# SimonsRoad/gf-pl-slam

Measured on AMD Instinct MI355X. Metric: stereo frames/sec (2k ORB + 500 LBD, 10 GN iters), higher is better.
Workload: dtype f64

## Files before the change

gf-pl-slam_amd/csrc/gfpl_abi.hip:

```cpp
#include <hip/hip_runtime.h>

#include <algorithm>
#include <atomic>
#include <cmath>
#include <mutex>
#include <cstdio>
#include <cstdlib>
#include <cstring>
#include <vector>

#include "../../include/gfpl.h"
#include "gfpl_kernels.hpp"

using namespace gfpl;

#define GFPL_NEV 10

struct gfpl_ctx {
    int device = 0;
    hipStream_t stream = nullptr;
    bool own_stream = false;
    gfpl_camera cam{};
    gfpl_config cfg{};
    bool has_cam = false, has_cfg = false;
// ... 33 lines not shown
struct gfpl_event {
    int device = 0;
    hipEvent_t ev = nullptr;
    int64_t records = 0;
};

int gfpl_ctx_device(const gfpl_ctx* c) { return c->device; }
void* gfpl_ctx_stream(const gfpl_ctx* c) { return (void*)c->stream; }
const gfpl_camera* gfpl_ctx_camera(const gfpl_ctx* c) { return c->has_cam ? &c->cam : nullptr; }
int64_t gfpl_event_records(const gfpl_event* e) { return e->records; }
void gfpl_ctx_attach(gfpl_ctx* c) { c->n_detectors.fetch_add(1); }
void gfpl_ctx_detach(gfpl_ctx* c) { c->n_detectors.fetch_sub(1); }


namespace {

#define HIPCHK(x)                                                  \
    do {                                                            \
        hipError_t e_ = (x);                                        \
        if (e_ != hipSuccess) {                                     \
            std::fprintf(stderr, "gfpl: %s failed: %s\n", #x, hipGetErrorString(e_)); \
            return GFPL_E_HIP;                                      \
        }                                                           \
    } while (0)

int debug_fill_byte() {
    const char* e = getenv("GFPL_DEBUG_FILL");
    return e ? (int)(strtol(e, nullptr, 0) & 0xFF) : 0;
}

template <typename F, typename H, typename V>
void frame_fields(F& f, H& o, V& v) {
    v.pt(f.pt.pl, o.pt_pl, 2); v.pt(f.pt.pl_obs, o.pt_pl_obs, 2);
    v.pt(f.pt.disp, o.pt_disp, 1); v.pt(f.pt.P, o.pt_P, 3); v.pt(f.pt.sigma2, o.pt_sigma2, 1);
    v.pt(f.pt.idx, o.pt_idx, 1); v.pt(f.pt.level, o.pt_level, 1); v.pt(f.pt.inlier, o.pt_inlier, 1);
    v.pt(f.pt.desc, o.pdesc, 32); v.count(f.pt.n);
    v.ls(f.ls.spl, o.ls_spl, 2); v.ls(f.ls.epl, o.ls_epl, 2);
    v.ls(f.ls.spl_obs, o.ls_spl_obs, 2); v.ls(f.ls.epl_obs, o.ls_epl_obs, 2);
    v.ls(f.ls.sdisp, o.ls_sdisp, 1); v.ls(f.ls.edisp, o.ls_edisp, 1);
    v.ls(f.ls.sdisp_obs, o.ls_sdisp_obs, 1); v.ls(f.ls.edisp_obs, o.ls_edisp_obs, 1);
    v.ls(f.ls.angle, o.ls_angle, 1); v.ls(f.ls.sigma2, o.ls_sigma2, 1);
    v.ls(f.ls.sP, o.ls_sP, 3); v.ls(f.ls.eP, o.ls_eP, 3);
    v.ls(f.ls.le, o.ls_le, 3); v.ls(f.ls.le_obs, o.ls_le_obs, 3);
    v.ls(f.ls.covS, o.ls_covS, 9); v.ls(f.ls.covE, o.ls_covE, 9);
    v.ls(f.ls.cut, o.ls_cut, 2); v.ls(f.ls.invcov, o.ls_invcov, 36);
    v.ls(f.ls.idx, o.ls_idx, 1); v.ls(f.ls.level, o.ls_level, 1); v.ls(f.ls.inlier, o.ls_inlier, 1);
    v.ls(f.ls.desc, o.ldesc, 32); v.count(f.ls.n);
    v.seq(f.pose.Tfw, o.Tfw, 16); v.seq(f.pose.DT, o.DT, 16);
    v.seq(f.pose.DT_cov, o.DT_cov, 36); v.seq(f.pose.Tfw_cov, o.Tfw_cov, 36);
    v.seq(f.pose.DT_cov_eig, o.DT_cov_eig, 6);
    v.seq(f.pose.err_norm, &o.err_norm, 1); v.seq(f.pose.time_stamp, &o.time_stamp, 1);
}

struct SlotCarve {
    Carver& c;
    size_t B, P, L;
    template <typename T, typename U> void pt(T*& d, U, int w) { d = c.take<T>(P * w); }
    template <typename T, typename U> void ls(T*& d, U, int w) { d = c.take<T>(L * w); }
    template <typename T, typename U> void seq(T*& d, U, int w) { d = c.take<T>(B * w); }
    void count(int32_t*& d) { d = c.take<int32_t>(B); }
};

void carve(Carver& c, gfpl_seqbatch* sb) {
    const size_t B = sb->B, P = (size_t)B * sb->kp_cap, L = (size_t)B * sb->kl_cap;
    const gfpl_frame_host none{};
    SlotCarve v{c, B, P, L};
    for (int s = 0; s < 2; ++s) frame_fields(sb->slot[s], none, v);
    sb->tr.matched_pt = c.take<int32_t>(B * sb->mpt_cap);
    sb->tr.n_matched_pt = c.take<int32_t>(B);
    sb->tr.matched_ls = c.take<int32_t>(B * sb->mls_cap);
    sb->tr.n_matched_ls = c.take<int32_t>(B);
    sb->tr.n_inliers = c.take<int32_t>(B);
    sb->tr.n_inliers_pt = c.take<int32_t>(B);
    sb->tr.n_inliers_ls = c.take<int32_t>(B);
    sb->tr.num_frame_loss = c.take<int32_t>(B);
    sb->tr.kf_T = c.take<double>(B * 16);
    sb->tr.kf_cov = c.take<double>(B * 36);
    sb->tr.kf_entropy0 = c.take<double>(B);
    sb->tr.kf_ratio = c.take<double>(B);
    sb->tr.kf_prev_iskf = c.take<int32_t>(B);
    sb->tr.kf_nsince = c.take<int32_t>(B);
    sb->tr.kf_flag = c.take<int32_t>(B);
    sb->scr.cut_rec = c.take<double>(B * sb->mls_cap * CUT_REC);
    sb->scr.knn = c.take<int32_t>(B * 2 * (size_t)sb->kp_cap * 3);
    sb->scr.proj = reinterpret_cast<double*>(sb->scr.knn);
    sb->scr.bytes = c.take<int64_t>(B * STEP_REC);
    sb->scr.n_subpix = c.take<int32_t>(B);
    sb->scr.cut_sum = c.take<double>(B * 24);
    sb->scr.cut_dtinv = c.take<double>(B * 16);
    sb->scr.cut_vtab = c.take<double>(B * sb->mls_cap * 2 * CUT_KS);
    sb->scr.pose_DT = c.take<double>(B * 16);
    sb->scr.pose_H = c.take<double>(B * 36);
    sb->scr.pose_err = c.take<double>(B);
    sb->scr.pose_ok = c.take<int32_t>(B);
    sb->scr.pose_in = c.take<double>(B * (6 * (size_t)sb->mpt_cap + 10 * (size_t)sb->mls_cap));
    sb->scr.pose_act = c.take<double>(B * (6 * (size_t)sb->mpt_cap + 10 * (size_t)sb->mls_cap));
    sb->scr.pose_dtini = c.take<double>(B * 16);
    sb->scr.cross_tinv = c.take<double>(B * 16);
    sb->scr.dbg = c.take<int64_t>(B * 8);
    sb->scr.cut_prog = c.take<int32_t>((size_t)1 << 17);
    sb->scr.cut_path = c.take<uint8_t>(B * sb->mls_cap * CUT_PATH);
    sb->scr.cut_flag = c.take<int32_t>(B);
    sb->scr.cut_vmax = c.take<double>(B * sb->mls_cap * CUT_VMAX);
    sb->scr.cut_offl = c.take<int32_t>(1 + B * sb->mls_cap);
    sb->scr.cut_dtln = c.take<int32_t>(1 + CUT_DTL * B);
    sb->scr.cut_dtl = c.take<double>(CUT_DTL * B * 32);
    sb->scr.kf_mask = c.take<int32_t>(B);
    sb->last_n_pt = c.take<int32_t>(B);
    sb->last_n_ls = c.take<int32_t>(B);
}

DevCam devcam(const gfpl_camera& c) {
    DevCam d;
    d.fx = c.fx; d.fy = c.fy; d.cx = c.cx; d.cy = c.cy; d.b = c.b;
    d.width = c.width; d.height = c.height; d.n_levels = c.n_levels;
    for (int i = 0; i < GFPL_MAX_LEVELS; ++i) {
        d.scale[i] = c.scale[i]; d.inv_scale[i] = c.inv_scale[i];
        d.lvl_cols[i] = c.lvl_cols[i]; d.lvl_rows[i] = c.lvl_rows[i];
        d.lvl_offset[i] = c.lvl_offset[i];
        d.sigma2_pt[i] = c.sigma2_pt[i]; d.sigma2_ln[i] = c.sigma2_ln[i];
    }
    d.pyr_bytes = c.pyr_bytes;
    return d;
}

KParams params(gfpl_seqbatch* sb, const gfpl_frames* in) {
    KParams p;
    std::memset(&p, 0, sizeof p);
    p.cam = devcam(sb->ctx->cam);
    p.cfg = sb->ctx->cfg;
    p.prev = sb->slot[sb->prev_slot];
    p.curr = sb->slot[1 - sb->prev_slot];
    p.tr = sb->tr;
    p.scr = sb->scr;
    if (in) p.in = *in;
    p.B = sb->B; p.kp_cap = sb->kp_cap; p.kl_cap = sb->kl_cap;
    p.mpt_cap = sb->mpt_cap; p.mls_cap = sb->mls_cap;
    p.cfg.max_point_match_num = std::min(p.cfg.max_point_match_num, sb->mpt_cap);
    p.cfg.max_line_match_num = std::min(p.cfg.max_line_match_num, sb->mls_cap);
    p.sp_maxD = (float)p.cam.fx;
    p.sp_mbf = (float)(p.cam.fx * p.cam.b);
    p.cut_tq = 0.25 * p.cfg.cut_certify - 4.0 * 0x1p-53;
    {
        const double s = p.cfg.cut_step, lo = p.cfg.cut_rng[0], hi = p.cfg.cut_rng[1];
        auto same = [](double x, double y) { return std::memcmp(&x, &y, sizeof x) == 0; };
        int n = 0;
        for (double t = 0.0; n < CUT_KS && t <= hi && s > 0.0; t = t + s) p.cut_keys[n++] = t;
        const int ns = n;
        for (int i = 1; i < ns && n < CUT_KS; ++i) {
            const double e = p.cut_keys[i] - s;
            bool have = false;
            for (int k = 0; k < n; ++k) have = have || same(p.cut_keys[k], e);
            if (!have && e >= lo) p.cut_keys[n++] = e;
        }
        for (int i = 0; i < n; ++i) {
            int up = -1, dn = -1;
            for (int k = 0; k < n; ++k) {
                if (same(p.cut_keys[k], p.cut_keys[i] + s)) up = k;
                if (same(p.cut_keys[k], p.cut_keys[i] - s)) dn = k;
            }
            p.cut_knxt[i] = (int8_t)up;
            p.cut_kprv[i] = (int8_t)dn;
        }
        p.cut_nkeys = n;
    }
    return p;
// ... 898 lines not shown
    HIPCHK(v.e);
    HIPCHK(hipStreamSynchronize(s));
    sb->initialized = true;
    if (which == GFPL_CURR) sb->has_curr = true;
    return GFPL_OK;
}

int gfpl_read_track(gfpl_seqbatch* sb, int seq, gfpl_track_host* o) {
    return read_track(sb, seq, o, sb ? sb->tr.n_matched_pt : nullptr, sb ? sb->tr.n_matched_ls : nullptr);
}

int gfpl_read_last_track(gfpl_seqbatch* sb, int seq, gfpl_track_host* o) {
    return read_track(sb, seq, o, sb ? sb->last_n_pt : nullptr, sb ? sb->last_n_ls : nullptr);
}

int gfpl_write_track(gfpl_seqbatch* sb, int seq, const gfpl_track_host* o) {
    if (!sb || !o || seq < 0 || seq >= sb->B) return GFPL_E_INVALID;
    if (o->n_matched_pt < 0 || o->n_matched_pt > sb->mpt_cap || o->n_matched_ls < 0 || o->n_matched_ls > sb->mls_cap)
        return GFPL_E_CAPACITY;
    hipStream_t s = sb->ctx->stream;
    XFER(h2d, sb->tr.n_matched_pt + seq, &o->n_matched_pt, 1);
    XFER(h2d, sb->tr.n_matched_ls + seq, &o->n_matched_ls, 1);
    XFER(h2d, sb->tr.n_inliers + seq, &o->n_inliers, 1);
    XFER(h2d, sb->tr.n_inliers_pt + seq, &o->n_inliers_pt, 1);
    XFER(h2d, sb->tr.n_inliers_ls + seq, &o->n_inliers_ls, 1);
    XFER(h2d, sb->tr.num_frame_loss + seq, &o->num_frame_loss, 1);
    XFER(h2d, sb->tr.matched_pt + (size_t)seq * sb->mpt_cap, o->matched_pt, (size_t)o->n_matched_pt);
    XFER(h2d, sb->tr.matched_ls + (size_t)seq * sb->mls_cap, o->matched_ls, (size_t)o->n_matched_ls);
    HIPCHK(hipStreamSynchronize(s));
    return GFPL_OK;
}

int gfpl_set_timing(gfpl_ctx* c, int enable) {
    if (!c) return GFPL_E_INVALID;
    c->timing = enable != 0;
    return GFPL_OK;
}

int gfpl_get_stage_times(gfpl_ctx* c, float* ms7) {
    if (!c || !ms7) return GFPL_E_INVALID;
    if (!c->timing) return GFPL_E_STATE;
    HIPCHK(hipEventSynchronize(c->ev[6]));
    for (int i = 0; i < 6; ++i) HIPCHK(hipEventElapsedTime(&ms7[i], c->ev[i], c->ev[i + 1]));
    HIPCHK(hipEventElapsedTime(&ms7[6], c->ev[0], c->ev[6]));
    return GFPL_OK;
}

int gfpl_get_kernel_times(gfpl_ctx* c, float* ms4) {
    if (!c || !ms4) return GFPL_E_INVALID;
    if (!c->timing) return GFPL_E_STATE;
    if (!c->cfg.use_line_conf_cut) return GFPL_E_STATE;
    HIPCHK(hipEventSynchronize(c->ev[6]));
    HIPCHK(hipEventElapsedTime(&ms4[0], c->ev[4], c->ev[7]));
    HIPCHK(hipEventElapsedTime(&ms4[1], c->ev[7], c->ev[8]));
    HIPCHK(hipEventElapsedTime(&ms4[2], c->ev[8], c->ev[5]));
    HIPCHK(hipEventElapsedTime(&ms4[3], c->ev[5], c->ev[9]));
    return GFPL_OK;
}

}

namespace {
int step_rec_sums(gfpl_seqbatch* sb, int64_t* sums) {
    std::vector<int64_t> v((size_t)sb->B * STEP_REC);
    HIPCHK(hipStreamSynchronize(sb->ctx->stream));
    HIPCHK(hipMemcpy(v.data(), sb->scr.bytes, sizeof(int64_t) * v.size(), hipMemcpyDeviceToHost));
    for (int s = 0; s < STEP_REC; ++s) {
        int64_t t = 0;
        for (int b = 0; b < sb->B; ++b) t += v[(size_t)b * STEP_REC + s];
        sums[s] = t;
    }
    return GFPL_OK;
}
}

extern "C" {

int gfpl_last_step_kernel_bytes(gfpl_seqbatch* sb, int64_t* bytes4) {
    if (!sb || !bytes4) return GFPL_E_INVALID;
    int64_t v[STEP_REC];
    int e = step_rec_sums(sb, v);
    if (e) return e;
    const bool cut = sb->last_cut_mode >= 0;
    bytes4[0] = cut ? 212 * v[14] + 44 * v[13] + 552 * (int64_t)sb->B : 0;
    bytes4[1] = v[7];
    bytes4[2] = cut ? 612 * v[14] : 0;
    bytes4[3] = v[5];
    return GFPL_OK;
}

int gfpl_last_step_stage_bytes(gfpl_seqbatch* sb, int64_t* bytes7) {
    if (!sb || !bytes7) return GFPL_E_INVALID;
    int64_t v[STEP_REC];
    int e = step_rec_sums(sb, v);
    if (e) return e;
    for (int s = 0; s < 7; ++s) bytes7[s] = v[s];
    return GFPL_OK;
}

int gfpl_last_step_counts(gfpl_seqbatch* sb, int64_t* counts8) {
    if (!sb || !counts8) return GFPL_E_INVALID;
    int64_t v[STEP_REC];
    int e = step_rec_sums(sb, v);
    if (e) return e;
    for (int s = 0; s < 8; ++s) counts8[s] = v[8 + s];
    return GFPL_OK;
}

int gfpl_last_step_track_counts(gfpl_seqbatch* sb, int64_t* counts4) {
    if (!sb || !counts4) return GFPL_E_INVALID;
    int64_t v[STEP_REC];
    int e = step_rec_sums(sb, v);
    if (e) return e;
    for (int s = 0; s < 4; ++s) counts4[s] = v[16 + s];
    return GFPL_OK;
}

int gfpl_last_step_cut_proof(gfpl_seqbatch* sb, int64_t* counts4) {
    if (!sb || !counts4) return GFPL_E_INVALID;
    int64_t v[STEP_REC];
    int e = step_rec_sums(sb, v);
    if (e) return e;
    const bool on = sb->last_cut_mode == 1 || sb->last_cut_mode == 3;
    for (int s = 0; s < 4; ++s) counts4[s] = on ? v[20 + s] : 0;
    return GFPL_OK;
}

int gfpl_debug_cut_records(gfpl_seqbatch* sb, int b, double* out, int n_lines) {
    if (!sb || !out || b < 0 || b >= sb->B || n_lines < 0 || n_lines > sb->mls_cap) return GFPL_E_INVALID;
    if (hipSetDevice(sb->ctx->device) != hipSuccess) return GFPL_E_HIP;
    if (hipStreamSynchronize(sb->ctx->stream) != hipSuccess) return GFPL_E_HIP;
    const size_t n = (size_t)n_lines * CUT_REC;
    return hipMemcpy(out, sb->scr.cut_rec + (size_t)b * sb->mls_cap * CUT_REC, n * sizeof(double),
                     hipMemcpyDeviceToHost) == hipSuccess ? GFPL_OK : GFPL_E_HIP;
}

int gfpl_debug_step_records(gfpl_seqbatch* sb, int64_t* out) {
    if (!sb || !out) return GFPL_E_INVALID;
    if (hipSetDevice(sb->ctx->device) != hipSuccess) return GFPL_E_HIP;
    if (hipStreamSynchronize(sb->ctx->stream) != hipSuccess) return GFPL_E_HIP;
    return hipMemcpy(out, sb->scr.bytes, (size_t)sb->B * STEP_REC * sizeof(int64_t), hipMemcpyDeviceToHost) == hipSuccess
               ? GFPL_OK : GFPL_E_HIP;
}

int gfpl_debug_clocks(gfpl_seqbatch* sb, int64_t* out) {
    if (!sb || !out) return GFPL_E_INVALID;
    if (hipSetDevice(sb->ctx->device) != hipSuccess) return GFPL_E_HIP;
    if (hipStreamSynchronize(sb->ctx->stream) != hipSuccess) return GFPL_E_HIP;
    return hipMemcpy(out, sb->scr.dbg, (size_t)sb->B * 8 * sizeof(int64_t), hipMemcpyDeviceToHost) == hipSuccess
               ? GFPL_OK : GFPL_E_HIP;
}

int gfpl_last_step_bytes(gfpl_seqbatch* sb, int64_t* bytes) {
    if (!bytes) return GFPL_E_INVALID;
    int64_t v[7];
    int e = gfpl_last_step_stage_bytes(sb, v);
    if (e) return e;
    *bytes = v[6];
    return GFPL_OK;
}

}
```

gf-pl-slam_amd/csrc/gfpl_state.hpp:

```cpp
#pragma once
#include <stdint.h>

#include "../../include/gfpl.h"
#include "gfpl_device.hpp"

namespace gfpl {

struct DevPoints {
    double* pl;
    double* pl_obs;
    double* disp;
    double* P;
    double* sigma2;
    int32_t* idx;
    int32_t* level;
    uint8_t* inlier;
    uint8_t* desc;
    int32_t* n;
};

struct DevLines {
    double *spl, *epl, *spl_obs, *epl_obs;
    double *sdisp, *edisp, *sdisp_obs, *edisp_obs;
    double *angle, *sigma2;
    double *sP, *eP, *le, *le_obs;
    double *covS, *covE;
    double *cut;
    double *invcov;
    int32_t *idx, *level;
    uint8_t *inlier;
    uint8_t *desc;
    int32_t* n;
};

struct DevPose {
    double *Tfw, *DT;
    double *DT_cov, *Tfw_cov;
    double *DT_cov_eig;
    double *err_norm, *time_stamp;
};

struct DevFrame {
    DevPoints pt;
    DevLines ls;
    DevPose pose;
};

struct DevTrack {
    int32_t* matched_pt;
    int32_t* n_matched_pt;
    int32_t* matched_ls;
    int32_t* n_matched_ls;
    int32_t* n_inliers;
    int32_t* n_inliers_pt;
    int32_t* n_inliers_ls;
    int32_t* num_frame_loss;
    double* kf_T;
    double* kf_cov;
    double* kf_entropy0;
    double* kf_ratio;
    int32_t* kf_prev_iskf;
    int32_t* kf_nsince;
    int32_t* kf_flag;
};

#define STEP_REC 24
#define CUT_PATH 64
#define CUT_DTL 4
#define CUT_VMAX 14
#define CUT_P_STAY 8
#define CUT_P_EXACT 16
#define CUT_KS 22
#define CUT_FAST 56
#define CUT_REC 80

struct DevScratch {
    double* cut_rec;
    int32_t* knn;
    double* proj;
    int64_t* bytes;
    int32_t* n_subpix;
    double* cut_sum;
    double* cut_dtinv;
    double* cut_vtab;
    double* pose_DT;
    double* pose_H;
    double* pose_err;
    int32_t* pose_ok;
    double* pose_in;
    double* pose_act;
    double* pose_dtini;
    int32_t* kf_mask;
    double* cross_tinv;
    int64_t* dbg;
    int32_t* cut_prog;
    uint8_t* cut_path;
    int32_t* cut_flag;
    int32_t* cut_offl;
    int32_t* cut_dtln;
    double* cut_dtl;
    double* cut_vmax;
};

struct KParams {
    DevCam cam;
    gfpl_config cfg;
    DevFrame prev, curr;
    DevTrack tr;
    DevScratch scr;
    gfpl_frames in;
    int B, kp_cap, kl_cap, mpt_cap, mls_cap;
    const double* dt_ini;
    float sp_maxD, sp_mbf;
    double cut_tq;
    double cut_keys[CUT_KS];
    int cut_nkeys;
    int8_t cut_knxt[CUT_KS], cut_kprv[CUT_KS];
};

}
```

gf-pl-slam_amd/csrc/k_cut.hip:

```cpp
#include <cstdlib>

#include "gfpl_kernels.hpp"

namespace gfpl {

struct LineCutData {
    double sP[3], eP[3], covS[9], covE[9], Jl[2];
};

template <typename T, bool SD = false>
__device__ __forceinline__ T endpointVar_t(const DevCam& cam, const double* DT_inv, const T* Jl, const T* Pt,
                                           const T* cov, double zlo) {
    T Jdt[9];
#pragma unroll
    for (int i = 0; i < 3; ++i)
#pragma unroll
        for (int j = 0; j < 3; ++j) Jdt[i * 3 + j] = T(DT_inv[i * 4 + j]);
    T cur[3];
    se3_apply_t<T, double>(DT_inv, Pt, cur);
    rb_floor(cur[2], zlo);
    const T f = T(cam.fx), pz = cur[2], pz_2 = pz * pz;
    T Jp[9];
    Jp[0] = f / pz; Jp[3] = T(0.0); Jp[6] = T(0.0);
    Jp[1] = T(0.0); Jp[4] = f / pz; Jp[7] = T(0.0);
// ... 32 lines not shown
    const T r0 = Jl[0] * M[0] + Jl[1] * M[2];
    const T r1 = Jl[0] * M[1] + Jl[1] * M[3];
    return r0 * Jl[0] + r1 * Jl[1];
}

template <typename T, bool VAR = true>
__device__ __forceinline__ void cut_endpoint_t(const DevCam& cam, double homog, const double* DT_inv, const T* Jl,
                                               const T* P0, const T* P1, const T* C0, const T* C1, T c, T* out7,
                                               double zlo) {
    T Pt[3];
#pragma unroll
    for (int k = 0; k < 3; ++k) Pt[k] = (T(1.0) - c) * P0[k] + c * P1[k];
    if (VAR) {
        const T a = (T(1.0) - c) * (T(1.0) - c), q = c * c;
        T cov[9];
#pragma unroll
        for (int i = 0; i < 9; ++i) cov[i] = a * C0[i] + q * C1[i];
        out7[0] = endpointVar_t<T>(cam, DT_inv, Jl, Pt, cov, zlo);
    }
    T cur[3];
    se3_apply_t<T, double>(DT_inv, Pt, cur);
    rb_floor(cur[2], zlo);
    poseJac_t<T>(cam, homog, cur, Jl[0], Jl[1], out7 + 1);
}
__device__ __forceinline__ void cut_endpoint(const DevCam& cam, double homog, const double* DT_inv, const double* Jl,
                                             const double* P0, const double* P1, const double* C0, const double* C1,
                                             double c, double* out7) {
    cut_endpoint_t<double>(cam, homog, DT_inv, Jl, P0, P1, C0, C1, c, out7, 0.0);
}

template <bool FULL>
__device__ __forceinline__ void cut_assemble(const double* S7, const double* E7, double* info) {
    const double vs = S7[0], ve = E7[0];
    const double* Js = S7 + 1;
    const double* Je = E7 + 1;
    const double det = vs * ve - 0.0 * 0.0;
    const double invdet = 1.0 / det;
    const double i00 = ve * invdet, i10 = -0.0 * invdet, i01 = -0.0 * invdet, i11 = vs * invdet;
    double T0[6], T1[6];
#pragma unroll
    for (int i = 0; i < 6; ++i) {
        T0[i] = Js[i] * i00 + Je[i] * i10;
        T1[i] = Js[i] * i01 + Je[i] * i11;
    }
    if (FULL) {
#pragma unroll
        for (int i = 0; i < 6; ++i)
#pragma unroll
            for (int j = 0; j < 6; ++j) info[i * 6 + j] = T0[i] * Js[j] + T1[i] * Je[j];
    } else {
#pragma unroll
        for (int i = 0; i < 6; ++i)
#pragma unroll
            for (int j = 0; j <= i; ++j) info[tri(i, j)] = T0[i] * Js[j] + T1[i] * Je[j];
    }
}

template <bool FULL>
__device__ __forceinline__ void poseInfoOnLine(const DevCam& cam, double homog, const double* DT_inv,
                                               const LineCutData& L, double c0, double c1, double* info) {
    double S7[7], E7[7];
    cut_endpoint(cam, homog, DT_inv, L.Jl, L.sP, L.eP, L.covS, L.covE, c0, S7);
    cut_endpoint(cam, homog, DT_inv, L.Jl, L.eP, L.sP, L.covE, L.covS, c1, E7);
    cut_assemble<FULL>(S7, E7, info);
}

__device__ __forceinline__ void load_line(const DevLines& L, size_t q, LineCutData& d) {
#pragma unroll
    for (int k = 0; k < 3; ++k) { d.sP[k] = L.sP[3 * q + k]; d.eP[k] = L.eP[3 * q + k]; }
#pragma unroll
    for (int k = 0; k < 9; ++k) { d.covS[k] = L.covS[9 * q + k]; d.covE[k] = L.covE[9 * q + k]; }
    d.Jl[0] = L.le_obs[3 * q];
    d.Jl[1] = L.le_obs[3 * q + 1];
}

#define PD_PS 0
#define PD_PE 18
#define PD_VS 36
#define PD_VE 41
#define PD_OK 46
#define PD_NEXT 47
#define PD_ERR 48
static_assert(CUT_FAST == 56, "per-line comparison data layout");

template <typename T>
__device__ __forceinline__ T sym3_t(const T* A, const T* x, const T* y) {
    const T ax = (A[0] * y[0] + A[1] * y[1]) + A[2] * y[2];
    const T ay = (A[1] * y[0] + A[3] * y[1]) + A[4] * y[2];
    const T az = (A[2] * y[0] + A[4] * y[1]) + A[5] * y[2];
    return (x[0] * ax + x[1] * ay) + x[2] * az;
}

template <typename T>
__device__ __forceinline__ void cut_poly_coeff_t(const T* g0, const T* g1, T lx, T ly, int k, T* Pk) {
    const T dx = g1[0] - g0[0], dy = g1[1] - g0[1], dz = g1[2] - g0[2];
    auto prod = [&](T a0, T a1, T b0, T b1) -> T {
        return k == 0 ? a0 * b0 : (k == 1 ? a0 * b1 + a1 * b0 : a1 * b1);
    };
    auto lin = [&](T a0, T a1) -> T { return k == 0 ? a0 : (k == 1 ? a1 : T(0.0)); };
    const T x0 = g0[0], y0 = g0[1], z0 = g0[2];
    Pk[0] = lx * lin(z0, dz);
    Pk[1] = ly * lin(z0, dz);
    Pk[2] = -(lx * lin(x0, dx) + ly * lin(y0, dy));
    Pk[3] = -((lx * prod(x0, dx, y0, dy) + ly * prod(y0, dy, y0, dy)) + ly * prod(z0, dz, z0, dz));
    Pk[4] = (lx * prod(x0, dx, x0, dx) + lx * prod(z0, dz, z0, dz)) + ly * prod(x0, dx, y0, dy);
    Pk[5] = ly * prod(x0, dx, z0, dz) - lx * prod(y0, dy, z0, dz);
}

template <typename T>
__device__ __forceinline__ void cut_poly_coef_t(const double* Dl, const T* sP, const T* eP, const T* covS,
                                                const T* covE, const T* Jl, T* P, T* V, T* g) {
    se3_apply_t<T, double>(Dl, sP, g);
    se3_apply_t<T, double>(Dl, eP, g + 3);
    T A[2][6];
    const T* Cs[2] = {covS, covE};
#pragma unroll
    for (int w = 0; w < 2; ++w) {
        T Tm[9];
#pragma unroll
        for (int i = 0; i < 3; ++i)
#pragma unroll
            for (int k = 0; k < 3; ++k)
                Tm[i * 3 + k] = (T(Dl[i * 4 + 0]) * Cs[w][0 * 3 + k] + T(Dl[i * 4 + 1]) * Cs[w][1 * 3 + k]) +
                                T(Dl[i * 4 + 2]) * Cs[w][2 * 3 + k];
        const int ii[6] = {0, 0, 0, 1, 1, 2}, jj[6] = {0, 1, 2, 1, 2, 2};
#pragma unroll
        for (int e = 0; e < 6; ++e)
            A[w][e] = (Tm[ii[e] * 3 + 0] * T(Dl[jj[e] * 4 + 0]) + Tm[ii[e] * 3 + 1] * T(Dl[jj[e] * 4 + 1])) +
                      Tm[ii[e] * 3 + 2] * T(Dl[jj[e] * 4 + 2]);
    }
#pragma unroll
    for (int side = 0; side < 2; ++side) {
        T* Ps = P + 18 * side;
#pragma unroll
        for (int k = 0; k < 3; ++k) cut_poly_coeff_t<T>(g + 3 * side, g + 3 * (1 - side), Jl[0], Jl[1], k, Ps + 6 * k);
        const T* p0 = Ps;
        const T* p1 = Ps + 6;
        const T a0 = sym3_t<T>(A[side], p0, p0), a1 = sym3_t<T>(A[side], p0, p1), a2 = sym3_t<T>(A[side], p1, p1);
        const T b0 = sym3_t<T>(A[1 - side], p0, p0), b1 = sym3_t<T>(A[1 - side], p0, p1), b2 = sym3_t<T>(A[1 - side], p1, p1);
        T* v = V + 5 * side;
        v[0] = a0;
        v[1] = T(2.0) * (a1 - a0);
        v[2] = ((a2 - T(4.0) * a1) + a0) + b0;
        v[3] = T(2.0) * ((a1 - a2) + b1);
        v[4] = a2 + b2;
    }
}

__device__ __forceinline__ void cut_poly_data(const double* Dl, const LineCutData& d, double homog, double* fd) {
    double P[36], V[10], g[6];
    cut_poly_coef_t<double>(Dl, d.sP, d.eP, d.covS, d.covE, d.Jl, P, V, g);
#pragma unroll
    for (int i = 0; i < 18; ++i) { fd[PD_PS + i] = P[i]; fd[PD_PE + i] = P[18 + i]; }
#pragma unroll
    for (int i = 0; i < 5; ++i) { fd[PD_VS + i] = V[i]; fd[PD_VE + i] = V[5 + i]; }
    const double z0 = g[2], z1 = g[5];
    fd[PD_OK] = (((z0 > 0.0 && z1 > 0.0) || (z0 < 0.0 && z1 < 0.0)) && z0 * z0 > 2.0 * homog && z1 * z1 > 2.0 * homog)
                    ? 1.0 : 0.0;
}

__device__ __forceinline__ void wave_lds_sync() { asm volatile("s_waitcnt lgkmcnt(0)" ::: "memory"); }

template <int W>
__global__ void __launch_bounds__(64 * W) k_cut_prep(KParams p) {
    extern __shared__ double prep_lds[];
    const int b = blockIdx.x;
    const int lane = threadIdx.x & 63, wv = W > 1 ? (int)(threadIdx.x >> 6) : 0;
    const int nls = p.tr.n_matched_ls[b];
    const int npt = p.tr.n_matched_pt[b];
    if (nls == 0) return;
    double (*chunk)[65] = reinterpret_cast<double (*)[65]>(prep_lds + (size_t)wv * 21 * 65);
    const DevCam& cam = p.cam;
    const double homog = p.cfg.homog_th;
    DevLines& L = p.prev.ls;
    const DevPoints& P = p.prev.pt;
    const size_t lb = (size_t)b * p.kl_cap, pbase = (size_t)b * p.kp_cap;
    const int32_t* mls = p.tr.matched_ls + (size_t)b * p.mls_cap;
    const int32_t* mpt = p.tr.matched_pt + (size_t)b * p.mpt_cap;
    double* rec_l = p.scr.cut_rec + (size_t)b * p.mls_cap * CUT_REC;
    double Dl[16];
    {
        double Tc[16], Tp[16], Ti[16];
#pragma unroll
        for (int i = 0; i < 16; ++i) { Tc[i] = p.curr.pose.Tfw[16 * b + i]; Tp[i] = p.prev.pose.Tfw[16 * b + i]; }
        mat4_inv(Tc, Ti);
        mat4_mul(Ti, Tp, Dl);
    }
    if (wv == 0 && lane < 16) p.scr.cut_dtinv[16 * b + lane] = Dl[lane];
    double s = 0.0;
    const int nl_ch = (nls + 63) >> 6, np_ch = (npt + 63) >> 6;
    auto chunk_cnt = [&](int c) {
        const bool lines = c < nl_ch;
        return min(64, (lines ? nls : npt) - (((lines ? c : c - nl_ch)) << 6));
    };
    for (int c0 = 0; c0 < nl_ch + np_ch; c0 += W) {
        const int c = c0 + wv;
        if (c < nl_ch + np_ch) {
            const bool lines = c < nl_ch;
            const int m = ((lines ? c : c - nl_ch) << 6) + lane;
            const int cnt = chunk_cnt(c);
            double info[21];
            double fd[CUT_FAST];
            if (lane < cnt) {
                if (lines) {
                    LineCutData d;
                    load_line(L, lb + mls[m], d);
                    poseInfoOnLine<false>(cam, homog, Dl, d, 0.0, 0.0, info);
#pragma unroll
                    for (int i = PD_ERR; i < CUT_FAST; ++i) fd[i] = 0.0;
                    cut_poly_data(Dl, d, homog, fd);
                    fd[PD_NEXT] = (double)mls[min(m + 1, nls - 1)];
                } else {
                    const size_t q = pbase + mpt[m];
                    double Pp[3] = {P.P[3 * q], P.P[3 * q + 1], P.P[3 * q + 2]};
                    double cur[3], uv[2];
                    se3_apply(Dl, Pp, cur);
                    projection(cam, cur, uv);
                    const double dx = uv[0] - P.pl_obs[2 * q], dy = uv[1] - P.pl_obs[2 * q + 1];
                    double J[6];
                    poseJac(cam, homog, cur, dx, dy, J);
#pragma unroll
                    for (int i = 0; i < 6; ++i)
#pragma unroll
                        for (int j = 0; j <= i; ++j) info[tri(i, j)] = J[i] * J[j];
                }
            }
            if (lines) {
                double* stg = &chunk[0][0];
                const int pl = lane >> 3, pp = lane & 7;
                double* rc = rec_l + (size_t)(c << 6) * CUT_REC;
#pragma unroll
                for (int sl = 0; sl < CUT_REC / 16; ++sl) {
                    if (lane < cnt) {
#pragma unroll
                        for (int k = 0; k < 16; ++k) {
                            const int x = 16 * sl + k;
                            stg[lane * 17 + k] = x < CUT_FAST ? fd[x] : (x < CUT_FAST + 21 ? info[x - CUT_FAST] : 0.0);
                        }
                    }
                    wave_lds_sync();
#pragma unroll
                    for (int g8 = 0; g8 < 8; ++g8) {
                        const int ln = 8 * g8 + pl;
                        if (ln < cnt)
                            reinterpret_cast<double2*>(rc + (size_t)ln * CUT_REC + 16 * sl)[pp] =
                                make_double2(stg[ln * 17 + 2 * pp], stg[ln * 17 + 2 * pp + 1]);
                    }
                    wave_lds_sync();
                }
            }
            if (lane < cnt) {
#pragma unroll
                for (int i = 0; i < 21; ++i) chunk[i][lane] = info[i];
            }
        }
        __syncthreads();
        if (wv == 0 && lane < 21) {
            const double (*all)[21][65] = reinterpret_cast<const double (*)[21][65]>(prep_lds);
            for (int k = 0; k < W && c0 + k < nl_ch + np_ch; ++k) {
                const int cnt = chunk_cnt(c0 + k);
                for (int e = 0; e < cnt; ++e) s = s + all[k][lane][e];
            }
        }
        __syncthreads();
    }
    if (wv == 0 && lane < 21) p.scr.cut_sum[24 * b + lane] = s;
}
constexpr size_t cut_prep_lds(int w) { return (size_t)w * 21 * 65 * sizeof(double); }

__device__ __forceinline__ float ceil_f32(double x) {
    if (!(x >= 0.0)) return __builtin_inff();
    float f = (float)x;
    if ((double)f < x) f = __uint_as_float(__float_as_uint(f) + 1u);
    return f;
}
__device__ __forceinline__ double ref_vprime(const DevCam& cam, double homog, const double* Dl, const DevLines& L,
                                             size_t q, int side, double c) {
    const double* P0 = side ? L.eP + 3 * q : L.sP + 3 * q;
    const double* P1 = side ? L.sP + 3 * q : L.eP + 3 * q;
    const double* C0 = side ? L.covE + 9 * q : L.covS + 9 * q;
    const double* C1 = side ? L.covS + 9 * q : L.covE + 9 * q;
    const double Jl[2] = {L.le_obs[3 * q], L.le_obs[3 * q + 1]};
    double Pt[3];
#pragma unroll
    for (int k = 0; k < 3; ++k) Pt[k] = (1.0 - c) * P0[k] + c * P1[k];
    const double a = (1.0 - c) * (1.0 - c), qq = c * c;
    double cov[9];
#pragma unroll
    for (int i = 0; i < 9; ++i) cov[i] = a * C0[i] + qq * C1[i];
    const double v = endpointVar_t<double>(cam, Dl, Jl, Pt, cov, 0.0);
    double cur[3];
    se3_apply(Dl, Pt, cur);
    const double f = cam.fx / ref_max(homog, cur[2] * cur[2]);
    return v / (f * f);
}

__global__ void __launch_bounds__(256) k_cut_vtab(KParams p) {
    const int b = blockIdx.x;
    const int nls = p.tr.n_matched_ls[b];
    const int nk = p.cut_nkeys;
    if (nls == 0 || nk == 0 || (p.cfg.cut_proof != 2 && p.scr.cut_flag[b] == 0)) return;
    const DevLines& L = p.prev.ls;
    const double* Dl = p.scr.cut_dtinv + 16 * (size_t)b;
    const int per = 2 * nk;
    for (int idx = threadIdx.x; idx < nls * per; idx += 256) {
        const int m = idx / per, r = idx - m * per;
        const int side = r >= nk ? 1 : 0, slot = r - side * nk;
        const size_t q = (size_t)b * p.kl_cap + p.tr.matched_ls[(size_t)b * p.mls_cap + m];
        p.scr.cut_vtab[((size_t)b * p.mls_cap + m) * (2 * CUT_KS) + side * CUT_KS + slot] =
            ref_vprime(p.cam, p.cfg.homog_th, Dl, L, q, side, p.cut_keys[slot]);
    }
}

__device__ __forceinline__ void cut_line_bounds(const KParams& p, size_t q, bool pd_ok, const double* Dl, float* eb) {
    const DevLines& L = p.prev.ls;
    const double rlo = p.cfg.cut_rng[0], rhi = p.cfg.cut_rng[1];
    const double C = fmax(rhi, 0.0), T = fmax(fabs(rlo), fabs(rhi));
#pragma unroll
    for (int i = 0; i < 14; ++i) eb[i] = __builtin_inff();
    bool ok = rlo >= 0.0 && rhi <= 1.0 && pd_ok && p.cam.fx > 0.0;
// ... 34 lines not shown
#pragma unroll
        for (int side = 0; side < 2; ++side) {
            RB o7[7];
            cut_endpoint_t<RB, false>(p.cam, p.cfg.homog_th, Dl, Jl, side ? eP : sP, side ? sP : eP, side ? cE : cS,
                                      side ? cS : cE, RB(C, 0.0, 0.0), o7, zlo);
#pragma unroll
            for (int i = 0; i < 6; ++i) eb[7 * side + i] = ceil_f32(1.01 * (eo[side][i] + o7[1 + i].e * s1));
            {
                const RB c(C, 0.0, 0.0);
                const RB* Q0 = side ? eP : sP;
                const RB* Q1 = side ? sP : eP;
                RB Pt[3], cur[3];
#pragma unroll
                for (int k = 0; k < 3; ++k) Pt[k] = (RB(1.0) - c) * Q0[k] + c * Q1[k];
                se3_apply_t<RB, double>(Dl, Pt, cur);
                rb_floor(cur[2], zlo);
                eb[7 * side + 6] = cur[2].lo > 0.0 ? ceil_f32(1.01 * cur[2].e / cur[2].lo) : __builtin_inff();
            }
        }
    }
}

__device__ __forceinline__ void cut_line_bounds_p(const KParams& p, size_t q, bool pd_ok, const double* Dl, float* eb) {
    const DevLines& L = p.prev.ls;
    const double rlo = p.cfg.cut_rng[0], rhi = p.cfg.cut_rng[1];
    const double C = fmax(rhi, 0.0), T = fmax(fabs(rlo), fabs(rhi));
#pragma unroll
    for (int i = 0; i < 14; ++i) eb[i] = __builtin_inff();
    if (!(rlo >= 0.0 && rhi <= 1.0 && pd_ok && p.cam.fx > 0.0)) return;
    RB sP[3], eP[3], Jl[2];
#pragma unroll
    for (int k = 0; k < 3; ++k) { sP[k] = RB(L.sP[3 * q + k]); eP[k] = RB(L.eP[3 * q + k]); }
    Jl[0] = RB(L.le_obs[3 * q]);
    Jl[1] = RB(L.le_obs[3 * q + 1]);
    RB g[6];
    se3_apply_t<RB, double>(Dl, sP, g);
    se3_apply_t<RB, double>(Dl, eP, g + 3);
    double gd[6];
    {
        const double s3[3] = {L.sP[3 * q], L.sP[3 * q + 1], L.sP[3 * q + 2]};
        const double e3[3] = {L.eP[3 * q], L.eP[3 * q + 1], L.eP[3 * q + 2]};
        se3_apply(Dl, s3, gd);
        se3_apply(Dl, e3, gd + 3);
    }
    const double zlo = fmin(fabs(gd[2]) - g[2].e, fabs(gd[5]) - g[5].e);
    const double zmax = fmax(fabs(gd[2]) + g[2].e, fabs(gd[5]) + g[5].e);
    if (!(zlo > 0.0)) return;
    const double s1 = zmax * zmax / p.cam.fx;
#pragma unroll
    for (int side = 0; side < 2; ++side) {
        double eo[6] = {0, 0, 0, 0, 0, 0};
        double tk = 1.0;
#pragma unroll
        for (int k = 0; k < 3; ++k) {
            RB Pk[6];
            cut_poly_coeff_t<RB>(g + 3 * side, g + 3 * (1 - side), Jl[0], Jl[1], k, Pk);
#pragma unroll
            for (int i = 0; i < 6; ++i) eo[i] = eo[i] + tk * Pk[i].e;
            tk = tk * T;
        }
        RB o7[7];
        cut_endpoint_t<RB, false>(p.cam, p.cfg.homog_th, Dl, Jl, side ? eP : sP, side ? sP : eP, nullptr, nullptr,
                                  RB(C, 0.0, 0.0), o7, zlo);
#pragma unroll
        for (int i = 0; i < 6; ++i) eb[7 * side + i] = ceil_f32(1.01 * (eo[i] + o7[1 + i].e * s1));
        const RB c(C, 0.0, 0.0);
        const RB* Q0 = side ? eP : sP;
        const RB* Q1 = side ? sP : eP;
        RB Pt[3], cur[3];
#pragma unroll
        for (int k = 0; k < 3; ++k) Pt[k] = (RB(1.0) - c) * Q0[k] + c * Q1[k];
        se3_apply_t<RB, double>(Dl, Pt, cur);
        rb_floor(cur[2], zlo);
        eb[7 * side + 6] = cur[2].lo > 0.0 ? ceil_f32(1.01 * cur[2].e / cur[2].lo) : __builtin_inff();
    }
}

__global__ void __launch_bounds__(64) k_cut_bounds(KParams p) {
    const int b = blockIdx.y;
    const int m = blockIdx.x * 64 + threadIdx.x;
    const int nls = p.tr.n_matched_ls[b];
    if (m >= nls || (p.cfg.cut_proof != 2 && p.scr.cut_flag[b] == 0)) return;
    const size_t q = (size_t)b * p.kl_cap + p.tr.matched_ls[(size_t)b * p.mls_cap + m];
    double* rec = p.scr.cut_rec + ((size_t)b * p.mls_cap + m) * CUT_REC;
    double Dl[16];
#pragma unroll
    for (int i = 0; i < 16; ++i) Dl[i] = p.scr.cut_dtinv[16 * b + i];
    float eb[14];
    cut_line_bounds(p, q, rec[PD_OK] != 0.0, Dl, eb);
    float* out = reinterpret_cast<float*>(rec + PD_ERR);
#pragma unroll
    for (int i = 0; i < 14; ++i) out[i] = eb[i];
}

#define CUT_G 8
#ifndef CUT_BATCH
#define CUT_BATCH 8
#endif
#ifndef CUT_WAIT
#define CUT_WAIT 16
#endif
#define CUT_SL 7
#define CUT_EP 43
#define CUT_NX (CUT_FAST + 21)
static_assert(CUT_REC * 8 == 640 && CUT_NX + 3 <= CUT_REC, "a record is 5 x 128 B: five 16-B loads per lane");

__device__ __forceinline__ void exact_endpoint(const DevCam& cam, double homog, const double* Dl, const DevLines& L,
                                               size_t q, int side, double t, double* o7) {
    const double* sP = L.sP + 3 * q;
    const double* eP = L.eP + 3 * q;
    const double* cS = L.covS + 9 * q;
    const double* cE = L.covE + 9 * q;
    const double Jl[2] = {L.le_obs[3 * q], L.le_obs[3 * q + 1]};
    cut_endpoint(cam, homog, Dl, Jl, side ? eP : sP, side ? sP : eP, side ? cE : cS, side ? cS : cE, t, o7);
}

__device__ __forceinline__ int nb_off(int j, int side) {
    const unsigned pl = side == 0 ? 0x31u : 0x54u, mi = side == 0 ? 0xC2u : 0xA8u;
    return (int)((pl >> j) & 1u) - (int)((mi >> j) & 1u);
}
__device__ __forceinline__ double nb_step(int j, int side, double st) {
    return (double)nb_off(j, side) * st;
}
__device__ __forceinline__ int nb_slot(int j, int side) {
    return 1 + nb_off(j, side);
}

constexpr double CUT_MIN_PIVOT = 1e-2;
__device__ __forceinline__ void chol_s(const double* a, double* out) {
    double L[21];
#pragma unroll
    for (int i = 0; i < 21; ++i) L[i] = a[i];
    bool ok = true;
#pragma unroll
    for (int k = 0; k < 6; ++k) {
        const double akk = L[tri(k, k)];
        double x = akk;
#pragma unroll
        for (int j = 0; j < k; ++j) x = x - L[tri(k, j)] * L[tri(k, j)];
        if (!(x > CUT_MIN_PIVOT * akk && akk < 1e300)) { ok = false; x = 1.0; }
        double r = __builtin_amdgcn_rsq(x);
        r = r * (1.5 - (0.5 * x) * (r * r));
        r = r * (1.5 - (0.5 * x) * (r * r));
        L[tri(k, k)] = 0.0;
        out[21 + k] = r;
#pragma unroll
        for (int i = k + 1; i < 6; ++i) {
            double v = L[tri(i, k)];
#pragma unroll
            for (int j = 0; j < k; ++j) v = v - L[tri(i, j)] * L[tri(k, j)];
            L[tri(i, k)] = v * r;
        }
    }
#pragma unroll
    for (int i = 0; i < 21; ++i) out[i] = L[i];
    out[27] = ok ? 1.0 : 0.0;
}

__device__ __forceinline__ double rcp_fast(double x) {
    double r = __builtin_amdgcn_rcp(x);
    r = __builtin_fma(__builtin_fma(-x, r, 1.0), r, r);
    r = __builtin_fma(__builtin_fma(-x, r, 1.0), r, r);
    return r;
}

__device__ __forceinline__ double h4(const double* c, double t) {
    return __builtin_fma(t, __builtin_fma(t, __builtin_fma(t, __builtin_fma(t, c[4], c[3]), c[2]), c[1]), c[0]);
}
__device__ __forceinline__ double h4abs(const double* c, double t) {
    return __builtin_fma(t, __builtin_fma(t, __builtin_fma(t, __builtin_fma(t, fabs(c[4]), fabs(c[3])), fabs(c[2])),
                                          fabs(c[1])), fabs(c[0]));
}
__device__ __forceinline__ double h2(double c0, double c1, double c2, double t) {
    return __builtin_fma(t, __builtin_fma(t, c2, c1), c0);
}

__device__ __forceinline__ double cut_ours_P(const double* fd, int side, int i, double t) {
    const int o = side ? PD_PE : PD_PS;
    return h2(fd[o + i], fd[o + 6 + i], fd[o + 12 + i], t);
}
__device__ __forceinline__ double cut_ours_V(const double* fd, int side, double t) {
    const int o = side ? PD_VE : PD_VS;
    return __builtin_fma(t, __builtin_fma(t, __builtin_fma(t, __builtin_fma(t, fd[o + 4], fd[o + 3]), fd[o + 2]),
                                          fd[o + 1]), fd[o]);
}
__device__ __forceinline__ double cut_ours_info(const double* xs, double is, double ie, int ra, int cb) {
    return __builtin_fma(xs[1 + ra] * is, xs[1 + cb], (xs[8 + ra] * ie) * xs[8 + cb]);
}

struct __attribute__((aligned(16))) CutCmp {
    double ns[5], ne[5];
    double vs[5], ve[5];
    double cc[9];
    double bnd[3];
    double bs[3], be[3];
    float eb[6];
};
static_assert(sizeof(CutCmp) == 336, "CutCmp: 84 dwords (bank spread of the 8 groups' rows)");
struct CutReg {
    double ns[5], ne[5], vs[5], ve[5], cc[9], bnd[3];
    float eb[6];
};
__device__ __forceinline__ void cut_reg_load(const CutCmp& c, CutReg& r) {
#pragma unroll
    for (int i = 0; i < 5; ++i) { r.ns[i] = c.ns[i]; r.ne[i] = c.ne[i]; r.vs[i] = c.vs[i]; r.ve[i] = c.ve[i]; }
#pragma unroll
    for (int i = 0; i < 9; ++i) r.cc[i] = c.cc[i];
#pragma unroll
    for (int i = 0; i < 3; ++i) r.bnd[i] = c.bnd[i];
#pragma unroll
    for (int i = 0; i < 6; ++i) r.eb[i] = c.eb[i];
}

template <bool PROOF>
__device__ __forceinline__ double cut_dcore_p1(double Ns, double Vs, double Ne, double Ve, double C, double P1,
                                              double VsA, double VeA, const float* eb, double tq, int& bound_ok) {
    const double D = __builtin_fma(Vs + Ns, Ve + Ne, -(C * C));
    const double den = Vs * Ve;
    const double r = rcp_fast(den);
    const double d = D * r;
    const double P2 = __builtin_fma(VsA, Ve, VeA * Vs);
    constexpr double u = 0x1p-53;
    const double Dd = D * den;
    const bool healthy = (Vs > 0.0) & (Ve > 0.0) & (D > 0.0) & (d < 1e300) & (Dd < 1e300);
    const float iVs = (float)(Ve * r), iVe = (float)(Vs * r);
    const float E = __builtin_fmaf(iVs, __builtin_fmaf(eb[2], iVs, eb[1]), iVe * __builtin_fmaf(eb[4], iVe, eb[3]));
    bool agree = true;
    if (PROOF) agree = (E * 1.0001f <= eb[0]) & (eb[5] * (iVs + iVe) <= 0.25f);
    (void)E;
    const bool fwd = __builtin_fma((40.0 * u) * P1, den, ((16.0 * u) * P2) * D) <= tq * Dd;
    bound_ok = healthy & agree & fwd;
    return healthy ? d : __longlong_as_double(0x7ff8000000000000ll);
}
template <bool PROOF>
__device__ __forceinline__ double cut_dval(const CutReg& c, double t0, double t1, double tq, int& bound_ok,
                                           double vs_t = 0.0, double ve_t = 0.0) {
    const double Ns = h4(c.ns, t0), Ne = h4(c.ne, t1);
    const double Vs = PROOF ? vs_t : h4(c.vs, t0), Ve = PROOF ? ve_t : h4(c.ve, t1);
    const double C = __builtin_fma(t1, __builtin_fma(t1, h2(c.cc[2], c.cc[5], c.cc[8], t0), h2(c.cc[1], c.cc[4], c.cc[7], t0)),
                                   h2(c.cc[0], c.cc[3], c.cc[6], t0));
    return cut_dcore_p1<PROOF>(Ns, Vs, Ne, Ve, C, c.bnd[0], c.bnd[1], c.bnd[2], c.eb, tq, bound_ok);
}

__device__ __attribute__((noinline)) double cut_exact_step(const double* sj, const double* ej, const double* s1,
                                                           const double* e4, const double* S, const double* Sb,
                                                           int first, double* mc) {
    double tot[21], tmp[21];
    cut_assemble<false>(sj, ej, tmp);
#pragma unroll
    for (int i = 0; i < 21; ++i) tot[i] = tmp[i] + S[i];
    const double vj = logdet6_lower(tot);
    if (first) {
#pragma unroll
        for (int i = 0; i < 21; ++i) tot[i] = Sb[i];
    } else {
        cut_assemble<false>(s1, e4, tmp);
#pragma unroll
        for (int i = 0; i < 21; ++i) tot[i] = tmp[i] + S[i];
    }
    *mc = logdet6_lower(tot);
    return vj;
}


// ... 14 lines not shown
template <int CTRL>
__device__ __forceinline__ double dpp_mov_f64(double v) {
    const int lo = __builtin_amdgcn_mov_dpp(__double2loint(v), CTRL, 0xF, 0xF, false);
    const int hi = __builtin_amdgcn_mov_dpp(__double2hiint(v), CTRL, 0xF, 0xF, false);
    return __hiloint2double(hi, lo);
}
__device__ __forceinline__ int group_first_max(double v, int valid, int j, double mc, double& top) {
    const double x = (valid && v == v) ? v : -__builtin_inf();
    double mx = fmax(x, dpp_mov_f64<DPP_XOR1>(x));
    mx = fmax(mx, dpp_mov_f64<DPP_XOR2>(mx));
    mx = fmax(mx, dpp_mov_f64<DPP_HALF_MIRROR>(mx));
    top = mx;
    const unsigned long long at = __ballot((x == mx) & (mx > -__builtin_inf()));
    const unsigned gb = (unsigned)(at >> (threadIdx.x & ~7u)) & 0xFFu;
    const int k = gb ? __builtin_ctz(gb) : 8;
    (void)j;
    return (k < 8 && mx > mc) ? k : -1;
}


struct CutX {
    int best;
    int m_sync;
};
template <typename T>
__device__ __forceinline__ T* rl_ptr(T* p, int l) {
    const unsigned long long v = reinterpret_cast<unsigned long long>(p);
    const unsigned lo = (unsigned)__builtin_amdgcn_readlane((int)(unsigned)v, l);
    const unsigned hi = (unsigned)__builtin_amdgcn_readlane((int)(unsigned)(v >> 32), l);
    return reinterpret_cast<T*>(((unsigned long long)hi << 32) | lo);
}
__device__ __attribute__((noinline)) CutX cut_exact_round(bool exact, int valid, int first, int m, int m_sync, double r0,
                                                          double r1, size_t q_cur, size_t lb, int best,
                                                          const int32_t* mls, const double* rec_l, double* sP, double* eP,
                                                          double* covS, double* covE, double* le_obs, double* cut,
                                                          double* sumE, double* tmp, double* tmpw, const double* Dl,
                                                          double fx, double cb, double homog, double st) {
    const int j = threadIdx.x & 7;
    const int lane = threadIdx.x & 63;
    DevCam cam{};
    cam.fx = fx;
    cam.b = cb;
    DevLines L{};
    L.sP = sP;
    L.eP = eP;
    L.covS = covS;
    L.covE = covE;
    L.le_obs = le_obs;
    L.cut = cut;
    __builtin_amdgcn_fence(__ATOMIC_SEQ_CST, "workgroup");
    {
        unsigned long long need = __ballot(j == 0 && exact && m_sync < m);
        while (need) {
            const int gl = __ffsll((long long)need) - 1;
            need &= need - 1;
            const int ms = __builtin_amdgcn_readlane(m_sync, gl), me = __builtin_amdgcn_readlane(m, gl);
            const size_t lbG = (size_t)(unsigned)__builtin_amdgcn_readlane((int)(unsigned)lb, gl) |
                               ((size_t)(unsigned)__builtin_amdgcn_readlane((int)(unsigned)(lb >> 32), gl) << 32);
            const int32_t* mlsG = rl_ptr(mls, gl);
            const double* recG = rl_ptr(rec_l, gl);
            const double* DlG = rl_ptr(Dl, gl);
            double* sumEG = rl_ptr(sumE, gl);
            const bool mine = (lane >> 3) == (gl >> 3);
            for (int s0 = ms; s0 < me; s0 += 64) {
                const int nl = min(64, me - s0);
                double info[21];
                if (lane < nl) {
                    const size_t qf = lbG + mlsG[s0 + lane];
                    const double c0 = __hip_atomic_load(&L.cut[2 * qf], __ATOMIC_RELAXED, __HIP_MEMORY_SCOPE_WORKGROUP);
                    const double c1 = __hip_atomic_load(&L.cut[2 * qf + 1], __ATOMIC_RELAXED, __HIP_MEMORY_SCOPE_WORKGROUP);
                    double s7[7], e7[7];
                    exact_endpoint(cam, homog, DlG, L, qf, 0, c0, s7);
                    exact_endpoint(cam, homog, DlG, L, qf, 1, c1, e7);
                    cut_assemble<false>(s7, e7, info);
                }
#pragma unroll
                for (int c = 0; c < 6; ++c) {
                    if (lane < nl) {
#pragma unroll
                        for (int i = 0; i < 4; ++i) {
                            const int e = 4 * c + i;
                            if (e < 21) {
                                tmpw[4 * lane + i] = info[e];
                                tmpw[256 + 4 * lane + i] = recG[(size_t)(s0 + lane) * CUT_REC + CUT_FAST + e];
                            }
                        }
                    }
                    wave_lds_sync();
                    if (mine && j < 4 && 4 * c + j < 21) {
                        const int e = 4 * c + j;
                        double Se = sumEG[e];
                        for (int l = 0; l < nl; ++l) Se = (Se - tmpw[256 + 4 * l + j]) + tmpw[4 * l + j];
                        sumEG[e] = Se;
                    }
                    wave_lds_sync();
                }
            }
            if (mine) m_sync = me;
        }
    }
    double* const epf = tmp;
    double* const xs = tmp + CUT_EP;
    if (exact) {
        if (j < 6) {
            const int eside = j < 3 ? 0 : 1;
            const double eoff = (j % 3) == 0 ? -st : ((j % 3) == 2 ? st : 0.0);
            const double t = (eside == 0 ? r0 : r1) + eoff;
            double o7[7];
            exact_endpoint(cam, homog, Dl, L, q_cur, eside, t, o7);
#pragma unroll
            for (int i = 0; i < 7; ++i) epf[CUT_SL * j + i] = o7[i];
        }
#pragma unroll
        for (int e = 0; e < 21; ++e) xs[e] = sumE[e] - rec_l[(size_t)m * CUT_REC + CUT_FAST + e];
    }
    wave_lds_sync();
    if (exact) {
        const int cs = nb_slot(j, 0), ce = 3 + nb_slot(j, 1);
        double mc, top;
        const double vj = cut_exact_step(&epf[CUT_SL * cs], &epf[CUT_SL * ce], &epf[CUT_SL * 1], &epf[CUT_SL * 4], xs,
                                         sumE, first, &mc);
        best = group_first_max(vj, valid, j, mc, top);
    }
    wave_lds_sync();
    return CutX{best, m_sync};
}

constexpr unsigned long long tri_pack(int want_row) {
    unsigned long long v = 0;
    int e = 0;
    for (int i = 0; i < 6; ++i)
        for (int k = 0; k <= i; ++k, ++e) v |= (unsigned long long)(want_row ? i : k) << (3 * e);
    return v;
}

__device__ __attribute__((noinline)) void cut_bound_row(int j, double T, const double* fs, const double* sA,
                                                        const double* tg, double* wg) {
    const float* ef = reinterpret_cast<const float*>(fs + PD_ERR);
    const double sg = 1.002 * tg[57 + j];
    const double Sii = sA[tri(j, j)];
    const double es = ef[j], ee = ef[7 + j];
    const double ps = fabs(fs[PD_PS + j]) + T * (fabs(fs[PD_PS + 6 + j]) + T * fabs(fs[PD_PS + 12 + j])) + es;
    const double pe = fabs(fs[PD_PE + j]) + T * (fabs(fs[PD_PE + 6 + j]) + T * fabs(fs[PD_PE + 12 + j])) + ee;
    const double rs = sqrt(sg);
    double row = 0.0;
    const double kc = Sii * sg;
    const int ex = __builtin_amdgcn_frexp_exp(Sii);
    wg[j] = kc;
    wg[6 + j] = sqrt(kc);
    wg[12 + j] = sg * ps * ps;
    wg[18 + j] = sg * pe * pe;
    wg[24 + j] = es * rs;
    wg[30 + j] = ee * rs;
    wg[36 + j] = (Sii > 0.0 && Sii < 1e300) ? 0.6931471805599453 * (double)(abs(ex) + 1) : __builtin_inf();
    wg[42 + j] = row * rs;
}
__device__ __attribute__((noinline)) void cut_bound_line(double T, double tau, const double* cl, const double* fs,
                                                         const double* wg, float* eb) {
    const float* ef = reinterpret_cast<const float*>(fs + PD_ERR);
    const double Bs = h2(cl[32], cl[33], cl[34], T), Be = h2(cl[35], cl[36], cl[37], T);
    double sum[8];
    for (int q = 0; q < 8; ++q) {
        double a = wg[6 * q];
        for (int i = 1; i < 6; ++i) a = a + wg[6 * q + i];
        sum[q] = a;
    }
    constexpr double u = 0x1p-53;
    const double Kc = sum[0], xi = sum[1], Qs = sum[2], Qe = sum[3], Lam = sum[6];
    const double epsS = sum[7] + (7.01 * u) * xi * xi;
    const double hs = sum[4] + (6.01 * u) * Bs * xi, he = sum[5] + (6.01 * u) * Be * xi;
    const double rvs = 4.1 * (double)ef[6] + 12.0 * u, rve = 4.1 * (double)ef[13] + 12.0 * u;
    const double ck = 110.0 * u;
    const double K0 = 1.002 * epsS + ck * Kc + (7.1 * u) * Lam;
    const double bs = Bs + hs, be = Be + he;
    const double A1 = 1.03 * (2.0 * ck * Qs + 4.0 * hs * bs + 4.0 * rvs * bs * bs), A2 = 0.0;
    const double B1 = 1.03 * (2.0 * ck * Qe + 4.0 * he * be + 4.0 * rve * be * be), B2 = 0.0;
    double R0 = fmin(0.125 * tau, 1e-3) - 1.01 * K0;
    if (!(epsS <= 1e-3 && Kc <= 1e8 && R0 > 0.0)) R0 = -1.0;
    float r0f = (float)R0;
    if ((double)r0f > R0) r0f = R0 > 0.0 ? __uint_as_float(__float_as_uint(r0f) - 1u) : -1.0f;
    eb[0] = r0f;
    eb[1] = ceil_f32(A1);
    eb[2] = ceil_f32(A2);
    eb[3] = ceil_f32(B1);
    eb[4] = ceil_f32(B2);
    eb[5] = (rvs <= 0.25 && rve <= 0.25) ? 0.0f : __builtin_inff();
}

__device__ __forceinline__ int wave_sum8(int v) {
    v += __shfl_xor(v, 8);
    v += __shfl_xor(v, 16);
    v += __shfl_xor(v, 32);
    return __builtin_amdgcn_readfirstlane(v);
}
struct CutProg { int* own; int* partner; };
__device__ __forceinline__ CutProg cut_prog_slots(int* base) {
    const unsigned hw = __builtin_amdgcn_s_getreg((4 << 0) | (0 << 6) | (31 << 11));
    const unsigned xcc = __builtin_amdgcn_s_getreg((20 << 0) | (0 << 6) | (31 << 11));
    const unsigned simd = ((((xcc & 7u) * 8u + ((hw >> 13) & 7u)) * 2u + ((hw >> 12) & 1u)) * 16u + ((hw >> 8) & 15u)) * 4u +
                          ((hw >> 4) & 3u);
    const unsigned slot = hw & 15u;
    return CutProg{base + simd * 16u + slot, base + simd * 16u + (slot ^ 1u)};
}
#ifndef GFPL_CUT_WPE
#define GFPL_CUT_WPE 2
#endif
#ifndef GFPL_CUT_NOPF
#define GFPL_CUT_NOPF 0
#endif
#define CUT_SSTR (GFPL_CUT_NOPF ? 21 : 25)
template <bool PROOF, bool REC = false>
__global__ void __launch_bounds__(64) __attribute__((amdgpu_waves_per_eu(GFPL_CUT_WPE, GFPL_CUT_WPE))) k_cut_search(KParams p) {
    __shared__ double sumA[CUT_G][CUT_SSTR];
    __shared__ double sumE[CUT_G][CUT_SSTR];
    __shared__ double fst[CUT_G][CUT_FAST + 1];
    constexpr bool PF = !PROOF && !GFPL_CUT_NOPF;
    __shared__ __attribute__((aligned(16))) double nxl[PF ? 5 : 1][PF ? 128 : 2];
    __shared__ double tmp[CUT_G][CUT_EP + 25 + 1];
    static_assert(CUT_G * (CUT_EP + 25 + 1) >= 512, "the exact-sum flush stages 64 x (4 + 4) doubles in tmp");
    __shared__ CutCmp cmpl[CUT_G];
    __shared__ double vtab[PROOF ? CUT_G : 1][PROOF ? 2 * CUT_KS : 1];
    __shared__ int cnxt[PROOF ? CUT_KS : 1], cprv[PROOF ? CUT_KS : 1];
    const int lane = threadIdx.x;
#ifdef GFPL_CUT_CLOCK
    const uint64_t t_beg = wall_clock64();
#endif
    const int g = lane >> 3, j = lane & 7;
    const int b = blockIdx.x * CUT_G + g;
    if (!PROOF && p.cfg.cut_proof == 0 && j == 0 && b < p.B) {
        p.scr.dbg[8 * (size_t)b + 6] = (int64_t)__builtin_amdgcn_s_getreg((4 << 0) | (0 << 6) | (31 << 11));
        p.scr.dbg[8 * (size_t)b + 7] = (int64_t)__builtin_amdgcn_s_getreg((20 << 0) | (0 << 6) | (31 << 11));
    }
    const bool live = b < p.B && (!PROOF || p.cfg.cut_proof == 2 || p.scr.cut_flag[b] != 0);
    const int nls = live ? p.tr.n_matched_ls[b] : 0;
    constexpr bool rec = !PROOF && REC;
    uint8_t* const path = p.scr.cut_path + (size_t)(live ? b : 0) * p.mls_cap * CUT_PATH;
    int lstep = 0;
    __shared__ __attribute__((aligned(8))) uint8_t pth[REC ? CUT_G : 1][REC ? CUT_PATH : 8];
    const DevCam& cam = p.cam;
    const double homog = p.cfg.homog_th;
    const double tau = p.cfg.cut_certify;
    const double tq = p.cut_tq;
    DevLines& L = p.prev.ls;
    const size_t lb = (size_t)(live ? b : 0) * p.kl_cap;
    const int32_t* mls = p.tr.matched_ls + (size_t)(live ? b : 0) * p.mls_cap;
    const double* rec_l = p.scr.cut_rec + (size_t)(live ? b : 0) * p.mls_cap * CUT_REC;
    const double* Dl = p.scr.cut_dtinv + 16 * (size_t)(live ? b : 0);
    const double st = p.cfg.cut_step;
    const double rlo = p.cfg.cut_rng[0], rhi = p.cfg.cut_rng[1];
    double* const xs = &tmp[g][CUT_EP];
    double* const wg = &tmp[g][0];
    double* const gm = &tmp[g][36];
    const double nb0 = nb_step(j, 0, st), nb1 = nb_step(j, 1, st);
    constexpr unsigned long long TRI_ROW = tri_pack(1), TRI_COL = tri_pack(0);
    if (PROOF) {
        if (lane < CUT_KS) {
            cnxt[lane] = p.cut_knxt[lane];
            cprv[lane] = p.cut_kprv[lane];
        }
        __syncthreads();
    }
    int m = 0;
    int m_sync = 0;
    int first = 1;
    double r0 = 0.0, r1 = 0.0;
    int line_ok = 0;
    int pend = 0;
    int wait = 0;
    double dc = 0.0;
    int c_ok = 0;
    int n_unb = 0;
    int i0 = 0, i1 = 0, n0s = -1, p0s = -1, n1s = -1, p1s = -1;
    size_t q_cur = 0, q_nx = 0;
    auto open_line = [&]() {
        if (PROOF) {
            const double* vt = p.scr.cut_vtab + ((size_t)(live ? b : 0) * p.mls_cap + m) * (2 * CUT_KS);
            for (int idx = j; idx < 2 * CUT_KS; idx += 8) vtab[g][idx] = vt[idx];
            i0 = 0;
            i1 = 0;
            n0s = n1s = cnxt[0];
            p0s = p1s = cprv[0];
        }
        double o[28];
        {
            double S[21];
#pragma unroll
            for (int e = 0; e < 21; ++e) S[e] = sumA[g][e];
            chol_s(S, o);
        }
        line_ok = (o[27] != 0.0) && (fst[g][PD_OK] != 0.0);
        if (j < 6) {
            double w[6];
#pragma unroll
            for (int i = 0; i < 6; ++i) {
                double u = fst[g][6 * j + i];
#pragma unroll
                for (int k = 0; k < i; ++k) u = __builtin_fma(-o[tri(i, k)], w[k], u);
                w[i] = u * o[21 + i];
            }
#pragma unroll
            for (int i = 0; i < 6; ++i) wg[6 * j + i] = w[i];
            double x[6], sg = 0.0;
            if (PROOF) {
#pragma unroll
            for (int i = 0; i < 6; ++i) {
                double uu = i == j ? 1.0 : 0.0;
#pragma unroll
                for (int k = 0; k < i; ++k) uu = __builtin_fma(-o[tri(i, k)], x[k], uu);
                x[i] = uu * o[21 + i];
                sg = __builtin_fma(x[i], x[i], sg);
            }
            tmp[g][57 + j] = sg;
            }
        }
        wave_lds_sync();
#pragma unroll
        for (int kk = 0; kk < 3; ++kk) {
            const int e = j + 8 * kk;
            if (e < 21) {
                const int ra = (int)((TRI_ROW >> (3 * e)) & 7), cb = (int)((TRI_COL >> (3 * e)) & 7);
                double s = wg[6 * ra] * wg[6 * cb];
#pragma unroll
                for (int i = 1; i < 6; ++i) s = __builtin_fma(wg[6 * ra + i], wg[6 * cb + i], s);
                gm[e] = s;
            }
        }
        wave_lds_sync();
        double* cl = reinterpret_cast<double*>(&cmpl[g]);
        if (j < 2) {
            const int a = 3 * j, b2 = a + 1, c2 = a + 2;
            double* o = cl + 5 * j;
            o[0] = gm[tri(a, a)];
            o[1] = 2.0 * gm[tri(b2, a)];
            o[2] = __builtin_fma(2.0, gm[tri(c2, a)], gm[tri(b2, b2)]);
            o[3] = 2.0 * gm[tri(c2, b2)];
            o[4] = gm[tri(c2, c2)];
        } else if (j < 4) {
#pragma unroll
            for (int i = 0; i < 5; ++i) cl[10 + 5 * (j - 2) + i] = fst[g][PD_VS + 5 * (j - 2) + i];
        } else if (j < 7) {
            const int i = j - 4;
#pragma unroll
            for (int k = 0; k < 3; ++k) cl[20 + 3 * i + k] = gm[tri(3 + k, i)];
            const double gs = fmax(gm[tri(i, i)], 0.0), ge = fmax(gm[tri(3 + i, 3 + i)], 0.0);
            cl[32 + i] = gs > 0.0 ? 1.01 * gs * __builtin_amdgcn_rsq(gs) : 0.0;
            cl[35 + i] = ge > 0.0 ? 1.01 * ge * __builtin_amdgcn_rsq(ge) : 0.0;
        }
        wave_lds_sync();
        const double T = fmax(fabs(rlo), fabs(rhi));
        if (j == 7) {
            const double Bs = h2(cl[32], cl[33], cl[34], T), Be = h2(cl[35], cl[36], cl[37], T);
            const double VsA = h4abs(cl + 10, T), VeA = h4abs(cl + 15, T);
            const double Bs2 = Bs * Bs, Be2 = Be * Be;
            cl[29] = __builtin_fma(Bs2 + VsA, Be2 + VeA, Bs2 * Be2);
            cl[30] = VsA;
            cl[31] = VeA;
        } else if (PROOF && j < 6) {
            cut_bound_row(j, T, fst[g], sumA[g], tmp[g], wg);
        }
        wave_lds_sync();
        if (PROOF && j == 7) cut_bound_line(T, tau, cl, fst[g], wg, cmpl[g].eb);
        wave_lds_sync();
        if (PROOF) {
            const float* e6 = cmpl[g].eb;
            bool usable = e6[0] > 0.0f;
#pragma unroll
            for (int i = 1; i < 6; ++i) usable = usable && e6[i] < __builtin_inff();
            n_unb += usable ? 0 : 1;
            if (j < 6 && live) reinterpret_cast<float*>(const_cast<double*>(rec_l) + (size_t)m * CUT_REC + CUT_NX)[j] = e6[j];
        }
        const double vs0 = PROOF ? vtab[g][0] : cl[10], ve0 = PROOF ? vtab[g][CUT_KS] : cl[15];
        dc = cut_dcore_p1<PROOF>(cl[0], vs0, cl[5], ve0, cl[20], cl[29], cl[30], cl[31], cmpl[g].eb, tq, c_ok);
    };
    auto pf_issue = [&](int mm) {
        if (!PF) return;
        const char* src = reinterpret_cast<const char*>(rec_l + (size_t)mm * CUT_REC) + 16 * j;
#pragma unroll
        for (int k = 0; k < (PF ? 5 : 0); ++k) {
            const uint32_t dst = (uint32_t)(uintptr_t)&nxl[k][0];
            asm volatile("s_mov_b32 m0, %1\n\tglobal_load_lds_dwordx4 %0, off" ::"v"(src + 128 * k), "s"(dst)
                         : "memory", "m0");
        }
    };
    if (m < nls) {
        q_cur = lb + mls[0];
        if (nls > 1) q_nx = lb + mls[1];
        for (int e = j; e < CUT_FAST; e += 8) fst[g][e] = rec_l[e];
#pragma unroll
        for (int e = j; e < 21; e += 8) {
            const double s0 = p.scr.cut_sum[24 * b + e];
            sumA[g][e] = s0 - rec_l[CUT_FAST + e];
            sumE[g][e] = s0;
        }
        wave_lds_sync();
        open_line();
        if (nls > 1) pf_issue(1);
    }
    __syncthreads();
    int n_steps = 0, n_exact = 0;
    const CutProg prog = cut_prog_slots(p.scr.cut_prog);
    if (lane == 0) __hip_atomic_store(prog.own, 0, __ATOMIC_RELAXED, __HIP_MEMORY_SCOPE_AGENT);
    int partner_done = 0;
    __shared__ int pslot[1];
    if (!PROOF && lane == 0) pslot[0] = 0;
    __builtin_amdgcn_s_setprio(2);
#ifdef GFPL_CUT_PCLOCK
    uint64_t pk[4] = {0, 0, 0, 0};
    uint64_t pk0 = clock64();
    int n_it = 0, n_tr = 0;
    uint64_t tk[3] = {0, 0, 0}, tk0 = 0;
#define PCK(i) do { const uint64_t t_ = clock64(); pk[i] += t_ - pk0; pk0 = t_; } while (0)
#define TCK0() do { tk0 = clock64(); } while (0)
#define TCK(i) do { const uint64_t t_ = clock64(); tk[i] += t_ - tk0; tk0 = t_; } while (0)
#else
#define PCK(i) do { } while (0)
#define TCK0() do { } while (0)
#define TCK(i) do { } while (0)
#endif
    while (__any(m < nls)) {
        const bool act = m < nls && !pend;
        const double t0 = r0 + nb0, t1 = r1 + nb1;
        int valid = act ? 1 : 0;
        if (t0 + t1 > 1.0) valid = 0;
        if (t0 < rlo || t0 > rhi) valid = 0;
        if (t1 < rlo || t1 > rhi) valid = 0;
        int bok;
        double dj;
        CutReg cr;
        cut_reg_load(cmpl[g], cr);
        double vst = 0.0, vet = 0.0;
        if (PROOF) {
            const int s0 = nb0 > 0.0 ? n0s : (nb0 < 0.0 ? p0s : i0);
            const int s1 = nb1 > 0.0 ? n1s : (nb1 < 0.0 ? p1s : i1);
            vst = s0 >= 0 ? vtab[g][s0] : __longlong_as_double(0x7ff8000000000000ll);
            vet = s1 >= 0 ? vtab[g][CUT_KS + s1] : __longlong_as_double(0x7ff8000000000000ll);
        }
        dj = cut_dval<PROOF>(cr, t0, t1, tq, bok, vst, vet);
        double top;
        int best = group_first_max(dj, valid, j, dc, top);
        const bool has = best >= 0, vl = valid != 0;
        const bool f1 = vl & !bok;
        const bool f2 = has & vl & (j != best) & !(top - dj > tau * top);
        const bool f3 = has & !(top - dc > tau * top);
        const bool f4 = !has & vl & !(dc - dj > tau * dc);
        const bool f5 = !((tau > 0.0) & (line_ok != 0) & (c_ok != 0) & (dc == dc));
        const int ok = (f1 | f2 | f3 | f4 | f5) ? 0 : 1;
        const bool exact = act && ((__ballot(!ok) >> (8 * g)) & 0xFFull) != 0;
        n_steps += act ? 1 : 0;
        n_exact += exact ? 1 : 0;
        double dnext = top;
        int cnext = 1;
        PCK(0);
        if (__any(exact)) {
            const CutX xr = cut_exact_round(exact, valid, first, m, m_sync, r0, r1, q_cur, lb, best, mls, rec_l, L.sP, L.eP,
                                            L.covS, L.covE, L.le_obs, L.cut, sumE[g], tmp[g], &tmp[0][0], Dl, cam.fx, cam.b,
                                            homog, st);
            best = xr.best;
            m_sync = xr.m_sync;
            const int src = (lane & ~7) + (best >= 0 ? best : 0);
            const double sd = __shfl(dj, src);
            const int sb = __shfl(bok, src);
            if (exact) { dnext = sd; cnext = sb; }
        }
        PCK(1);
        int finalize = 0;
        if (rec && act) {
            if (j == 0 && lstep < CUT_PATH)
                pth[g][lstep] = (uint8_t)((best >= 0 ? best : CUT_P_STAY) | (exact ? CUT_P_EXACT : 0));
            ++lstep;
        }
        if (act) {
            first = 0;
            if (best >= 0) {
                if (PROOF) {
                    const double a0 = nb_step(best, 0, st), a1 = nb_step(best, 1, st);
                    i0 = i0 < 0 ? -1 : (a0 > 0.0 ? n0s : (a0 < 0.0 ? p0s : i0));
                    i1 = i1 < 0 ? -1 : (a1 > 0.0 ? n1s : (a1 < 0.0 ? p1s : i1));
                    n0s = i0 >= 0 ? cnxt[i0] : -1;
                    p0s = i0 >= 0 ? cprv[i0] : -1;
                    n1s = i1 >= 0 ? cnxt[i1] : -1;
                    p1s = i1 >= 0 ? cprv[i1] : -1;
                }
                r0 = r0 + nb_step(best, 0, st);
                r1 = r1 + nb_step(best, 1, st);
                dc = dnext;
                c_ok = cnext;
                if (!(r0 + r1 <= 1.0)) finalize = 1;
            } else {
                finalize = 1;
            }
        }
        if (rec && act && finalize && m + 1 >= nls) {
            __builtin_amdgcn_wave_barrier();
            if (8 * j < lstep)
                *reinterpret_cast<unsigned long long*>(path + (size_t)m * CUT_PATH + 8 * j) =
                    *reinterpret_cast<const unsigned long long*>(&pth[g][8 * j]);
        }
        if (act && finalize) {
            if (j == 0 && (PROOF || m + 1 >= nls)) {
                L.cut[2 * q_cur] = r0;
                L.cut[2 * q_cur + 1] = r1;
            }
            ++m;
            pend = m < nls;
            wait = 0;
        }
        PCK(2);
        const int npend = __popcll(__ballot(pend)) >> 3;
#ifdef GFPL_CUT_PCLOCK
        ++n_it;
#endif
        if (npend > 0 && (npend >= CUT_BATCH || __any(pend && wait >= CUT_WAIT) || __ballot(m < nls && !pend) == 0)) {
#ifdef GFPL_CUT_PCLOCK
            ++n_tr;
#endif
            TCK0();
            double info[3];
            if (pend) {
                if (!PROOF && fst[g][PD_OK] != 0.0) {
                    if (j < 6) {
                        xs[1 + j] = cut_ours_P(fst[g], 0, j, r0);
                        xs[8 + j] = cut_ours_P(fst[g], 1, j, r1);
                    } else {
                        xs[7 * (j - 6)] = cut_ours_V(fst[g], j - 6, j == 6 ? r0 : r1);
                    }
                } else if (j < 2) {
                    double o7[7];
                    exact_endpoint(cam, homog, Dl, L, q_cur, j, j ? r1 : r0, o7);
#pragma unroll
                    for (int i = 0; i < 7; ++i) xs[7 * j + i] = o7[i];
                }
            }
            wave_lds_sync();
            if (pend) {
                const double is = rcp_fast(xs[0]), ie = rcp_fast(xs[7]);
                const double invdet = 1.0 / (xs[0] * xs[7] - 0.0 * 0.0);
                const double i00 = xs[7] * invdet, i10 = -0.0 * invdet, i01 = -0.0 * invdet, i11 = xs[0] * invdet;
#pragma unroll
                for (int kk = 0; kk < 3; ++kk) {
                    const int e = min(j + 8 * kk, 20);
                    const int ra = (int)((TRI_ROW >> (3 * e)) & 7), cb = (int)((TRI_COL >> (3 * e)) & 7);
                    if (PROOF) {
                        const double T0 = xs[1 + ra] * i00 + xs[8 + ra] * i10, T1 = xs[1 + ra] * i01 + xs[8 + ra] * i11;
                        info[kk] = T0 * xs[1 + cb] + T1 * xs[8 + cb];
                    } else {
                        info[kk] = cut_ours_info(xs, is, ie, ra, cb);
                    }
                }
                if (!PF) {
#pragma unroll
                    for (int k = 0; k < CUT_FAST / 8; ++k) fst[g][j + 8 * k] = rec_l[(size_t)m * CUT_REC + j + 8 * k];
                }
                if (!PROOF) {
                    if (PF) asm volatile("s_waitcnt vmcnt(0)" ::: "memory");
                    if (j == 0) {
                        L.cut[2 * q_cur] = r0;
                        L.cut[2 * q_cur + 1] = r1;
                    }
                    if (rec && 8 * j < lstep)
                        *reinterpret_cast<unsigned long long*>(path + (size_t)(m - 1) * CUT_PATH + 8 * j) =
                            *reinterpret_cast<const unsigned long long*>(&pth[g][8 * j]);
#pragma unroll
                    for (int k = 0; k < (PF ? CUT_FAST / 8 : 0); ++k) {
                        const int e = j + 8 * k;
                        fst[g][e] = nxl[e >> 4][16 * g + (e & 15)];
                    }
                }
            }
            wave_lds_sync();
            if (pend) {
                q_cur = q_nx;
                q_nx = lb + (size_t)(int)fst[g][PD_NEXT];
                if (PROOF) m_sync = m;
                first = 1;
                lstep = 0;
                r0 = 0.0;
                r1 = 0.0;
#pragma unroll
                for (int kk = 0; kk < 3; ++kk) {
                    const int e = j + 8 * kk;
                    const int x = CUT_FAST + e;
                    if (e < 21) {
                        const double mid = sumA[g][e] + info[kk];
                        const double nw = mid - (PF ? nxl[x >> 4][16 * g + (x & 15)] : rec_l[(size_t)m * CUT_REC + x]);
                        sumA[g][e] = nw;
                        if (PROOF) sumE[g][e] = mid;
                    }
                }
            }
            wave_lds_sync();
            TCK(0);
            if (pend) {
                open_line();
                if (m + 1 < nls) pf_issue(m + 1);
                pend = 0;
            }
            TCK(1);
            {
                if (!PROOF) partner_done = pslot[0];
                const int done = wave_sum8(j == 0 ? m : 0);
                if (done > __builtin_amdgcn_readfirstlane(partner_done)) __builtin_amdgcn_s_setprio(0);
                else __builtin_amdgcn_s_setprio(2);
                if (lane == 0) __hip_atomic_store(prog.own, done, __ATOMIC_RELAXED, __HIP_MEMORY_SCOPE_AGENT);
                if (PROOF) {
                    partner_done = __hip_atomic_load(prog.partner, __ATOMIC_RELAXED, __HIP_MEMORY_SCOPE_AGENT);
                } else if (lane == 0) {
                    const uint32_t dst = (uint32_t)(uintptr_t)&pslot[0];
                    asm volatile("s_mov_b32 m0, %1\n\tglobal_load_lds_dword %0, off sc1" ::"v"(prog.partner), "s"(dst)
                                 : "memory", "m0");
                }
            }
            TCK(2);
        } else if (pend) {
            ++wait;
        }
        PCK(3);
    }
#ifdef GFPL_CUT_PCLOCK
    if (live && j == 0)
        for (int i = 0; i < 4; ++i) p.scr.dbg[8 * (size_t)b + i] = (int64_t)pk[i];
    if (live && j == 0) {
        for (int i = 0; i < 3; ++i) p.scr.dbg[8 * (size_t)b + 4 + i] = (int64_t)tk[i];
        p.scr.dbg[8 * (size_t)b + 7] = ((int64_t)n_it << 32) | n_tr;
    }
#endif
#undef PCK
#undef TCK0
#undef TCK
    if (live && j == 0) {
        p.scr.bytes[(size_t)STEP_REC * b + 16] = n_steps;
        p.scr.bytes[(size_t)STEP_REC * b + 17] = n_exact;
        p.scr.bytes[(size_t)STEP_REC * b + 19] = n_unb;
#ifdef GFPL_CUT_CLOCK
        const uint64_t t_end = wall_clock64();
        p.scr.bytes[(size_t)STEP_REC * b + 19] = (int64_t)(t_end - t_beg);
        p.scr.dbg[8 * (size_t)b + 0] = (int64_t)t_beg;
        p.scr.dbg[8 * (size_t)b + 1] = (int64_t)t_end;
        p.scr.dbg[8 * (size_t)b + 2] = (int64_t)__builtin_amdgcn_s_getreg((4 << 0) | (0 << 6) | (31 << 11));
        p.scr.dbg[8 * (size_t)b + 3] = (int64_t)__builtin_amdgcn_s_getreg((20 << 0) | (0 << 6) | (31 << 11));
#endif
    }
}

#ifndef CUT_WAVE_MAX_B
#define CUT_WAVE_MAX_B 2048
#endif
__device__ __forceinline__ double readlane_f64(double v, int l) {
    const int lo = __builtin_amdgcn_readlane(__double2loint(v), l);
    const int hi = __builtin_amdgcn_readlane(__double2hiint(v), l);
    return __hiloint2double(hi, lo);
}
__device__ __forceinline__ int nb_da(int j, int side) {
    return nb_off(j, side);
}

__global__ void __launch_bounds__(64) __attribute__((amdgpu_waves_per_eu(2, 2))) k_cut_search_w(KParams p) {
    __shared__ double sumA[25];
    __shared__ double sumE[25];
    __shared__ double fst[CUT_FAST + 1];
    __shared__ double tmp[CUT_G][CUT_EP + 25 + 1];
    __shared__ double wgs[64];
    __shared__ double xsl[16];
    __shared__ CutCmp cmpl;
    __shared__ double dgx[100];
// ... 23 lines not shown
    uint64_t tk[8] = {0, 0, 0, 0, 0, 0, 0, 0};
    uint64_t tk0 = clock64();
#define TCK(i) do { const uint64_t t_ = clock64(); tk[i] += t_ - tk0; tk0 = t_; } while (0)
#else
#define TCK(i) do { } while (0)
#endif
    auto open_line = [&]() {
        double o[28];
        {
            double S[21];
#pragma unroll
            for (int e = 0; e < 21; ++e) S[e] = sumA[e];
            chol_s(S, o);
        }
        TCK(2);
        line_ok = (o[27] != 0.0) && (fst[PD_OK] != 0.0);
        if (lane < 6) {
            double w[6];
#pragma unroll
            for (int i = 0; i < 6; ++i) {
                double u = fst[6 * lane + i];
#pragma unroll
                for (int k = 0; k < i; ++k) u = __builtin_fma(-o[tri(i, k)], w[k], u);
                w[i] = u * o[21 + i];
            }
#pragma unroll
            for (int i = 0; i < 6; ++i) wgs[6 * lane + i] = w[i];
        }
        wave_lds_sync();
        TCK(3);
        if (lane < 21) {
            const int ra = (int)((TRI_ROW >> (3 * lane)) & 7), cb = (int)((TRI_COL >> (3 * lane)) & 7);
            double s = wgs[6 * ra] * wgs[6 * cb];
#pragma unroll
            for (int i = 1; i < 6; ++i) s = __builtin_fma(wgs[6 * ra + i], wgs[6 * cb + i], s);
            wgs[36 + lane] = s;
        }
        wave_lds_sync();
        TCK(4);
        const double* gm = wgs + 36;
        double* cl = reinterpret_cast<double*>(&cmpl);
        double G[21], cv[38];
#pragma unroll
        for (int e = 0; e < 21; ++e) G[e] = gm[e];
#pragma unroll
        for (int i = 0; i < 10; ++i) cv[10 + i] = fst[PD_VS + i];
#pragma unroll
        for (int sd = 0; sd < 2; ++sd) {
            const int a0 = 3 * sd, b2 = a0 + 1, c2 = a0 + 2;
            cv[5 * sd + 0] = G[tri(a0, a0)];
            cv[5 * sd + 1] = 2.0 * G[tri(b2, a0)];
            cv[5 * sd + 2] = __builtin_fma(2.0, G[tri(c2, a0)], G[tri(b2, b2)]);
            cv[5 * sd + 3] = 2.0 * G[tri(c2, b2)];
            cv[5 * sd + 4] = G[tri(c2, c2)];
        }
#pragma unroll
        for (int i = 0; i < 3; ++i) {
#pragma unroll
            for (int k = 0; k < 3; ++k) cv[20 + 3 * i + k] = G[tri(3 + k, i)];
            const double gs = fmax(G[tri(i, i)], 0.0), ge = fmax(G[tri(3 + i, 3 + i)], 0.0);
            cv[32 + i] = gs > 0.0 ? 1.01 * gs * __builtin_amdgcn_rsq(gs) : 0.0;
            cv[35 + i] = ge > 0.0 ? 1.01 * ge * __builtin_amdgcn_rsq(ge) : 0.0;
        }
        {
            const double T = fmax(fabs(rlo), fabs(rhi));
            const double Bs = h2(cv[32], cv[33], cv[34], T), Be = h2(cv[35], cv[36], cv[37], T);
            const double VsA = h4abs(cv + 10, T), VeA = h4abs(cv + 15, T);
            const double Bs2 = Bs * Bs, Be2 = Be * Be;
            cv[29] = __builtin_fma(Bs2 + VsA, Be2 + VeA, Bs2 * Be2);
            cv[30] = VsA;
            cv[31] = VeA;
        }
        if (lane == 0) {
#pragma unroll
            for (int i = 0; i < 38; ++i) cl[i] = cv[i];
        }
        wave_lds_sync();
        TCK(5);
        dc = cut_dcore_p1<false>(cv[0], cv[10], cv[5], cv[15], cv[20], cv[29], cv[30], cv[31], cmpl.eb, tq, c_ok);
        TCK(6);
    };
    if (nls > 0) {
        q_cur = lb + mls[0];
        for (int e = lane; e < CUT_FAST; e += 64) fst[e] = rec_l[e];
        if (lane < 21) {
            const double s0 = p.scr.cut_sum[24 * b + lane];
            sumA[lane] = s0 - rec_l[CUT_FAST + lane];
            sumE[lane] = s0;
        }
        wave_lds_sync();
        open_line();
    }
    double pf_f0 = 0.0, pf_i0 = 0.0;
    int pf_q = 0;
    auto prefetch = [&](int mn) {
        if (mn < nls) {
            int iv = mn;
            asm volatile("" : "+v"(iv));
            const double* rn = rec_l + (size_t)iv * CUT_REC;
            pf_i0 = lane < 21 ? rn[CUT_FAST + lane] : 0.0;
            pf_f0 = rn[lane < CUT_FAST ? lane : 0];
            pf_q = mls[iv];
        }
    };
    prefetch(1);
#ifdef GFPL_CUTW_CLOCK
    uint64_t ck_eval = 0, ck_dec = 0, ck_walk = 0, ck_trans = 0, ck_exact = 0, n_rounds = 0, n_trans = 0;
    uint64_t ck0 = clock64();
#define CUTW_CK(acc) do { const uint64_t ck1 = clock64(); acc += ck1 - ck0; ck0 = ck1; } while (0)
#else
#define CUTW_CK(acc) do { } while (0)
#endif
    while (m < nls) {
        double g0[8], g1[8];
        g0[1] = r0;
        g1[1] = r1;
        g0[0] = r0 + (-st);
        g1[0] = r1 + (-st);
#pragma unroll
        for (int k = 2; k < 8; ++k) { g0[k] = g0[k - 1] + st; g1[k] = g1[k - 1] + st; }
        int inc0 = 0, inc1 = 0;
#pragma unroll
        for (int k = 2; k <= 6; ++k) {
            inc0 |= (__double_as_longlong(g0[k] + (-st)) != __double_as_longlong(g0[k - 1])) ? (1 << k) : 0;
            inc1 |= (__double_as_longlong(g1[k] + (-st)) != __double_as_longlong(g1[k - 1])) ? (1 << k) : 0;
        }
        const int k0 = inc0 ? __builtin_ctz(inc0) : -1, k1 = inc1 ? __builtin_ctz(inc1) : -1;
        int dj_valid = 0, bok = 0;
        double dj = 0.0;
        double t0 = g0[0], t1 = g1[0];
        CutReg cr;
        cut_reg_load(cmpl, cr);
        {
            const int a = lane >> 3, c = lane & 7;
#pragma unroll
            for (int k = 1; k < 8; ++k) { t0 = a == k ? g0[k] : t0; t1 = c == k ? g1[k] : t1; }
            int valid = 1;
            if (t0 + t1 > 1.0) valid = 0;
            if (t0 < rlo || t0 > rhi) valid = 0;
            if (t1 < rlo || t1 > rhi) valid = 0;
            dj_valid = valid;
            dj = cut_dval<false>(cr, t0, t1, tq, bok);
        }
        if (inc0 | inc1) {
            const int a = lane >> 3, c = lane & 7;
            const int k0s = __builtin_amdgcn_readfirstlane(k0), k1s = __builtin_amdgcn_readfirstlane(k1);
            const double h0 = readlane_f64(t0, k0s > 0 ? 8 * k0s : 0) + (-st);
            const double h1 = readlane_f64(t1, k1s > 0 ? k1s : 0) + (-st);
            const bool row = lane < 8, col = lane == 8 || (c == 7 && a >= 1), cor = lane == 16;
            const double u0 = (row || cor) ? h0 : (lane == 8 ? g0[0] : t0);
            const double u1 = row ? t1 : h1;
            int valid = (row && k0s >= 0) || (col && k1s >= 0) || (cor && k0s >= 0 && k1s >= 0);
            if (u0 + u1 > 1.0) valid = 0;
            if (u0 < rlo || u0 > rhi) valid = 0;
            if (u1 < rlo || u1 > rhi) valid = 0;
            int abok = 0;
            const double da = cut_dval<false>(cr, u0, u1, tq, abok);
            if (row | col | cor) {
                const int slot = row ? 82 + lane : (cor ? 98 : 90 + (lane == 8 ? 0 : a));
                dgx[slot] = (valid && da == da) ? da : -__builtin_inf();
                dgf[slot] = abok | (valid << 1) | ((valid && !(da == da)) ? 4 : 0);
            }
        }
        CUTW_CK(ck_eval);
        constexpr int WAVE_EXACT = 16, WAVE_STOP = 32;
        int dec = WAVE_STOP;
        {
            const int a = lane >> 3, c = lane & 7;
            const int bad0 = inc0 & ~(k0 >= 0 ? 1 << k0 : 0), bad1 = inc1 & ~(k1 >= 0 ? 1 << k1 : 0);
            const bool cons = a >= 1 && a <= 6 && c >= 1 && c <= 6 && !((bad0 >> a) & 1) && !((bad1 >> c) & 1);
            const bool ia = a == k0, ic = c == k1;
            const double xo = (dj_valid && dj == dj) ? dj : -__builtin_inf();
            dgx[9 + lane] = xo;
            dgf[9 + lane] = bok | (dj_valid << 1) | ((dj_valid && !(dj == dj)) ? 4 : 0);
            wave_lds_sync();
            double vjn[8];
            int fl[8];
            if (inc0 | inc1) {
#pragma unroll
                for (int jn = 0; jn < 8; ++jn) {
                    const int da = nb_da(jn, 0), dc = nb_da(jn, 1);
                    const bool xa = ia && da < 0, xc = ic && dc < 0;
                    const int l = (xa && xc) ? 82 + 16 : (xa ? 82 + c + dc : (xc ? 90 + a + da : 9 + lane + 8 * da + dc));
                    vjn[jn] = dgx[l];
// ... 95 lines not shown
            const int pa = pos >> 3, pc = pos & 7;
#pragma unroll
            for (int jn = 0; jn < 8; ++jn) {
                const int l = (pa + nb_da(jn, 0)) * 8 + (pc + nb_da(jn, 1));
                vj[jn] = readlane_f64(dj, l);
                bj[jn] = __builtin_amdgcn_readlane(bok, l);
                valj[jn] = __builtin_amdgcn_readlane(dj_valid, l);
            }
        }
        r0 = readlane_f64(t0, pos);
        r1 = readlane_f64(t1, pos);
        CUTW_CK(ck_walk);
#ifdef GFPL_CUTW_CLOCK
        ++n_rounds;
#endif
        if (exact) {
            int myv = 0;
#pragma unroll
            for (int jn = 0; jn < 8; ++jn) myv = lane == jn ? valj[jn] : myv;
            const CutX xr = cut_exact_round(lane < 8, myv, first, m, m_sync, r0, r1, q_cur, lb, -1, mls, rec_l, L.sP,
                                            L.eP, L.covS, L.covE, L.le_obs, L.cut, sumE, tmp[0], &tmp[0][0], Dl,
                                            cam.fx, cam.b, homog, st);
            const int best = __builtin_amdgcn_readfirstlane(xr.best);
            m_sync = __builtin_amdgcn_readfirstlane(xr.m_sync);
            ++n_steps;
            ++n_exact;
            if (rec && lane == 0) {
                if (lstep < CUT_PATH)
                    path[(size_t)m * CUT_PATH + lstep] = (uint8_t)((best >= 0 ? best : CUT_P_STAY) | CUT_P_EXACT);
            }
            ++lstep;
            first = 0;
            if (best < 0) {
                finalize = 1;
            } else {
                double vb = vj[0];
                int bb = bj[0];
#pragma unroll
                for (int jn = 1; jn < 8; ++jn) { vb = best == jn ? vj[jn] : vb; bb = best == jn ? bj[jn] : bb; }
                dc = vb;
                c_ok = bb;
                r0 = r0 + nb_step(best, 0, st);
                r1 = r1 + nb_step(best, 1, st);
                if (!(r0 + r1 <= 1.0)) finalize = 1;
            }
        }
        CUTW_CK(ck_exact);
        if (finalize) {
#ifdef GFPL_CUTW_CLOCK
            ++n_trans;
#endif
#ifdef GFPL_CUTW_TCLOCK
            tk0 = clock64();
#endif
            if (lane == 0) {
                L.cut[2 * q_cur] = r0;
                L.cut[2 * q_cur + 1] = r1;
            }
            double info = 0.0;
            {
                const int ra = (int)((TRI_ROW >> (3 * lane)) & 7), cb = (int)((TRI_COL >> (3 * lane)) & 7);
                if (fst[PD_OK] != 0.0) {
                    if (lane < 21) {
                        const double is = rcp_fast(cut_ours_V(fst, 0, r0)), ie = rcp_fast(cut_ours_V(fst, 1, r1));
                        const double psr = cut_ours_P(fst, 0, ra, r0), psc = cut_ours_P(fst, 0, cb, r0);
                        const double per = cut_ours_P(fst, 1, ra, r1), pec = cut_ours_P(fst, 1, cb, r1);
                        info = __builtin_fma(psr * is, psc, (per * ie) * pec);
                    }
                } else {
                    if (lane < 2) {
                        double o7[7];
                        exact_endpoint(cam, homog, Dl, L, q_cur, lane, lane ? r1 : r0, o7);
#pragma unroll
                        for (int i = 0; i < 7; ++i) xsl[7 * lane + i] = o7[i];
                    }
                    wave_lds_sync();
                    if (lane < 21) info = cut_ours_info(xsl, rcp_fast(xsl[0]), rcp_fast(xsl[7]), ra, cb);
                }
            }
            ++m;
            TCK(0);
            if (m < nls) {
                wave_lds_sync();
                if (lane < CUT_FAST) fst[lane] = pf_f0;
                if (lane < 21) sumA[lane] = (sumA[lane] + info) - pf_i0;
                q_cur = lb + __builtin_amdgcn_readfirstlane(pf_q);
                first = 1;
                lstep = 0;
                r0 = 0.0;
                r1 = 0.0;
                wave_lds_sync();
                TCK(1);
                open_line();
                prefetch(m + 1);
            }
        }
        CUTW_CK(ck_trans);
    }
    if (lane == 0) {
        p.scr.bytes[(size_t)STEP_REC * b + 16] = n_steps;
        p.scr.bytes[(size_t)STEP_REC * b + 17] = n_exact;
        p.scr.bytes[(size_t)STEP_REC * b + 19] = 0;
#ifdef GFPL_CUTW_CLOCK
        int64_t* d = p.scr.dbg + 8 * (size_t)b;
        d[0] = ck_eval; d[1] = ck_dec; d[2] = ck_walk; d[3] = ck_exact; d[4] = ck_trans; d[5] = n_rounds; d[6] = n_trans;
        d[7] = n_steps;
#endif
#ifdef GFPL_CUTW_TCLOCK
        for (int i = 0; i < 7; ++i) p.scr.dbg[8 * (size_t)b + i] = (int64_t)tk[i];
#endif
    }
}

#define CUTE_LN 27
__global__ void __launch_bounds__(64) __attribute__((amdgpu_waves_per_eu(2, 2))) k_cut_search_eig(KParams p) {
    __shared__ double lnd[CUT_G][CUTE_LN];
    __shared__ double dti[CUT_G][17];
    __shared__ double smat[CUT_G][21];
    __shared__ double ninf[CUT_G][8 * 21 + 1];
    const int lane = threadIdx.x;
    const int g = lane >> 3, j = lane & 7;
    const int b = blockIdx.x * CUT_G + g;
    const bool seq = b < p.B;
    const int nls = seq ? p.tr.n_matched_ls[b] : 0;
    const DevCam& cam = p.cam;
    const double homog = p.cfg.homog_th;
    DevLines& L = p.prev.ls;
    const size_t lb = (size_t)(seq ? b : 0) * p.kl_cap;
    const int32_t* mls = p.tr.matched_ls + (size_t)(seq ? b : 0) * p.mls_cap;
    const double* rec_l = p.scr.cut_rec + (size_t)(seq ? b : 0) * p.mls_cap * CUT_REC;
    const double st = p.cfg.cut_step;
    const double rlo = p.cfg.cut_rng[0], rhi = p.cfg.cut_rng[1];
    const double nb0 = nb_step(j, 0, st), nb1 = nb_step(j, 1, st);
    int m = 0;
    int open = 1;
    double r0 = 0.0, r1 = 0.0;
    double mc = 0.0;
    size_t q_cur = 0;
    double se[3] = {0.0, 0.0, 0.0}, ss[3] = {0.0, 0.0, 0.0}, ci[3] = {0.0, 0.0, 0.0};
    int n_steps = 0, n_eval = 0, n_sweeps = 0;
    auto open_line = [&]() {
        q_cur = lb + mls[m];
        for (int i = j; i < 26; i += 8) {
            double v;
            if (i < 3) v = L.sP[3 * q_cur + i];
            else if (i < 6) v = L.eP[3 * q_cur + i - 3];
            else if (i < 15) v = L.covS[9 * q_cur + i - 6];
            else if (i < 24) v = L.covE[9 * q_cur + i - 15];
            else v = L.le_obs[3 * q_cur + i - 24];
            lnd[g][i] = v;
        }
#pragma unroll
        for (int kk = 0; kk < 3; ++kk) {
            const int e = j + 8 * kk;
            if (e < 21) {
                ci[kk] = rec_l[(size_t)m * CUT_REC + CUT_FAST + e];
                ss[kk] = se[kk] - ci[kk];
                smat[g][e] = se[kk];
            }
        }
        r0 = 0.0;
        r1 = 0.0;
        open = 1;
    };
    if (nls > 0) {
        for (int i = j; i < 16; i += 8) dti[g][i] = p.scr.cut_dtinv[16 * (size_t)b + i];
#pragma unroll
        for (int kk = 0; kk < 3; ++kk) {
            const int e = j + 8 * kk;
            if (e < 21) se[kk] = p.scr.cut_sum[24 * (size_t)b + e];
        }
        open_line();
    }
    while (__any(m < nls)) {
        wave_lds_sync();
        const bool live = m < nls;
        const double t0 = r0 + nb0, t1 = r1 + nb1;
        int valid = (live && !open) ? 1 : 0;
        if (t0 + t1 > 1.0) valid = 0;
        if (t0 < rlo || t0 > rhi) valid = 0;
        if (t1 < rlo || t1 > rhi) valid = 0;
        double v = 0.0;
        if (live && (open || valid)) {
            double tot[21];
            if (open) {
#pragma unroll
                for (int e = 0; e < 21; ++e) tot[e] = smat[g][e];
            } else {
                double S7[7], E7[7], info[21];
                const double* d = lnd[g];
                cut_endpoint(cam, homog, dti[g], d + 24, d, d + 3, d + 6, d + 15, t0, S7);
                cut_endpoint(cam, homog, dti[g], d + 24, d + 3, d, d + 15, d + 6, t1, E7);
                cut_assemble<false>(S7, E7, info);
#pragma unroll
                for (int e = 0; e < 21; ++e) {
                    ninf[g][21 * j + e] = info[e];
                    tot[e] = info[e] + smat[g][e];
                }
            }
            double A[36], w[6];
#pragma unroll
            for (int i = 0; i < 6; ++i)
#pragma unroll
                for (int k = 0; k <= i; ++k) {
                    A[i * 6 + k] = tot[tri(i, k)];
                    A[k * 6 + i] = tot[tri(i, k)];
                }
            int sw = 0;
            eig_sym<6, true>(A, w, &sw);
            v = w[0];
            if (!open || j == 0) {
                n_sweeps += sw;
                ++n_eval;
            }
        }
        wave_lds_sync();
        double top;
        const int best = group_first_max(v, valid, j, mc, top);
        if (live && open) {
            mc = v;
            open = 0;
#pragma unroll
            for (int kk = 0; kk < 3; ++kk) {
                const int e = j + 8 * kk;
                if (e < 21) smat[g][e] = ss[kk];
            }
        } else if (live) {
            ++n_steps;
            bool fin = true;
            if (best >= 0) {
#pragma unroll
                for (int kk = 0; kk < 3; ++kk) {
                    const int e = j + 8 * kk;
                    if (e < 21) ci[kk] = ninf[g][21 * best + e];
                }
                r0 = r0 + nb_step(best, 0, st);
                r1 = r1 + nb_step(best, 1, st);
                mc = top;
                fin = !(r0 + r1 <= 1.0);
// ... 23 lines not shown

#ifndef GFPL_FIN_WAVES
#define GFPL_FIN_WAVES 4
#endif
__global__ void __launch_bounds__(64, GFPL_FIN_WAVES) k_cut_finish(KParams p) {
    const int b = blockIdx.x;
    const int nls = p.tr.n_matched_ls[b];
    if (nls == 0) return;
    const bool ends_only = p.cfg.cut_with_max_vol && (p.cfg.cut_proof == 1 || p.cfg.cut_proof == 3) &&
                           p.scr.cut_flag[b] == 0;
    const DevCam& cam = p.cam;
    DevLines& L = p.prev.ls;
    const size_t lb = (size_t)b * p.kl_cap;
    const int32_t* mls = p.tr.matched_ls + (size_t)b * p.mls_cap;
    double Dl[16];
#pragma unroll
    for (int i = 0; i < 16; ++i) Dl[i] = p.scr.cut_dtinv[16 * b + i];
    for (int m0 = 0; m0 < nls; m0 += 64) {
        const int m = m0 + (int)threadIdx.x;
        const bool live = m < nls;
        const size_t q = lb + (live ? mls[m] : 0);
        LineCutData d;
        double r0 = 0.0, r1 = 0.0;
        double info[36];
        if (live && ends_only) {
            load_line(L, q, d);
            r0 = L.cut[2 * q];
            r1 = L.cut[2 * q + 1];
        } else if (live) {
            load_line(L, q, d);
            r0 = L.cut[2 * q];
            r1 = L.cut[2 * q + 1];
            poseInfoOnLine<true>(cam, p.cfg.homog_th, Dl, d, r0, r1, info);
            double2* iv = reinterpret_cast<double2*>(L.invcov + 36 * q);
#pragma unroll
            for (int i = 0; i < 18; ++i) iv[i] = make_double2(info[2 * i], info[2 * i + 1]);
        }
        if (live && !(fabs(r0) < 0.0001 && fabs(r1) < 0.0001)) {
            double sP[3] = {d.sP[0], d.sP[1], d.sP[2]}, eP[3] = {d.eP[0], d.eP[1], d.eP[2]};
            if (fabs(r0) > 0.0001) {
                double s[3];
                for (int k = 0; k < 3; ++k) s[k] = (1 - r0) * sP[k] + r0 * eP[k];
                for (int k = 0; k < 3; ++k) { sP[k] = s[k]; L.sP[3 * q + k] = s[k]; }
                double uv[2];
                projection(cam, sP, uv);
                L.spl[2 * q] = uv[0]; L.spl[2 * q + 1] = uv[1];
                L.sdisp[q] = (cam.fx * cam.b) / sP[2];
            }
            if (fabs(r1) > 0.0001) {
                double e[3];
                for (int k = 0; k < 3; ++k) e[k] = (1 - r1) * eP[k] + r1 * sP[k];
                for (int k = 0; k < 3; ++k) { eP[k] = e[k]; L.eP[3 * q + k] = e[k]; }
                double uv[2];
                projection(cam, eP, uv);
                L.epl[2 * q] = uv[0]; L.epl[2 * q + 1] = uv[1];
                L.edisp[q] = (cam.fx * cam.b) / eP[2];
            }
        }
    }
}

__device__ __forceinline__ double verify_vref(const KParams& p, const double* Dl, size_t q, int side, double t) {
    return ref_vprime(p.cam, p.cfg.homog_th, Dl, p.prev.ls, q, side, t);
}

__device__ __forceinline__ double vref_regs(const DevCam& cam, double homog, const double* Dl, const double* P0,
                                            const double* P1, const double* C0, const double* C1, const double* Jl,
                                            double c) {
    double Pt[3];
#pragma unroll
    for (int k = 0; k < 3; ++k) Pt[k] = (1.0 - c) * P0[k] + c * P1[k];
    const double a = (1.0 - c) * (1.0 - c), qq = c * c;
    double cov[9];
#pragma unroll
    for (int i = 0; i < 9; ++i) cov[i] = a * C0[i] + qq * C1[i];
    const double v = endpointVar_t<double, true>(cam, Dl, Jl, Pt, cov, 0.0);
    double cur[3];
    se3_apply(Dl, Pt, cur);
    const double f = cam.fx / ref_max(homog, cur[2] * cur[2]);
    return v / (f * f);
}

__device__ __forceinline__ void vref_replay(const KParams& p, int b, int m) {
    const double* fd = p.scr.cut_rec + ((size_t)b * p.mls_cap + m) * CUT_REC;
    double* out = p.scr.cut_vmax + ((size_t)b * p.mls_cap + m) * CUT_VMAX;
    const uint8_t* path = p.scr.cut_path + ((size_t)b * p.mls_cap + m) * CUT_PATH;
    const DevLines& L = p.prev.ls;
    const size_t q = (size_t)b * p.kl_cap + p.tr.matched_ls[(size_t)b * p.mls_cap + m];
    const double* Dl = p.scr.cut_dtinv + 16 * (size_t)b;
    const double st = p.cfg.cut_step, rlo = p.cfg.cut_rng[0], rhi = p.cfg.cut_rng[1];
    double sP[3], eP[3], cS[9], cE[9], Jl[2], qs[5], qe[5];
#pragma unroll
    for (int k = 0; k < 3; ++k) { sP[k] = L.sP[3 * q + k]; eP[k] = L.eP[3 * q + k]; }
#pragma unroll
    for (int k = 0; k < 9; ++k) { cS[k] = L.covS[9 * q + k]; cE[k] = L.covE[9 * q + k]; }
    Jl[0] = L.le_obs[3 * q];
    Jl[1] = L.le_obs[3 * q + 1];
#pragma unroll
    for (int k = 0; k < 5; ++k) { qs[k] = fd[PD_VS + k]; qe[k] = fd[PD_VE + k]; }
    double r0 = 0.0, r1 = 0.0;
    bool done = false;
    long long ct0[4] = {-1, -1, -1, -1}, ct1[4] = {-1, -1, -1, -1};
    double cv0[4] = {0, 0, 0, 0}, cv1[4] = {0, 0, 0, 0};
    int slot0 = 0, slot1 = 0;
    double ivm[2] = {0.0, 0.0}, rim[2] = {0.0, 0.0};
    int marg = 0, nbad = 0, nev = 0;
    for (int k = 0; k < CUT_PATH && !done; ++k) {
        const int by = path[k];
        if (!(by & CUT_P_EXACT)) {
            ++marg;
            for (int w = 0; w < 6; ++w) {
                const int side = w >= 3 ? 1 : 0, o = w - 3 * side;
                const double rc = side ? r1 : r0;
                const double t = o == 0 ? rc + (-st) : (o == 2 ? rc + st : rc);
                if (!(t >= rlo && t <= rhi)) continue;
                const long long tb = __double_as_longlong(t);
                double vr = 0.0;
                bool hit = false;
#pragma unroll
                for (int z = 0; z < 4; ++z) {
                    const bool h = side ? ct1[z] == tb : ct0[z] == tb;
                    vr = h ? (side ? cv1[z] : cv0[z]) : vr;
                    hit = hit || h;
                }
                if (!hit) {
                    vr = side ? vref_regs(p.cam, p.cfg.homog_th, Dl, eP, sP, cE, cS, Jl, t)
                              : vref_regs(p.cam, p.cfg.homog_th, Dl, sP, eP, cS, cE, Jl, t);
                    ++nev;
#pragma unroll
                    for (int z = 0; z < 4; ++z) {
                        if (side && slot1 == z) { ct1[z] = tb; cv1[z] = vr; }
                        if (!side && slot0 == z) { ct0[z] = tb; cv0[z] = vr; }
                    }
                    if (side) slot1 = (slot1 + 1) & 3; else slot0 = (slot0 + 1) & 3;
                }
                const double* qc = side ? qe : qs;
                const double vo = __builtin_fma(t, __builtin_fma(t, __builtin_fma(t, __builtin_fma(t, qc[4], qc[3]), qc[2]),
                                                                 qc[1]), qc[0]);
                const double lo = fmin(vr, vo);
                const double rv = fabs(vo - vr) / vr;
                if (!(lo > 0.0 && rv < 0.01)) { ++nbad; continue; }
                const double iv = 1.01 / lo;
                ivm[side] = fmax(ivm[side], iv);
                rim[side] = fmax(rim[side], rv * iv);
            }
        }
        if (by & CUT_P_STAY) {
            done = true;
        } else {
            const int jj = by & 7;
            r0 = r0 + nb_step(jj, 0, st);
            r1 = r1 + nb_step(jj, 1, st);
            if (!(r0 + r1 <= 1.0)) done = true;
        }
    }
    if (!done || __double_as_longlong(r0) != __double_as_longlong(L.cut[2 * q]) ||
        __double_as_longlong(r1) != __double_as_longlong(L.cut[2 * q + 1]))
        nbad += 1 << 20;
    out[0] = ivm[0];
    out[1] = rim[0];
    out[2] = ivm[1];
    out[3] = rim[1];
    out[4] = (double)marg + 1024.0 * (double)nev;
    out[5] = (double)nbad;
}


// ... 25 lines not shown
    int marg = 0, nbad = 0;
    bool off = nk == 0;
    if (on && !off) {
        const uint4* pv = reinterpret_cast<const uint4*>(p.scr.cut_path + ((size_t)b * p.mls_cap + m) * CUT_PATH);
        uint32_t pw[CUT_PATH / 4];
#pragma unroll
        for (int i = 0; i < CUT_PATH / 16; ++i) {
            const uint4 v = pv[i];
            pw[4 * i] = v.x; pw[4 * i + 1] = v.y; pw[4 * i + 2] = v.z; pw[4 * i + 3] = v.w;
        }
        double r[2] = {0.0, 0.0};
        int kc[2] = {0, 0};
        bool done = false;
        for (int k = 0; k < CUT_PATH && !done && !off; ++k) {
            uint32_t wd = pw[0];
#pragma unroll
            for (int i = 1; i < CUT_PATH / 4; ++i) wd = (k >> 2) == i ? pw[i] : wd;
            const int by = (int)((wd >> (8 * (k & 3))) & 255u);
            if (!(by & CUT_P_EXACT)) {
                ++marg;
#pragma unroll
                for (int side = 0; side < 2; ++side) {
#pragma unroll
                    for (int o = 0; o < 3; ++o) {
                        const double t = o == 0 ? r[side] + (-st) : (o == 2 ? r[side] + st : r[side]);
                        if (!(t >= rlo && t <= rhi)) continue;
                        const int kk = kc[side] < 0 ? -1 : (o == 0 ? kpv[kc[side]] : (o == 2 ? knx[kc[side]] : kc[side]));
                        if (kk < 0 || __double_as_longlong(keys[kk]) != __double_as_longlong(t)) { off = true; continue; }
                        mk[side] |= 1u << kk;
                    }
                }
            }
            if (by & CUT_P_STAY) {
                done = true;
            } else {
                const int jj = by & 7;
#pragma unroll
                for (int side = 0; side < 2; ++side) {
                    const double sv = nb_step(jj, side, st);
                    r[side] = r[side] + sv;
                    if (kc[side] >= 0) kc[side] = sv > 0.0 ? knx[kc[side]] : (sv < 0.0 ? kpv[kc[side]] : kc[side]);
                }
                if (!(r[0] + r[1] <= 1.0)) done = true;
            }
        }
        const int qi = p.tr.matched_ls[(size_t)b * p.mls_cap + m];
        qln[lane] = qi;
        const size_t q = (size_t)b * p.kl_cap + qi;
        if (!done || __double_as_longlong(r[0]) != __double_as_longlong(p.prev.ls.cut[2 * q]) ||
            __double_as_longlong(r[1]) != __double_as_longlong(p.prev.ls.cut[2 * q + 1]))
            nbad += 1 << 20;
    }
    if (off) mk[0] = mk[1] = 0u;
    const int cnt = __popc(mk[0]) + __popc(mk[1]);
    int inc = cnt;
#pragma unroll
    for (int o = 1; o < 64; o <<= 1) {
        const int v = __shfl_up(inc, o);
        if (lane >= o) inc += v;
    }
    const int total = __shfl(inc, 63);
    {
        int w = inc - cnt;
#pragma unroll
        for (int side = 0; side < 2; ++side) {
            uint32_t x = mk[side];
            while (x) {
                const int kk = __ffs(x) - 1;
                x &= x - 1u;
                items[w++] = (uint16_t)((lane << 6) | (side << 5) | kk);
            }
        }
    }
    wave_lds_sync();
    const DevLines& L = p.prev.ls;
    const double* Dl = p.scr.cut_dtinv + 16 * (size_t)b;
    for (int i0 = 0; i0 < total; i0 += 64) {
        const int i = i0 + lane;
        if (i < total) {
            const int it = items[i];
            const int ln = it >> 6, side = (it >> 5) & 1, kk = it & 31;
            const int mm = blockIdx.x * 64 + ln;
            const size_t q = (size_t)b * p.kl_cap + qln[ln];
            const double* fd = p.scr.cut_rec + ((size_t)b * p.mls_cap + mm) * CUT_REC;
            double P0[3], P1[3], C0[9], C1[9], Jl[2], qc[5];
            const double* A3 = side ? L.eP : L.sP;
            const double* B3 = side ? L.sP : L.eP;
            const double* A9 = side ? L.covE : L.covS;
            const double* B9 = side ? L.covS : L.covE;
#pragma unroll
            for (int k = 0; k < 3; ++k) { P0[k] = A3[3 * q + k]; P1[k] = B3[3 * q + k]; }
#pragma unroll
            for (int k = 0; k < 9; ++k) { C0[k] = A9[9 * q + k]; C1[k] = B9[9 * q + k]; }
            Jl[0] = L.le_obs[3 * q];
            Jl[1] = L.le_obs[3 * q + 1];
#pragma unroll
            for (int k = 0; k < 5; ++k) qc[k] = fd[(side ? PD_VE : PD_VS) + k];
            const double t = keys[kk];
            const double vr = vref_regs(p.cam, p.cfg.homog_th, Dl, P0, P1, C0, C1, Jl, t);
            const double vo = __builtin_fma(t, __builtin_fma(t, __builtin_fma(t, __builtin_fma(t, qc[4], qc[3]), qc[2]),
                                                             qc[1]), qc[0]);
            const double lo = fmin(vr, vo);
            const double rv = fabs(vo - vr) / vr;
            if (!(lo > 0.0 && rv < 0.01)) {
                atomicAdd(&nbl[ln], 1);
            } else {
                const double iv = 1.01 / lo;
                atomicMax(&red[2 * side][ln], (unsigned long long)__double_as_longlong(iv));
                atomicMax(&red[2 * side + 1][ln], (unsigned long long)__double_as_longlong(rv * iv));
            }
        }
    }
    wave_lds_sync();
    if (!on) return;
    double* out = p.scr.cut_vmax + ((size_t)b * p.mls_cap + m) * CUT_VMAX;
    if (off) {
        const int slot = atomicAdd(p.scr.cut_offl, 1);
        p.scr.cut_offl[1 + slot] = b * p.mls_cap + m;
        return;
    }
#pragma unroll
    for (int i = 0; i < 4; ++i) out[i] = __longlong_as_double((long long)red[i][lane]);
    out[4] = (double)marg + 1024.0 * (double)cnt;
    out[5] = (double)(nbad + nbl[lane]);
}

__global__ void __launch_bounds__(64) k_cut_vref_off(KParams p) {
    const int n = p.scr.cut_offl[0];
    for (int i = blockIdx.x * 64 + threadIdx.x; i < n; i += gridDim.x * 64) {
        const int e = p.scr.cut_offl[1 + i];
        vref_replay(p, e / p.mls_cap, e % p.mls_cap);
    }
}

__global__ void __launch_bounds__(64) k_cut_ebound(KParams p) {
    const int b = blockIdx.y;
    const int m = blockIdx.x * 64 + threadIdx.x;
    if (m >= p.tr.n_matched_ls[b]) return;
    const double* fd = p.scr.cut_rec + ((size_t)b * p.mls_cap + m) * CUT_REC;
    if (fd[PD_OK] == 0.0) return;
    const size_t q = (size_t)b * p.kl_cap + p.tr.matched_ls[(size_t)b * p.mls_cap + m];
    double Dl[16];
#pragma unroll
    for (int i = 0; i < 16; ++i) Dl[i] = p.scr.cut_dtinv[16 * b + i];
    float eb[14];
    cut_line_bounds_p(p, q, true, Dl, eb);
    float* o = reinterpret_cast<float*>(p.scr.cut_vmax + ((size_t)b * p.mls_cap + m) * CUT_VMAX + 6);
#pragma unroll
    for (int i = 0; i < 14; ++i) o[i] = eb[i];
}

__device__ __attribute__((noinline)) int verify_exact_step(const KParams& p, const double* Dl, size_t q, double r0,
                                                           double r1, int first, const double* Sref, const double* Sfull,
                                                           int recorded) {
    const double st = p.cfg.cut_step, rlo = p.cfg.cut_rng[0], rhi = p.cfg.cut_rng[1];
    double ep[6][7];
#pragma unroll
    for (int j = 0; j < 6; ++j) {
        const int side = j < 3 ? 0 : 1;
        const double eoff = (j % 3) == 0 ? -st : ((j % 3) == 2 ? st : 0.0);
        exact_endpoint(p.cam, p.cfg.homog_th, Dl, p.prev.ls, q, side, (side == 0 ? r0 : r1) + eoff, ep[j]);
    }
    double tot[21], tmp[21];
    double mc;
    if (first) {
#pragma unroll
        for (int i = 0; i < 21; ++i) tot[i] = Sfull[i];
    } else {
        cut_assemble<false>(ep[1], ep[4], tmp);
#pragma unroll
        for (int i = 0; i < 21; ++i) tot[i] = tmp[i] + Sref[i];
    }
    mc = logdet6_lower(tot);
    double mx = -__builtin_inf();
    int best = -1;
    for (int jn = 0; jn < 8; ++jn) {
        const double t0 = r0 + nb_step(jn, 0, st), t1 = r1 + nb_step(jn, 1, st);
        if (t0 + t1 > 1.0 || t0 < rlo || t0 > rhi || t1 < rlo || t1 > rhi) continue;
        cut_assemble<false>(ep[nb_slot(jn, 0)], ep[3 + nb_slot(jn, 1)], tmp);
#pragma unroll
        for (int i = 0; i < 21; ++i) tot[i] = tmp[i] + Sref[i];
        const double v = logdet6_lower(tot);
        if (v == v && v > mx) { mx = v; best = jn; }
    }
    const int ref = (best >= 0 && mx > mc) ? best : CUT_P_STAY;
    return ref == recorded ? 1 : 0;
}

__device__ __attribute__((noinline)) int verify_line_detail(const KParams& p, const double* Dl, size_t q,
                                                            const uint8_t* path_m, const double* fd, double r0f,
                                                            double r1f, double K0, double A1, double B1, double cs,
                                                            double ce, double R0, double rts, double rte, bool line_ok,
                                                            const double* Scol, int sstride, int& n_xchk) {
    const double st = p.cfg.cut_step, rlo = p.cfg.cut_rng[0], rhi = p.cfg.cut_rng[1];
    const bool pdok = fd[PD_OK] != 0.0;
    int bad = 0;
    {
            double r0 = 0.0, r1 = 0.0;
            bool done = false;
            int first = 1;
            double ct[2][4], cv[2][4];
            int cn[2] = {0, 0};
            for (int k = 0; k < CUT_PATH && !done; ++k) {
                const int by = path_m[k];
                if (!(by & CUT_P_EXACT)) {
                    double ivm[2] = {0.0, 0.0}, rim[2] = {0.0, 0.0};
                    bool vok = pdok;
                    for (int w = 0; w < 6 && vok; ++w) {
                        const int side = w / 3, o = w % 3;
                        const double rc = side ? r1 : r0;
                        const double t = o == 0 ? rc + (-st) : (o == 2 ? rc + st : rc);
                        if (!(t >= rlo && t <= rhi)) continue;
                        double vr = 0.0;
                        bool hit = false;
                        for (int z = 0; z < cn[side]; ++z)
                            if (__double_as_longlong(ct[side][z]) == __double_as_longlong(t)) { vr = cv[side][z]; hit = true; }
                        if (!hit) {
                            vr = verify_vref(p, Dl, q, side, t);
                            const int z = cn[side] < 4 ? cn[side]++ : (k & 3);
                            ct[side][z] = t;
                            cv[side][z] = vr;
                        }
                        const double vo = cut_ours_V(fd, side, t);
                        const double lo = fmin(vr, vo);
                        const double rv = fabs(vo - vr) / vr;
                        if (!(lo > 0.0 && rv < 0.01)) { vok = false; continue; }
                        const double iv = 1.01 / lo;
                        ivm[side] = fmax(ivm[side], iv);
                        rim[side] = fmax(rim[side], (1.01 * rv + (side ? rte : rts)) * iv);
                    }
                    const double E = K0 + A1 * ivm[0] + cs * rim[0] + B1 * ivm[1] + ce * rim[1];
                    if (!(vok && line_ok && E * 1.0001 <= R0)) {
                        double Sref[21], Sfull[21];
#pragma unroll
                        for (int e = 0; e < 21; ++e) { Sfull[e] = Scol[sstride * e]; Sref[e] = Sfull[e] - fd[CUT_FAST + e]; }
                        ++n_xchk;
                        if (!verify_exact_step(p, Dl, q, r0, r1, first, Sref, Sfull, (by & CUT_P_STAY) ? CUT_P_STAY : (by & 7)))
                            bad |= 512;
                    }
                }
                first = 0;
                if (by & CUT_P_STAY) {
                    done = true;
                } else {
                    const int jj = by & 7;
                    r0 = r0 + nb_step(jj, 0, st);
                    r1 = r1 + nb_step(jj, 1, st);
                    if (!(r0 + r1 <= 1.0)) done = true;
                }
            }
            if (!done || __double_as_longlong(r0) != __double_as_longlong(r0f) ||
                __double_as_longlong(r1) != __double_as_longlong(r1f))
                bad |= 1;
        }
    return bad;
}

struct LineBound {
    double K0, A1, B1, cs, ce, R0, rts, rte, epsS, kt;
    int ok;
};
__device__ __forceinline__ LineBound verify_line_bound(const KParams& p, size_t q, const double* fd, const double* vmx,
                                                      const double* Dl, const double* So, const double* Sf) {
    const double rlo = p.cfg.cut_rng[0], rhi = p.cfg.cut_rng[1];
    const double T = fmax(fabs(rlo), fabs(rhi));
    const double tau = p.cfg.cut_certify;
    constexpr double u = 0x1p-53;
    LineBound lbd;
    double K0, A1, B1, cs, ce, R0, rts, rte, epsS_l, kt_l;
    bool line_ok;
        float eb[14];
        {
            const float* ebg = reinterpret_cast<const float*>(vmx + 6);
#pragma unroll
            for (int i = 0; i < 14; ++i) eb[i] = ebg[i];
        }
        double o28[28];
        {
            double S[21];
#pragma unroll
            for (int e = 0; e < 21; ++e) S[e] = So[65 * e];
            chol_s(S, o28);
        }
        double sg[6];
#pragma unroll
        for (int j = 0; j < 6; ++j) {
            double x[6], a = 0.0;
#pragma unroll
            for (int i = 0; i < 6; ++i) {
                double uu = i == j ? 1.0 : 0.0;
#pragma unroll
                for (int k = 0; k < i; ++k) uu = uu - o28[tri(i, k)] * x[k];
                x[i] = uu * o28[21 + i];
                a = a + x[i] * x[i];
            }
            sg[j] = 1.002 * a;
        }
        double Bn[2] = {0.0, 0.0};
#pragma unroll
        for (int side = 0; side < 2; ++side) {
            double tk = 1.0;
#pragma unroll
            for (int kk = 0; kk < 3; ++kk) {
                double w[6], a = 0.0;
#pragma unroll
                for (int i = 0; i < 6; ++i) {
                    double uu = fd[(side ? PD_PE : PD_PS) + 6 * kk + i];
#pragma unroll
                    for (int k = 0; k < i; ++k) uu = uu - o28[tri(i, k)] * w[k];
                    w[i] = uu * o28[21 + i];
                    a = a + w[i] * w[i];
                }
                Bn[side] = Bn[side] + 1.01 * sqrt(a) * tk;
                tk = tk * T;
            }
        }
        double Kc = 0.0, xi = 0.0, Qs = 0.0, Qe = 0.0, hs0 = 0.0, he0 = 0.0, Lam = 0.0, dSn = 0.0;
#pragma unroll
        for (int i = 0; i < 6; ++i) {
            const double Sii = So[65 * tri(i, i)];
            const double es = eb[i], ee = eb[7 + i];
            const double ps = fabs(fd[PD_PS + i]) + T * (fabs(fd[PD_PS + 6 + i]) + T * fabs(fd[PD_PS + 12 + i])) + es;
            const double pe = fabs(fd[PD_PE + i]) + T * (fabs(fd[PD_PE + 6 + i]) + T * fabs(fd[PD_PE + 12 + i])) + ee;
            const double kc = Sii * sg[i];
            Kc = Kc + kc;
            xi = xi + sqrt(kc);
            Qs = Qs + sg[i] * ps * ps;
            Qe = Qe + sg[i] * pe * pe;
            hs0 = hs0 + es * sqrt(sg[i]);
            he0 = he0 + ee * sqrt(sg[i]);
            Lam = Lam + ((Sii > 0.0 && Sii < 1e300) ? 0.6931471805599453 * (double)(abs(__builtin_amdgcn_frexp_exp(Sii)) + 1)
                                                     : __builtin_inf());
#pragma unroll
            for (int k = 0; k < 6; ++k) {
                const int e = tri(i > k ? i : k, i > k ? k : i);
                const double sref = Sf[65 * e] - fd[CUT_FAST + e];
                const double dd = 1.0000000000000004 * fabs(So[65 * e] - sref);
                dSn = dSn + dd * sqrt(sg[i] * sg[k]);
            }
        }
        const double epsS = 1.01 * dSn + (7.01 * u) * xi * xi;
        const double hs = hs0 + (6.01 * u) * Bn[0] * xi, he = he0 + (6.01 * u) * Bn[1] * xi;
        const double ck = 110.0 * u;
        K0 = 1.002 * epsS + ck * Kc + (7.1 * u) * Lam;
        const double bs = Bn[0] + hs, be = Bn[1] + he;
        rts = 4.1 * (double)eb[6] + 16.0 * u;
        rte = 4.1 * (double)eb[13] + 16.0 * u;
        A1 = 1.03 * (2.0 * ck * Qs + 4.0 * hs * bs);
        B1 = 1.03 * (2.0 * ck * Qe + 4.0 * he * be);
        cs = 4.12 * bs * bs;
        ce = 4.12 * be * be;
        R0 = fmin(0.125 * tau, 1e-3) - 1.01 * K0;
        line_ok = o28[27] != 0.0 && epsS <= 1e-3 && Kc <= 1e8 && R0 > 0.0 && rlo >= 0.0 && rhi <= 1.0 &&
                  tau > 0.0 && rts + rte <= 0.01;
        epsS_l = 1.002 * epsS;
        kt_l = ck * Kc + (7.1 * u) * Lam;

    lbd.K0 = K0; lbd.A1 = A1; lbd.B1 = B1; lbd.cs = cs; lbd.ce = ce; lbd.R0 = R0; lbd.rts = rts; lbd.rte = rte;
    lbd.epsS = epsS_l; lbd.kt = kt_l; lbd.ok = line_ok ? 1 : 0;
    return lbd;
}

__global__ void __launch_bounds__(64) __attribute__((amdgpu_waves_per_eu(2, 2))) k_cut_verify(KParams p) {
    __shared__ double fo[21][65];
    __shared__ double fr[21][65];
    const int b = blockIdx.x;
    const int lane = threadIdx.x;
    const int nls = p.tr.n_matched_ls[b];
    const DevCam& cam = p.cam;
    const double homog = p.cfg.homog_th;
    DevLines& L = p.prev.ls;
    const size_t lb = (size_t)b * p.kl_cap;
    const int32_t* mls = p.tr.matched_ls + (size_t)b * p.mls_cap;
    const double* rec_l = p.scr.cut_rec + (size_t)b * p.mls_cap * CUT_REC;
    double Dl[16];
#pragma unroll
    for (int i = 0; i < 16; ++i) Dl[i] = p.scr.cut_dtinv[16 * b + i];
    int bad = p.cfg.cut_proof == 3 ? 256 : 0;
    double worst = 0.0;
    double tS = 0.0, tK = 0.0, tA = 0.0, tV = 0.0;
    int64_t n_marg = 0, n_eval = 0, n_mline = 0, n_xchk = 0, n_dline = 0;
    double sA = 0.0, sE = 0.0;
    if (nls > 0 && lane < 21) {
        const double s0 = p.scr.cut_sum[24 * b + lane];
        sA = s0 - rec_l[CUT_FAST + lane];
        sE = s0;
    }
#ifdef GFPL_VERIFY_CLOCK
    uint64_t vk[5] = {0, 0, 0, 0, 0};
    uint64_t vk0 = clock64();
#define VK(i) do { const uint64_t vk1 = clock64(); vk[i] += vk1 - vk0; vk0 = vk1; } while (0)
#else
#define VK(i) do { } while (0)
#endif
    for (int c0 = 0; c0 < nls; c0 += 64) {
        const int m = c0 + lane;
        const bool on = m < nls;
        const size_t q = lb + (on ? mls[m] : mls[0]);
        const double* fd = rec_l + (size_t)(on ? m : 0) * CUT_REC;
        const double r0f = L.cut[2 * q], r1f = L.cut[2 * q + 1];
        {
            LineCutData d;
            load_line(L, q, d);
            double info[36];
            poseInfoOnLine<true>(cam, homog, Dl, d, r0f, r1f, info);
            if (on) {
                double2* iv = reinterpret_cast<double2*>(L.invcov + 36 * q);
#pragma unroll
                for (int i = 0; i < 18; ++i) iv[i] = make_double2(info[2 * i], info[2 * i + 1]);
#pragma unroll
                for (int i = 0; i < 6; ++i)
#pragma unroll
                    for (int k = 0; k <= i; ++k) fr[tri(i, k)][lane] = info[i * 6 + k];
            }
        }
        VK(0);
        const bool pdok = fd[PD_OK] != 0.0;
        {
            double xs[14];
            if (pdok) {
                xs[0] = cut_ours_V(fd, 0, r0f);
                xs[7] = cut_ours_V(fd, 1, r1f);
#pragma unroll
                for (int i = 0; i < 6; ++i) { xs[1 + i] = cut_ours_P(fd, 0, i, r0f); xs[8 + i] = cut_ours_P(fd, 1, i, r1f); }
            } else {
                exact_endpoint(cam, homog, Dl, L, q, 0, r0f, xs);
                exact_endpoint(cam, homog, Dl, L, q, 1, r1f, xs + 7);
            }
            const double is = rcp_fast(xs[0]), ie = rcp_fast(xs[7]);
            if (on) {
#pragma unroll
                for (int i = 0; i < 6; ++i)
#pragma unroll
                    for (int k = 0; k <= i; ++k) fo[tri(i, k)][lane] = cut_ours_info(xs, is, ie, i, k);
            }
        }
        wave_lds_sync();
        VK(1);
        const int cnt = min(64, nls - c0);
        if (lane < 21) {
            auto fetch = [&](int l0, double* v) {
#pragma unroll
                for (int k = 0; k < 17; ++k) {
                    const int mm = c0 + l0 + k;
                    v[k] = (l0 + k <= cnt && mm < nls) ? rec_l[(size_t)mm * CUT_REC + CUT_FAST + lane] : 0.0;
                }
            };
            double iv[17];
            for (int l0 = 0; l0 < cnt; l0 += 16) {
                fetch(l0, iv);
#pragma unroll
                for (int k = 0; k < 16; ++k) {
                    const int l = l0 + k;
                    if (l < cnt) {
                        const double sref = sE - iv[k];
                        const double f_o = fo[lane][l], f_r = fr[lane][l];
                        fo[lane][l] = sA;
                        fr[lane][l] = sE;
                        sE = sref + f_r;
                        sA = (sA + f_o) - iv[k + 1];
                    }
                }
            }
        }
        wave_lds_sync();
        VK(2);
        double K0 = 0.0, A1 = 0.0, B1 = 0.0, cs = 0.0, ce = 0.0, R0 = -1.0, rts = 0.0, rte = 0.0;
        double epsS_l = 0.0, kt_l = 0.0;
        bool line_ok = false;
        if (on && pdok) {
            const LineBound lbd = verify_line_bound(p, q, fd, p.scr.cut_vmax + ((size_t)b * p.mls_cap + m) * CUT_VMAX, Dl,
                                                    &fo[0][0] + lane, &fr[0][0] + lane);
            K0 = lbd.K0; A1 = lbd.A1; B1 = lbd.B1; cs = lbd.cs; ce = lbd.ce; R0 = lbd.R0; rts = lbd.rts; rte = lbd.rte;
            epsS_l = lbd.epsS; kt_l = lbd.kt; line_ok = lbd.ok != 0;
        }
        VK(3);
        int marg = 0;
        bool detail = false;
        if (on) {
            const double* vm = p.scr.cut_vmax + ((size_t)b * p.mls_cap + m) * CUT_VMAX;
            const double mv = vm[4];
            marg = (int)fmod(mv, 1024.0);
            n_eval += (int64_t)(mv / 1024.0);
            if (marg) {
                const double E = K0 + A1 * vm[0] + cs * (1.01 * vm[1] + rts * vm[0]) + B1 * vm[2] +
                                 ce * (1.01 * vm[3] + rte * vm[2]);
                detail = !(vm[5] == 0.0 && line_ok && E * 1.0001 <= R0);
                if (!detail && E / R0 > worst) {
                    worst = E / R0;
                    tS = epsS_l / R0;
                    tK = kt_l / R0;
                    tA = (A1 * vm[0] + B1 * vm[2]) / R0;
                    tV = (cs * (1.01 * vm[1] + rts * vm[0]) + ce * (1.01 * vm[3] + rte * vm[2])) / R0;
                }
            }
            n_marg += marg;
            n_mline += marg ? 1 : 0;
            n_dline += detail ? 1 : 0;
        }
        VK(4);
        if (detail) {
            const int slot = atomicAdd(p.scr.cut_dtln, 1);
            if (slot < CUT_DTL * p.B) {
                double* e = p.scr.cut_dtl + (size_t)slot * 32;
#pragma unroll
                for (int i = 0; i < 21; ++i) e[i] = fr[i][lane];
                e[21] = K0; e[22] = A1; e[23] = B1; e[24] = cs; e[25] = ce; e[26] = R0; e[27] = rts; e[28] = rte;
                e[29] = line_ok ? 1.0 : 0.0;
                p.scr.cut_dtln[1 + slot] = b * p.mls_cap + m;
            } else {
                bad |= 1024;
            }
        }
        wave_lds_sync();
    }
    int mask = bad;
    int wl = lane;
#pragma unroll
    for (int o = 32; o > 0; o >>= 1) {
        mask |= __shfl_xor(mask, o);
        const double ow = __shfl_xor(worst, o);
        const int ol = __shfl_xor(wl, o);
        if (ow > worst || (ow == worst && ol < wl)) { worst = ow; wl = ol; }
    }
    tS = __shfl(tS, wl); tK = __shfl(tK, wl); tA = __shfl(tA, wl); tV = __shfl(tV, wl);
    bad = mask != 0 ? 1 : 0;
#pragma unroll
    for (int o = 32; o > 0; o >>= 1) {
        n_marg += __shfl_xor(n_marg, o);
        n_eval += __shfl_xor(n_eval, o);
        n_mline += __shfl_xor(n_mline, o);
        n_xchk += __shfl_xor(n_xchk, o);
        n_dline += __shfl_xor(n_dline, o);
    }
    if (lane == 0) {
        p.scr.cut_flag[b] = bad;
        p.scr.bytes[(size_t)STEP_REC * b + 20] = bad;
        p.scr.bytes[(size_t)STEP_REC * b + 21] = n_marg;
        p.scr.bytes[(size_t)STEP_REC * b + 22] = n_eval;
        p.scr.bytes[(size_t)STEP_REC * b + 23] = n_mline;
        p.scr.dbg[8 * (size_t)b + 4] = mask;
        p.scr.dbg[8 * (size_t)b + 5] = __double_as_longlong(worst);
        p.scr.dbg[8 * (size_t)b + 6] = n_xchk;
        p.scr.dbg[8 * (size_t)b + 7] = n_dline;
        p.scr.dbg[8 * (size_t)b + 0] = __double_as_longlong(tS);
        p.scr.dbg[8 * (size_t)b + 1] = __double_as_longlong(tK);
        p.scr.dbg[8 * (size_t)b + 2] = __double_as_longlong(tA);
        p.scr.dbg[8 * (size_t)b + 3] = __double_as_longlong(tV);
#ifdef GFPL_VERIFY_CLOCK
        for (int i = 0; i < 5; ++i) p.scr.dbg[8 * (size_t)b + i] = (int64_t)vk[i];
#endif
    }
}

__global__ void __launch_bounds__(64) k_cut_verify_detail(KParams p) {
    const int n = min(p.scr.cut_dtln[0], CUT_DTL * p.B);
    for (int i = blockIdx.x * 64 + threadIdx.x; i < n; i += gridDim.x * 64) {
        const int e = p.scr.cut_dtln[1 + i];
        const int b = e / p.mls_cap, m = e % p.mls_cap;
        const double* pl = p.scr.cut_dtl + (size_t)i * 32;
        const size_t q = (size_t)b * p.kl_cap + p.tr.matched_ls[(size_t)b * p.mls_cap + m];
        const double* fd = p.scr.cut_rec + ((size_t)b * p.mls_cap + m) * CUT_REC;
        const uint8_t* path = p.scr.cut_path + ((size_t)b * p.mls_cap + m) * CUT_PATH;
        double Dl[16];
#pragma unroll
        for (int k = 0; k < 16; ++k) Dl[k] = p.scr.cut_dtinv[16 * b + k];
        int nx = 0;
        const int bad = verify_line_detail(p, Dl, q, path, fd, p.prev.ls.cut[2 * q], p.prev.ls.cut[2 * q + 1], pl[21],
                                           pl[22], pl[23], pl[24], pl[25], pl[26], pl[27], pl[28], pl[29] != 0.0, pl, 1,
                                           nx);
        if (bad) {
            atomicOr(&p.scr.cut_flag[b], 1);
            atomicOr(reinterpret_cast<unsigned long long*>(&p.scr.bytes[(size_t)STEP_REC * b + 20]), 1ull);
        }
        if (nx) atomicAdd(reinterpret_cast<unsigned long long*>(&p.scr.dbg[8 * (size_t)b + 6]), (unsigned long long)nx);
    }
}

static int cut_wave_max_b() {
    const char* e = getenv("GFPL_CUT_WAVE_MAX_B");
    return e ? atoi(e) : CUT_WAVE_MAX_B;
}

static int cut_prep_w8_max_b() {
    const char* e = getenv("GFPL_CUT_PREP_W8_MAX_B");
    return e ? atoi(e) : 256;
}

hipError_t launch_line_cut(const KParams& p, hipStream_t s, const hipEvent_t* marks) {
    const int mode = p.cfg.cut_proof;
    const dim3 gsearch((p.B + CUT_G - 1) / CUT_G);
    if (p.B <= cut_prep_w8_max_b()) {
        static std::atomic<unsigned long long> attr{0};
        const hipError_t e = ensure_dyn_lds(reinterpret_cast<const void*>(k_cut_prep<8>), (int)cut_prep_lds(8), &attr);
        if (e != hipSuccess) return e;
        hipLaunchKernelGGL(k_cut_prep<8>, dim3(p.B), dim3(512), cut_prep_lds(8), s, p);
    } else {
        hipLaunchKernelGGL(k_cut_prep<1>, dim3(p.B), dim3(64), cut_prep_lds(1), s, p);
    }
    if (!p.cfg.cut_with_max_vol) {
        if (marks) (void)hipEventRecord(marks[0], s);
        hipLaunchKernelGGL(k_cut_search_eig, gsearch, dim3(64), 0, s, p);
        if (marks) (void)hipEventRecord(marks[1], s);
        hipLaunchKernelGGL(k_cut_finish, dim3(p.B), dim3(64), 0, s, p);
        return hipGetLastError();
    }
    if (mode == 2) {
        hipLaunchKernelGGL(k_cut_bounds, dim3((p.mls_cap + 63) / 64, p.B), dim3(64), 0, s, p);
        hipLaunchKernelGGL(k_cut_vtab, dim3(p.B), dim3(256), 0, s, p);
    }
    if (marks) (void)hipEventRecord(marks[0], s);
    if (mode == 2)
        hipLaunchKernelGGL(k_cut_search<true>, gsearch, dim3(64), 0, s, p);
    else if (p.B <= cut_wave_max_b())
        hipLaunchKernelGGL(k_cut_search_w, dim3(p.B), dim3(64), 0, s, p);
    else if (mode == 1 || mode == 3)
        hipLaunchKernelGGL(HIP_KERNEL_NAME(k_cut_search<false, true>), gsearch, dim3(64), 0, s, p);
    else
        hipLaunchKernelGGL(k_cut_search<false>, gsearch, dim3(64), 0, s, p);
    if (marks) (void)hipEventRecord(marks[1], s);
    if (mode == 1 || mode == 3) {
        if (hipMemsetAsync(p.scr.cut_offl, 0, sizeof(int32_t), s) != hipSuccess) return hipGetLastError();
        hipLaunchKernelGGL(k_cut_vref, dim3((p.mls_cap + 63) / 64, p.B), dim3(64), 0, s, p);
        hipLaunchKernelGGL(k_cut_vref_off, dim3(256), dim3(64), 0, s, p);
        hipLaunchKernelGGL(k_cut_ebound, dim3((p.mls_cap + 63) / 64, p.B), dim3(64), 0, s, p);
        if (hipMemsetAsync(p.scr.cut_dtln, 0, sizeof(int32_t), s) != hipSuccess) return hipGetLastError();
        hipLaunchKernelGGL(k_cut_verify, dim3(p.B), dim3(64), 0, s, p);
        hipLaunchKernelGGL(k_cut_verify_detail, dim3(256), dim3(64), 0, s, p);
        hipLaunchKernelGGL(k_cut_bounds, dim3((p.mls_cap + 63) / 64, p.B), dim3(64), 0, s, p);
        hipLaunchKernelGGL(k_cut_vtab, dim3(p.B), dim3(256), 0, s, p);
        hipLaunchKernelGGL(k_cut_search<true>, gsearch, dim3(64), 0, s, p);
    }
    hipLaunchKernelGGL(k_cut_finish, dim3(p.B), dim3(64), 0, s, p);
    return hipGetLastError();
}

}
```

gf-pl-slam_amd/gfpl/__init__.py:

```python
from __future__ import annotations

import ctypes as C
import json
import os
from typing import Optional

import numpy as np

PKG_DIR = os.path.dirname(os.path.dirname(os.path.abspath(__file__)))
LIB_DIR = os.path.join(PKG_DIR, "lib")
REPO_DIR = os.path.dirname(PKG_DIR)

DESC = 32
MAX_LEVELS = 8
MAX_MATCHED_PT = 2048
MAX_MATCHED_LS = 1024
PREV, CURR = 0, 1
HAMMING, HAMMING2 = 1, 2

ERRORS = {0: "ok", -1: "invalid argument", -2: "HIP runtime error", -3: "no HIP device",
          -4: "knn-2 needs at least 2 train descriptors", -5: "capacity exceeded",
          -6: "call order violated", -7: "unsupported config", -8: "device memory allocation failed"}


class GfplError(RuntimeError):
    def __init__(self, code: int, what: str = ""):
        super().__init__(f"{what}: gfpl error {code} ({ERRORS.get(code, '?')})")
        self.code = code


class Camera(C.Structure):
    _fields_ = [("width", C.c_int), ("height", C.c_int),
                ("fx", C.c_double), ("fy", C.c_double), ("cx", C.c_double), ("cy", C.c_double),
                ("b", C.c_double), ("n_levels", C.c_int),
                ("scale", C.c_float * MAX_LEVELS), ("inv_scale", C.c_float * MAX_LEVELS),
                ("lvl_cols", C.c_int * MAX_LEVELS), ("lvl_rows", C.c_int * MAX_LEVELS),
                ("lvl_offset", C.c_int64 * MAX_LEVELS), ("pyr_bytes", C.c_int64),
                ("sigma2_pt", C.c_double * MAX_LEVELS), ("sigma2_ln", C.c_double * MAX_LEVELS)]


class Config(C.Structure):
    _fields_ = [("best_lr_matches", C.c_int), ("lr_in_parallel", C.c_int),
                ("use_line_conf_cut", C.c_int), ("cut_with_max_vol", C.c_int),
                ("ratio_disp_std", C.c_double), ("ratio_disp_std_hor", C.c_double),
                ("max_line_match_num", C.c_int), ("max_point_match_num", C.c_int),
                ("max_dist_epip", C.c_double), ("min_disp", C.c_double),
                ("max_ratio_12_p", C.c_double), ("point_match_radius", C.c_double),
                ("stereo_overlap_th", C.c_double), ("line_horiz_th", C.c_double),
                ("desc_th_l", C.c_double), ("line_cov_th", C.c_double),
                ("homog_th", C.c_double), ("min_features", C.c_int),
                ("max_iters", C.c_int), ("max_iters_ref", C.c_int),
                ("min_error", C.c_double), ("min_error_change", C.c_double),
                ("inlier_k", C.c_double), ("motion_step_th", C.c_double),
                ("orb_scale_factor", C.c_double), ("orb_n_levels", C.c_int),
                ("lsd_scale", C.c_double), ("cut_step", C.c_double),
                ("cut_rng", C.c_double * 2), ("proj_gate_px", C.c_double),
                ("min_entropy_ratio", C.c_double), ("max_kf_num_frames", C.c_int),
                ("cut_certify", C.c_double), ("cut_proof", C.c_int)]


KEYPOINT_DT = np.dtype([("x", "<f4"), ("y", "<f4"), ("octave", "<i4")])
CV_KEYPOINT_DT = np.dtype([("x", "<f4"), ("y", "<f4"), ("size", "<f4"), ("angle", "<f4"),
                           ("response", "<f4"), ("octave", "<i4")])
KEYLINE_DT = np.dtype([("sx", "<f4"), ("sy", "<f4"), ("ex", "<f4"), ("ey", "<f4"),
                       ("angle", "<f4"), ("octave", "<i4")])

_vp = C.c_void_p


class Frames(C.Structure):
    _fields_ = [("batch", C.c_int), ("kp_cap", C.c_int), ("kl_cap", C.c_int),
                ("n_kp_l", _vp), ("n_kp_r", _vp), ("kp_l", _vp), ("kp_r", _vp),
                ("pdesc_l", _vp), ("pdesc_r", _vp),
                ("n_kl_l", _vp), ("n_kl_r", _vp), ("kl_l", _vp), ("kl_r", _vp),
                ("ldesc_l", _vp), ("ldesc_r", _vp), ("pyr_r", _vp), ("time_stamp", _vp),
                ("ready", _vp), ("consumed", _vp)]


PT_FIELDS = [("pt_pl", np.float64, (2,)), ("pt_pl_obs", np.float64, (2,)),
             ("pt_disp", np.float64, ()), ("pt_P", np.float64, (3,)),
             ("pt_sigma2", np.float64, ()), ("pt_idx", np.int32, ()),
             ("pt_level", np.int32, ()), ("pt_inlier", np.uint8, ()),
             ("pdesc", np.uint8, (DESC,))]
LS_FIELDS = [("ls_spl", np.float64, (2,)), ("ls_epl", np.float64, (2,)),
             ("ls_spl_obs", np.float64, (2,)), ("ls_epl_obs", np.float64, (2,)),
             ("ls_sdisp", np.float64, ()), ("ls_edisp", np.float64, ()),
             ("ls_sdisp_obs", np.float64, ()), ("ls_edisp_obs", np.float64, ()),
             ("ls_angle", np.float64, ()), ("ls_sigma2", np.float64, ()),
             ("ls_sP", np.float64, (3,)), ("ls_eP", np.float64, (3,)),
             ("ls_le", np.float64, (3,)), ("ls_le_obs", np.float64, (3,)),
             ("ls_covS", np.float64, (9,)), ("ls_covE", np.float64, (9,)),
             ("ls_cut", np.float64, (2,)), ("ls_invcov", np.float64, (36,)),
             ("ls_idx", np.int32, ()), ("ls_level", np.int32, ()),
             ("ls_inlier", np.uint8, ()), ("ldesc", np.uint8, (DESC,))]
POSE_FIELDS = [("Tfw", 16), ("DT", 16), ("DT_cov", 36), ("Tfw_cov", 36), ("DT_cov_eig", 6)]


class FrameHostStruct(C.Structure):
    _fields_ = ([("n_pt", C.c_int), ("n_ls", C.c_int)]
# ... 155 lines not shown
        if not os.path.exists(p):
            raise GfplError(-3, f"{p} is not built (run __graft_entry__.build())")
        _LIBS[name] = C.CDLL(p)
    return _LIBS[name]


def hiplib() -> C.CDLL:
    if "libgfpl_hip.so" not in _LIBS:
        try:
            import torch
        except Exception:
            pass
    L = _load("libgfpl_hip.so")
    if not getattr(L, "_gfpl_typed", False):
        P = C.c_void_p
        sigs = {
            "gfpl_abi_version": ([], C.c_int),
            "gfpl_config_default": ([P], C.c_int),
            "gfpl_camera_init": ([P, C.c_int, C.c_int, C.c_double, C.c_double, C.c_double,
                                  C.c_double, C.c_double, P], C.c_int),
            "gfpl_create": ([C.c_int, P, C.POINTER(P)], C.c_int),
            "gfpl_create_async": ([C.c_int, C.POINTER(P)], C.c_int),
            "gfpl_get_stream": ([P], C.c_void_p),
            "gfpl_event_create": ([P, C.POINTER(P)], C.c_int),
            "gfpl_event_destroy": ([P], C.c_int),
            "gfpl_event_record": ([P, P], C.c_int),
            "gfpl_event_wait": ([P, P], C.c_int),
            "gfpl_event_synchronize": ([P], C.c_int),
            "gfpl_event_record_count": ([P, P], C.c_int),
            "gfpl_orb_extract_async": ([P, P, C.c_int, P, P, P, P, P, P, C.c_int64], C.c_int),
            "gfpl_orb_status": ([P], C.c_int),
            "gfpl_lsd_detect_async": ([P, P, C.c_int, P, P, P], C.c_int),
            "gfpl_lsd_status": ([P], C.c_int),
            "gfpl_lbd_compute_async": ([P, P, C.c_int, P, P, P], C.c_int),
            "gfpl_lbd_status": ([P], C.c_int),
            "gfpl_destroy": ([P], C.c_int),
            "gfpl_set_camera": ([P, P], C.c_int),
            "gfpl_set_config": ([P, P], C.c_int),
            "gfpl_get_camera": ([P, P], C.c_int),
            "gfpl_get_config": ([P, P], C.c_int),
            "gfpl_synchronize": ([P], C.c_int),
            "gfpl_copy_to_host": ([P, P, P, C.c_size_t], C.c_int),
            "gfpl_seqbatch_create": ([P, C.c_int, C.c_int, C.c_int, C.POINTER(P)], C.c_int),
            "gfpl_seqbatch_destroy": ([P], C.c_int),
            "gfpl_seqbatch_bytes": ([P], C.c_int64),
            "gfpl_initialize": ([P, P], C.c_int),
            "gfpl_insert_stereo_pair": ([P, P], C.c_int),
            "gfpl_optimize_pose": ([P], C.c_int),
            "gfpl_optimize_pose_ini": ([P, P], C.c_int),
            "gfpl_update_frame": ([P], C.c_int),
            "gfpl_frame_step": ([P, P], C.c_int),
            "gfpl_upload_frames": ([P, P, P], C.c_int),
            "gfpl_upload_frames_async": ([P, P, C.c_int, C.c_int, P], C.c_int),
            "gfpl_upload_wait": ([P, C.c_int64], C.c_int),
            "gfpl_upload_frames_l0_async": ([P, P, C.c_int, C.c_int, C.c_int64, P], C.c_int),
            "gfpl_staged_frames": ([P, C.c_int, P], C.c_int),
            "gfpl_stereo_points": ([P, P], C.c_int),
            "gfpl_stereo_lines": ([P, P], C.c_int),
            "gfpl_line_uncertainty": ([P], C.c_int),
            "gfpl_cross_points": ([P], C.c_int),
            "gfpl_cross_lines": ([P], C.c_int),
            "gfpl_line_cut": ([P], C.c_int),
            "gfpl_knn2_hamming": ([P, P, C.c_int, P, C.c_int, C.c_int, P, P], C.c_int),
            "gfpl_kf_common_matches": ([P, P, P, P, P, P, P], C.c_int),
            "gfpl_kf_local_map_matches": ([P, P, P, C.c_double, C.c_double, P, P, P, P], C.c_int),
            "gfpl_read_frame": ([P, C.c_int, C.c_int, P], C.c_int),
            "gfpl_write_frame": ([P, C.c_int, C.c_int, P], C.c_int),
            "gfpl_read_track": ([P, C.c_int, P], C.c_int),
            "gfpl_read_last_track": ([P, C.c_int, P], C.c_int),
            "gfpl_need_new_kf": ([P, P], C.c_int),
            "gfpl_curr_frame_is_kf": ([P, P], C.c_int),
            "gfpl_read_kf_state": ([P, C.c_int, P], C.c_int),
            "gfpl_write_track": ([P, C.c_int, P], C.c_int),
            "gfpl_set_timing": ([P, C.c_int], C.c_int),
            "gfpl_get_stage_times": ([P, P], C.c_int),
            "gfpl_get_kernel_times": ([P, P], C.c_int),
            "gfpl_last_step_kernel_bytes": ([P, P], C.c_int),
            "gfpl_last_step_bytes": ([P, P], C.c_int),
            "gfpl_last_step_stage_bytes": ([P, P], C.c_int),
            "gfpl_last_step_counts": ([P, P], C.c_int),
            "gfpl_last_step_track_counts": ([P, P], C.c_int),
            "gfpl_last_step_cut_proof": ([P, P], C.c_int),
            "gfpl_debug_cut_records": ([P, C.c_int, P, C.c_int], C.c_int),
            "gfpl_debug_step_records": ([P, P], C.c_int),
            "gfpl_debug_clocks": ([P, P], C.c_int),
            "gfpl_lsd_create": ([P, P, C.c_int, C.c_int, C.c_int, C.c_int, C.c_int, C.POINTER(P)], C.c_int),
            "gfpl_lsd_destroy": ([P], C.c_int),
            "gfpl_lsd_detect": ([P, P, C.c_int, P, P, P], C.c_int),
            "gfpl_lsd_sort_desc": ([P, P, C.c_int], C.c_int),
            "gfpl_strerror": ([C.c_int], C.c_char_p),
            "gfpl_orb_create": ([P, C.c_int, C.c_int, P, C.c_int, C.c_int, C.POINTER(P)], C.c_int),
            "gfpl_orb_destroy": ([P], C.c_int),
            "gfpl_orb_pyramid_bytes": ([P, P], C.c_int),
            "gfpl_orb_extract": ([P, P, C.c_int, P, P, P, P, P, P, C.c_int64], C.c_int),
            "gfpl_lbd_create": ([P, C.c_int, C.c_int, C.c_int, C.c_int, C.POINTER(P)], C.c_int),
            "gfpl_lbd_destroy": ([P], C.c_int),
            "gfpl_lbd_compute": ([P, P, C.c_int, P, P, P], C.c_int),
            "gfpl_lbd_gradients": ([P, P, P], C.c_int),
            "gfpl_detector_params_default": ([P, P, P], C.c_int),
            "gfpl_detector_create": ([P, P, C.c_int, C.c_int, C.c_int, C.c_int, C.POINTER(P)], C.c_int),
            "gfpl_detector_destroy": ([P], C.c_int),
            "gfpl_detect_stereo_async": ([P, P, P, C.c_int, P, P], C.c_int),
            "gfpl_detect_stereo_host": ([P, P, P, C.c_int, P, P], C.c_int),
            "gfpl_detect_stereo": ([P, P, P, C.c_int, P, C.c_int, P], C.c_int),
            "gfpl_detector_status": ([P], C.c_int),
            "gfpl_detector_discard": ([P, P], C.c_int),
            "gfpl_read_detections": ([P, P, C.c_int, P], C.c_int),
            "gfpl_rectify_maps_host": ([P, C.c_int, C.c_int, P, P], C.c_int),
            "gfpl_rectifier_create": ([P, P, P, C.c_int, C.c_int, C.POINTER(P)], C.c_int),
            "gfpl_rectifier_destroy": ([P], C.c_int),
            "gfpl_rectifier_read_maps": ([P, C.c_int, P, P], C.c_int),
            "gfpl_rectify": ([P, C.c_int, P, C.c_int, P], C.c_int),
            "gfpl_rectify_async": ([P, C.c_int, P, C.c_int, P], C.c_int),
            "gfpl_rectify_stereo_async": ([P, P, P, C.c_int, P, P], C.c_int),
            "gfpl_rectify_host": ([P, C.c_int, P, C.c_int, P], C.c_int),
            "gfpl_detector_set_rectifier": ([P, P], C.c_int),
        }
        for n, (a, r) in sigs.items():
            try:
                f = getattr(L, n)
            except AttributeError:
                continue
            f.argtypes = a
            f.restype = r
        L._gfpl_typed = True
    return L


def synthlib() -> C.CDLL:
    L = _load("libgfpl_synth.so")
    if not getattr(L, "_gfpl_typed", False):
        P = C.c_void_p
        L.gfpl_synth_default.argtypes = [P]
        L.gfpl_synth_default.restype = None
        L.gfpl_synth_batch.argtypes = ([P, P, C.c_int, C.c_int, C.c_int, C.c_int, C.c_int, C.c_int]
                                       + [P] * 14 + [C.c_int])
        L.gfpl_synth_batch.restype = C.c_int
        L.gfpl_synth_image.argtypes = [C.c_uint64, C.c_int, C.c_int, C.c_int, C.c_int, P]
        L.gfpl_synth_image.restype = C.c_int
        L.gfpl_synth_frame_ex.argtypes = [P, P, C.c_int, C.c_int, C.c_int, C.c_int] + [P] * 16
        L.gfpl_synth_frame_ex.restype = C.c_int
        L._gfpl_typed = True
    return L


def check(code: int, what: str = "") -> None:
    if code != 0:
        raise GfplError(code, what)


def default_config(**over) -> Config:
    cfg = Config()
    check(hiplib().gfpl_config_default(C.byref(cfg)), "config_default")
    for k, v in over.items():
        setattr(cfg, k, v)
    return cfg


CAMERAS = {
    "vga": dict(width=640, height=480, fx=554.25626, fy=554.25626, cx=320.0, cy=240.0, b=0.1),
    "euroc": dict(width=752, height=480, fx=458.654, fy=457.296, cx=367.215, cy=248.375, b=0.110077842),
    "kitti": dict(width=1241, height=376, fx=718.856, fy=718.856, cx=607.1928, cy=185.2157, b=0.537165719),
    "stress": dict(width=1920, height=1080, fx=1662.76878, fy=1662.76878, cx=960.0, cy=540.0, b=0.1),
}


# ... 440 lines not shown
        t = C.c_int64()
        if l0_stride > 0:
            check(self.L.gfpl_upload_frames_l0_async(self.h, C.byref(host), s0, slot, l0_stride, C.byref(t)),
                  "upload_frames_l0_async")
        else:
            check(self.L.gfpl_upload_frames_async(self.h, C.byref(host), s0, slot, C.byref(t)), "upload_frames_async")
        return t.value

    def upload_wait(self, ticket: int):
        check(self.L.gfpl_upload_wait(self.h, ticket), "upload_wait")

    def staged_frames(self, slot: int) -> Frames:
        dev = Frames()
        check(self.L.gfpl_staged_frames(self.h, slot, C.byref(dev)), "staged_frames")
        return dev

    def read_frame(self, which: int, seq: int) -> FrameHost:
        fh = FrameHost(self.kp_cap, self.kl_cap)
        check(self.L.gfpl_read_frame(self.h, which, seq, fh.ptr()), "read_frame")
        return fh

    def write_frame(self, which: int, seq: int, fh: FrameHost):
        check(self.L.gfpl_write_frame(self.h, which, seq, fh.ptr()), "write_frame")

    def read_track(self, seq: int) -> dict:
        t = TrackHost()
        check(self.L.gfpl_read_track(self.h, seq, C.byref(t)), "read_track")
        return t.as_dict()

    def read_last_track(self, seq: int) -> dict:
        t = TrackHost()
        check(self.L.gfpl_read_last_track(self.h, seq, C.byref(t)), "read_last_track")
        return t.as_dict()

    def needNewKF(self) -> np.ndarray:
        flags = np.zeros(self.B, np.int32)
        check(self.L.gfpl_need_new_kf(self.h, flags.ctypes.data), "need_new_kf")
        return flags.astype(bool)

    def currFrameIsKF(self, mask=None):
        if mask is None:
            check(self.L.gfpl_curr_frame_is_kf(self.h, None), "curr_frame_is_kf")
            return
        m = np.ascontiguousarray(np.broadcast_to(np.asarray(mask), (self.B,)), dtype=np.int32)
        check(self.L.gfpl_curr_frame_is_kf(self.h, m.ctypes.data), "curr_frame_is_kf")

    def read_kf_state(self, seq: int) -> dict:
        st = KFState()
        check(self.L.gfpl_read_kf_state(self.h, seq, C.byref(st)), "read_kf_state")
        return st.as_dict()

    def write_track(self, seq: int, tr: TrackHost):
        check(self.L.gfpl_write_track(self.h, seq, C.byref(tr)), "write_track")

    def last_step_bytes(self) -> int:
        v = C.c_int64()
        check(self.L.gfpl_last_step_bytes(self.h, C.byref(v)), "last_step_bytes")
        return v.value

    def last_step_stage_bytes(self) -> np.ndarray:
        v = np.zeros(7, np.int64)
        check(self.L.gfpl_last_step_stage_bytes(self.h, v.ctypes.data), "last_step_stage_bytes")
        return v

    STEP_COUNTS = ["N_o", "N_k", "M_o", "S_p", "S_l", "M_p", "M_l", "n_inliers"]

    def last_step_counts(self) -> dict:
        v = np.zeros(8, np.int64)
        check(self.L.gfpl_last_step_counts(self.h, v.ctypes.data), "last_step_counts")
        return {n: float(x) / self.B for n, x in zip(self.STEP_COUNTS, v)}

    def last_step_track_counts(self) -> dict:
        v = np.zeros(4, np.int64)
        check(self.L.gfpl_last_step_track_counts(self.h, v.ctypes.data), "last_step_track_counts")
        return {"steps": int(v[0]), "exact_steps": int(v[1]), "inliers_after_pose": int(v[2]),
                "lines_unbounded": int(v[3])}

    def last_step_cut_proof(self) -> dict:
        v = np.zeros(4, np.int64)
        check(self.L.gfpl_last_step_cut_proof(self.h, v.ctypes.data), "last_step_cut_proof")
        return {"redone": int(v[0]), "steps_proven": int(v[1]), "vref_evals": int(v[2]), "lines": int(v[3])}

    def debug_cut_records(self, b: int, n_lines: int) -> np.ndarray:
        out = np.zeros((n_lines, 80), np.float64)
        check(self.L.gfpl_debug_cut_records(self.h, b, out.ctypes.data, n_lines), "debug_cut_records")
        return out

    def debug_step_records(self) -> np.ndarray:
        out = np.zeros((self.B, 24), np.int64)
        check(self.L.gfpl_debug_step_records(self.h, out.ctypes.data), "debug_step_records")
        return out

    def debug_clocks(self) -> np.ndarray:
        out = np.zeros((self.B, 8), np.int64)
        check(self.L.gfpl_debug_clocks(self.h, out.ctypes.data), "debug_clocks")
        return out

    def last_step_kernel_bytes(self) -> np.ndarray:
        v = np.zeros(4, np.int64)
        check(self.L.gfpl_last_step_kernel_bytes(self.h, v.ctypes.data), "last_step_kernel_bytes")
        return v

    def nbytes(self) -> int:
        return int(self.L.gfpl_seqbatch_bytes(self.h))

    def close(self):
        if getattr(self, "h", None):
            self.L.gfpl_seqbatch_destroy(self.h)
            self.h = None

    def __del__(self):
        try:
            self.close()
        except Exception:
            pass


def track_from_dict(d: dict) -> TrackHost:
    t = TrackHost()
    t.n_matched_pt = len(d["matched_pt"])
    t.n_matched_ls = len(d["matched_ls"])
    for i, v in enumerate(d["matched_pt"]):
        t.matched_pt[i] = int(v)
    for i, v in enumerate(d["matched_ls"]):
        t.matched_ls[i] = int(v)
    t.n_inliers, t.n_inliers_pt, t.n_inliers_ls = d["n_inliers"], d["n_inliers_pt"], d["n_inliers_ls"]
    t.num_frame_loss = d["num_frame_loss"]
    return t


class ORBextractor:

    def __init__(self, nfeatures: int, scaleFactor: float, nlevels: int, iniThFAST: int, minThFAST: int,
                 width: int, height: int, max_images: int = 1, kp_cap: Optional[int] = None,
                 ctx: Optional[Context] = None, device: int = 0):
        self.L = hiplib()
        self.prm = OrbParams(nfeatures, scaleFactor, nlevels, iniThFAST, minThFAST)
        self.width, self.height, self.max_images = width, height, max_images
        self.kp_cap = kp_cap or nfeatures + 64 * nlevels + 64
        self._own = None
        if ctx is None:
            h = C.c_void_p()
            check(self.L.gfpl_create(device, None, C.byref(h)), "gfpl_create")
            self._own = h
            ch = h
        else:
            ch = ctx.h
        self._ctx = ctx
        o = C.c_void_p()
        check(self.L.gfpl_orb_create(ch, width, height, C.byref(self.prm), max_images, self.kp_cap, C.byref(o)),
              "orb_create")
        self.h = o
        b = C.c_int64()
        check(self.L.gfpl_orb_pyramid_bytes(o, C.byref(b)), "orb_pyramid_bytes")
        self.pyramid_bytes = b.value
        sc = [1.0]
        for _ in range(1, nlevels):
            sc.append(float(np.float32(sc[-1]) * np.float32(scaleFactor)))
        self.mvScaleFactor = np.array(sc, np.float32)
        self.mvLevelSigma2 = self.mvScaleFactor * self.mvScaleFactor
        self.mvInvScaleFactor = np.float32(1.0) / self.mvScaleFactor
        self.mvInvLevelSigma2 = np.float32(1.0) / self.mvLevelSigma2
        self.mvImagePyramid = []

    def GetLevels(self) -> int: return self.prm.nlevels
    def GetScaleFactor(self) -> float: return float(np.float32(self.prm.scale_factor))
    def GetScaleFactors(self): return self.mvScaleFactor.copy()
    def GetInverseScaleFactors(self): return self.mvInvScaleFactor.copy()
# ... 320 lines not shown
```

include/gfpl.h:

```cpp
#ifndef GFPL_H
#define GFPL_H

#include <stddef.h>
#include <stdint.h>

#ifdef __cplusplus
extern "C" {
#endif

#define GFPL_ABI_VERSION 6

#define GFPL_DESC_BYTES 32
#define GFPL_MAX_LEVELS 8
#define GFPL_MAX_IMAGE_DIM 2047
#define GFPL_MAX_MATCHED_PT 2048
#define GFPL_MAX_MATCHED_LS 1024
#define GFPL_PYR_TAIL 64

#define GFPL_OK                   0
#define GFPL_E_INVALID          (-1)
#define GFPL_E_HIP              (-2)
#define GFPL_E_NO_DEVICE        (-3)
#define GFPL_E_TOO_FEW_TRAIN    (-4)
#define GFPL_E_CAPACITY         (-5)
// ... 269 lines not shown
                              const double* time_stamp, gfpl_frames* out);
int  gfpl_detect_stereo_host(gfpl_detector* det, const uint8_t* img_l, const uint8_t* img_r, int n,
                             const double* time_stamp, gfpl_frames* out);
int  gfpl_detector_status(gfpl_detector* det);
int  gfpl_detect_stereo(gfpl_detector* det, const uint8_t* img_l, const uint8_t* img_r, int n,
                        const double* time_stamp, int host_pointers, gfpl_frames* out);
int  gfpl_detector_discard(gfpl_detector* det, const gfpl_frames* view);

typedef struct gfpl_detections_host {
    int n_kp_l, n_kp_r, n_kl_l, n_kl_r;
    gfpl_keypoint* kp_l;  gfpl_keypoint* kp_r;
    uint8_t* pdesc_l;     uint8_t* pdesc_r;
    gfpl_keyline* kl_l;   gfpl_keyline* kl_r;
    uint8_t* ldesc_l;     uint8_t* ldesc_r;
} gfpl_detections_host;
int  gfpl_read_detections(gfpl_ctx* ctx, const gfpl_frames* view, int seq, gfpl_detections_host* out);

typedef struct gfpl_rectify_side {
    int    model;
    double K[4];
    double D[8]; int n_dist;
    double R[9];
    double P[4];
} gfpl_rectify_side;
int  gfpl_rectify_maps_host(const gfpl_rectify_side* s, int width, int height,
                            int16_t* map1 , uint16_t* map2 );
typedef struct gfpl_rectifier gfpl_rectifier;
int  gfpl_rectifier_create(gfpl_ctx* ctx, const gfpl_rectify_side* left, const gfpl_rectify_side* right,
                           int width, int height, gfpl_rectifier** out);
int  gfpl_rectifier_destroy(gfpl_rectifier* r);
int  gfpl_rectifier_read_maps(gfpl_rectifier* r, int side, int16_t* map1, uint16_t* map2);
int  gfpl_rectify(gfpl_rectifier* r, int side, const uint8_t* src, int n, uint8_t* dst);
int  gfpl_rectify_async(gfpl_rectifier* r, int side, const uint8_t* src, int n, uint8_t* dst);
int  gfpl_rectify_stereo_async(gfpl_rectifier* r, const uint8_t* src_l, const uint8_t* src_r, int n,
                               uint8_t* dst_l, uint8_t* dst_r);
int  gfpl_rectify_host(gfpl_rectifier* r, int side, const uint8_t* src, int n, uint8_t* dst);
int  gfpl_detector_set_rectifier(gfpl_detector* det, gfpl_rectifier* r);

typedef struct gfpl_kf_view {
    int            n_pt;
    const uint8_t* pdesc;
    const double*  P;
    const double*  pl;
    const double*  pt_sigma2;
    int            n_ls;
    const uint8_t* ldesc;
    const double*  sP;
    const double*  eP;
    const double*  le;
    const double*  ls_sigma2;
    double         T_kf_w[16];
} gfpl_kf_view;

int  gfpl_kf_common_matches(gfpl_ctx* ctx, const gfpl_kf_view* kf0, const gfpl_kf_view* kf1,
                            int32_t* pt_pairs, int* n_pt_pairs, int32_t* ls_pairs, int* n_ls_pairs);

typedef struct gfpl_map_view {
    int            n_pt;
    const uint8_t* pdesc;
    const double*  P;
    int            n_ls;
    const uint8_t* ldesc;
    const double*  L;
} gfpl_map_view;

int  gfpl_kf_local_map_matches(gfpl_ctx* ctx, const gfpl_map_view* map, const gfpl_kf_view* kf1,
                               double max_kf_epip_p, double max_kf_epip_l,
                               int32_t* pt_pairs, int* n_pt_pairs, int32_t* ls_pairs, int* n_ls_pairs);

int  gfpl_read_frame(gfpl_seqbatch* sb, int which, int seq, gfpl_frame_host* out);
int  gfpl_write_frame(gfpl_seqbatch* sb, int which, int seq, const gfpl_frame_host* in);
int  gfpl_read_track(gfpl_seqbatch* sb, int seq, gfpl_track_host* out);
int  gfpl_write_track(gfpl_seqbatch* sb, int seq, const gfpl_track_host* in);
int  gfpl_read_last_track(gfpl_seqbatch* sb, int seq, gfpl_track_host* out);

int  gfpl_set_timing(gfpl_ctx* ctx, int enable);
int  gfpl_get_stage_times(gfpl_ctx* ctx, float* ms7);
int  gfpl_last_step_bytes(gfpl_seqbatch* sb, int64_t* bytes);
int  gfpl_last_step_stage_bytes(gfpl_seqbatch* sb, int64_t* bytes7);
int  gfpl_last_step_counts(gfpl_seqbatch* sb, int64_t* counts8);
int  gfpl_last_step_track_counts(gfpl_seqbatch* sb, int64_t* counts4);
int  gfpl_last_step_cut_proof(gfpl_seqbatch* sb, int64_t* counts4);
int  gfpl_debug_cut_records(gfpl_seqbatch* sb, int b, double* out, int n_lines);
int  gfpl_debug_step_records(gfpl_seqbatch* sb, int64_t* out);
int  gfpl_debug_clocks(gfpl_seqbatch* sb, int64_t* out);
int  gfpl_get_kernel_times(gfpl_ctx* ctx, float* ms4);
int  gfpl_last_step_kernel_bytes(gfpl_seqbatch* sb, int64_t* bytes4);

const char* gfpl_strerror(int code);

#ifdef __cplusplus
}
#endif
#endif
```

Measured before the change: 802,200.

## Compact per-line cut record from 80 to 64 doubles, moving error bounds aside

The per-line cut record is repacked from 640 B to 512 B. The error-bound floats move into a separate cut_err buffer, and six structurally zero/derived polynomial coefficients are replaced by info entries plus packed float seeds that are re-expanded on load. The hot cut kernel's prefetch drops from five to four 128-B global-to-LDS loads per line, which reduces memory traffic. In exchange, reads now need index remapping and reconstruction logic, and the stored seeds are rounded to float precision.

```diff
diff --git a/gf-pl-slam_amd/csrc/gfpl_abi.hip b/gf-pl-slam_amd/csrc/gfpl_abi.hip
--- a/gf-pl-slam_amd/csrc/gfpl_abi.hip
+++ b/gf-pl-slam_amd/csrc/gfpl_abi.hip
@@ -139,6 +139,7 @@
     sb->tr.kf_nsince = c.take<int32_t>(B);
     sb->tr.kf_flag = c.take<int32_t>(B);
     sb->scr.cut_rec = c.take<double>(B * sb->mls_cap * CUT_REC);
+    sb->scr.cut_err = c.take<double>(B * sb->mls_cap * CUT_ERR);
     sb->scr.knn = c.take<int32_t>(B * 2 * (size_t)sb->kp_cap * 3);
     sb->scr.proj = reinterpret_cast<double*>(sb->scr.knn);
     sb->scr.bytes = c.take<int64_t>(B * STEP_REC);
@@ -1203,7 +1204,7 @@
     int e = step_rec_sums(sb, v);
     if (e) return e;
     const bool cut = sb->last_cut_mode >= 0;
-    bytes4[0] = cut ? 212 * v[14] + 44 * v[13] + 552 * (int64_t)sb->B : 0;
+    bytes4[0] = cut ? (212 + 8 * CUT_REC) * v[14] + 44 * v[13] + 552 * (int64_t)sb->B : 0;
     bytes4[1] = v[7];
     bytes4[2] = cut ? 612 * v[14] : 0;
     bytes4[3] = v[5];
@@ -1256,6 +1257,15 @@
                      hipMemcpyDeviceToHost) == hipSuccess ? GFPL_OK : GFPL_E_HIP;
 }
 
+int gfpl_debug_cut_bounds(gfpl_seqbatch* sb, int b, double* out, int n_lines) {
+    if (!sb || !out || b < 0 || b >= sb->B || n_lines < 0 || n_lines > sb->mls_cap) return GFPL_E_INVALID;
+    if (hipSetDevice(sb->ctx->device) != hipSuccess) return GFPL_E_HIP;
+    if (hipStreamSynchronize(sb->ctx->stream) != hipSuccess) return GFPL_E_HIP;
+    const size_t n = (size_t)n_lines * CUT_ERR;
+    return hipMemcpy(out, sb->scr.cut_err + (size_t)b * sb->mls_cap * CUT_ERR, n * sizeof(double),
+                     hipMemcpyDeviceToHost) == hipSuccess ? GFPL_OK : GFPL_E_HIP;
+}
+
 int gfpl_debug_step_records(gfpl_seqbatch* sb, int64_t* out) {
     if (!sb || !out) return GFPL_E_INVALID;
     if (hipSetDevice(sb->ctx->device) != hipSuccess) return GFPL_E_HIP;
diff --git a/gf-pl-slam_amd/csrc/gfpl_state.hpp b/gf-pl-slam_amd/csrc/gfpl_state.hpp
--- a/gf-pl-slam_amd/csrc/gfpl_state.hpp
+++ b/gf-pl-slam_amd/csrc/gfpl_state.hpp
@@ -72,10 +72,12 @@
 #define CUT_P_EXACT 16
 #define CUT_KS 22
 #define CUT_FAST 56
-#define CUT_REC 80
+#define CUT_REC 64
+#define CUT_ERR 12
 
 struct DevScratch {
     double* cut_rec;
+    double* cut_err;
     int32_t* knn;
     double* proj;
     int64_t* bytes;
diff --git a/gf-pl-slam_amd/csrc/k_cut.hip b/gf-pl-slam_amd/csrc/k_cut.hip
--- a/gf-pl-slam_amd/csrc/k_cut.hip
+++ b/gf-pl-slam_amd/csrc/k_cut.hip
@@ -138,6 +138,48 @@
 #define PD_NEXT 47
 #define PD_ERR 48
 static_assert(CUT_FAST == 56, "per-line comparison data layout");
+#define RS_INFO 48
+#define RS_Z (PD_PE + 14)
+static_assert(CUT_REC * 8 % 128 == 0, "a record is a whole number of 128-B lines");
+static_assert(RS_INFO == PD_ERR && RS_INFO + 16 == CUT_REC,
+              "record fields: comparison data (48, six of them info and seeds) | info (16), none overlapping");
+__host__ __device__ constexpr int cut_rec_structural(int x) {
+    return (x >= PD_PS + 12 && x < PD_PS + 15) ? x - (PD_PS + 12) : ((x >= PD_PE + 12 && x < PD_PE + 15) ? x - (PD_PE + 12) : -1);
+}
+__host__ __device__ constexpr int cut_rec_info_slot(int e) {
+    return e < 16 ? RS_INFO + e : (e < 19 ? PD_PS + 12 + (e - 16) : PD_PE + 12 + (e - 19));
+}
+static_assert(cut_rec_structural(cut_rec_info_slot(16)) == 0 && cut_rec_info_slot(20) == RS_Z - 1 &&
+                  cut_rec_structural(RS_Z) == 2, "the info's 21 entries: 16 after the comparison data, 5 in its structural slots");
+__device__ __forceinline__ double cut_rec_seeds(double lx0, double ly0) {
+    return __hiloint2double((int)__float_as_uint((float)ly0), (int)__float_as_uint((float)lx0));
+}
+struct CutZeros { float z[3]; };
+__device__ __forceinline__ CutZeros cut_rec_zeros(double seeds) {
+    const float z0 = __uint_as_float((unsigned)__double2loint(seeds)), z1 = __uint_as_float((unsigned)__double2hiint(seeds));
+    return CutZeros{{z0, z1, -(z0 + z1)}};
+}
+__device__ __forceinline__ double cut_rec_value(int x, double v, const CutZeros& zs) {
+    const int i = cut_rec_structural(x);
+    return i < 0 ? v : (double)(i == 0 ? zs.z[0] : (i == 1 ? zs.z[1] : zs.z[2]));
+}
+template <typename LD>
+__device__ __forceinline__ void cut_rec_expand(double* fst, int j, LD ld) {
+    const CutZeros zs = cut_rec_zeros(ld(RS_Z));
+#pragma unroll
+    for (int k = 0; k < PD_ERR / 8; ++k) fst[j + 8 * k] = ld(j + 8 * k);
+#pragma unroll
+    for (int i = 0; i < 3; ++i) fst[PD_PS + 12 + i] = fst[PD_PE + 12 + i] = (double)zs.z[i];
+}
+struct CutRec {
+    const double* r;
+    __device__ __forceinline__ double operator[](int x) const {
+        const int i = cut_rec_structural(x);
+        const double v = r[i < 0 ? x : RS_Z];
+        return i < 0 ? v : cut_rec_value(x, v, cut_rec_zeros(v));
+    }
+    __device__ __forceinline__ double info(int e) const { return r[cut_rec_info_slot(e)]; }
+};
 
 template <typename T>
 __device__ __forceinline__ T sym3_t(const T* A, const T* x, const T* y) {
@@ -256,14 +298,12 @@
             const int m = ((lines ? c : c - nl_ch) << 6) + lane;
             const int cnt = chunk_cnt(c);
             double info[21];
-            double fd[CUT_FAST];
+            double fd[PD_ERR];
             if (lane < cnt) {
                 if (lines) {
                     LineCutData d;
                     load_line(L, lb + mls[m], d);
                     poseInfoOnLine<false>(cam, homog, Dl, d, 0.0, 0.0, info);
-#pragma unroll
-                    for (int i = PD_ERR; i < CUT_FAST; ++i) fd[i] = 0.0;
                     cut_poly_data(Dl, d, homog, fd);
                     fd[PD_NEXT] = (double)mls[min(m + 1, nls - 1)];
                 } else {
@@ -291,7 +331,11 @@
 #pragma unroll
                         for (int k = 0; k < 16; ++k) {
                             const int x = 16 * sl + k;
-                            stg[lane * 17 + k] = x < CUT_FAST ? fd[x] : (x < CUT_FAST + 21 ? info[x - CUT_FAST] : 0.0);
+                            const int h = cut_rec_structural(x);
+                            stg[lane * 17 + k] = x >= RS_INFO ? info[x - RS_INFO]
+                                                 : (h < 0 ? fd[x]
+                                                          : (x == RS_Z ? cut_rec_seeds(fd[PD_PS + 12], fd[PD_PS + 13])
+                                                                       : info[(x < PD_PE ? 16 : 19) + h]));
                         }
                     }
                     wave_lds_sync();
@@ -492,15 +536,16 @@
     const int nls = p.tr.n_matched_ls[b];
     if (m >= nls || (p.cfg.cut_proof != 2 && p.scr.cut_flag[b] == 0)) return;
     const size_t q = (size_t)b * p.kl_cap + p.tr.matched_ls[(size_t)b * p.mls_cap + m];
-    double* rec = p.scr.cut_rec + ((size_t)b * p.mls_cap + m) * CUT_REC;
+    const CutRec rec{p.scr.cut_rec + ((size_t)b * p.mls_cap + m) * CUT_REC};
     double Dl[16];
 #pragma unroll
     for (int i = 0; i < 16; ++i) Dl[i] = p.scr.cut_dtinv[16 * b + i];
     float eb[14];
     cut_line_bounds(p, q, rec[PD_OK] != 0.0, Dl, eb);
-    float* out = reinterpret_cast<float*>(rec + PD_ERR);
+    float* out = reinterpret_cast<float*>(p.scr.cut_err + ((size_t)b * p.mls_cap + m) * CUT_ERR);
 #pragma unroll
     for (int i = 0; i < 14; ++i) out[i] = eb[i];
+    out[14] = out[15] = 0.0f;
 }
 
 #define CUT_G 8
@@ -512,8 +557,10 @@
 #endif
 #define CUT_SL 7
 #define CUT_EP 43
-#define CUT_NX (CUT_FAST + 21)
-static_assert(CUT_REC * 8 == 640 && CUT_NX + 3 <= CUT_REC, "a record is 5 x 128 B: five 16-B loads per lane");
+#define CUT_PIECES (CUT_REC / 16)
+static_assert(CUT_REC * 8 == 512, "a record is 4 x 128 B: four 16-B loads per lane");
+#define CUT_ERR_EB 8
+static_assert(CUT_ERR_EB + 3 <= CUT_ERR && CUT_ERR_EB >= CUT_FAST - PD_ERR, "cut_err: operand bounds | agreement bound");
 
 __device__ __forceinline__ void exact_endpoint(const DevCam& cam, double homog, const double* Dl, const DevLines& L,
                                                size_t q, int side, double t, double* o7) {
@@ -585,11 +632,13 @@
     return __builtin_fma(t, __builtin_fma(t, c2, c1), c0);
 }
 
-__device__ __forceinline__ double cut_ours_P(const double* fd, int side, int i, double t) {
+template <typename FD>
+__device__ __forceinline__ double cut_ours_P(const FD& fd, int side, int i, double t) {
     const int o = side ? PD_PE : PD_PS;
     return h2(fd[o + i], fd[o + 6 + i], fd[o + 12 + i], t);
 }
-__device__ __forceinline__ double cut_ours_V(const double* fd, int side, double t) {
+template <typename FD>
+__device__ __forceinline__ double cut_ours_V(const FD& fd, int side, double t) {
     const int o = side ? PD_VE : PD_VS;
     return __builtin_fma(t, __builtin_fma(t, __builtin_fma(t, __builtin_fma(t, fd[o + 4], fd[o + 3]), fd[o + 2]),
                                           fd[o + 1]), fd[o]);
@@ -770,7 +819,7 @@
                             const int e = 4 * c + i;
                             if (e < 21) {
                                 tmpw[4 * lane + i] = info[e];
-                                tmpw[256 + 4 * lane + i] = recG[(size_t)(s0 + lane) * CUT_REC + CUT_FAST + e];
+                                tmpw[256 + 4 * lane + i] = recG[(size_t)(s0 + lane) * CUT_REC + cut_rec_info_slot(e)];
                             }
                         }
                     }
@@ -800,7 +849,7 @@
             for (int i = 0; i < 7; ++i) epf[CUT_SL * j + i] = o7[i];
         }
 #pragma unroll
-        for (int e = 0; e < 21; ++e) xs[e] = sumE[e] - rec_l[(size_t)m * CUT_REC + CUT_FAST + e];
+        for (int e = 0; e < 21; ++e) xs[e] = sumE[e] - rec_l[(size_t)m * CUT_REC + cut_rec_info_slot(e)];
     }
     wave_lds_sync();
     if (exact) {
@@ -903,7 +952,7 @@
     __shared__ double sumE[CUT_G][CUT_SSTR];
     __shared__ double fst[CUT_G][CUT_FAST + 1];
     constexpr bool PF = !PROOF && !GFPL_CUT_NOPF;
-    __shared__ __attribute__((aligned(16))) double nxl[PF ? 5 : 1][PF ? 128 : 2];
+    __shared__ __attribute__((aligned(16))) double nxl[PF ? CUT_PIECES : 1][PF ? 128 : 2];
     __shared__ double tmp[CUT_G][CUT_EP + 25 + 1];
     static_assert(CUT_G * (CUT_EP + 25 + 1) >= 512, "the exact-sum flush stages 64 x (4 + 4) doubles in tmp");
     __shared__ CutCmp cmpl[CUT_G];
@@ -933,6 +982,7 @@
     const size_t lb = (size_t)(live ? b : 0) * p.kl_cap;
     const int32_t* mls = p.tr.matched_ls + (size_t)(live ? b : 0) * p.mls_cap;
     const double* rec_l = p.scr.cut_rec + (size_t)(live ? b : 0) * p.mls_cap * CUT_REC;
+    double* const err_l = p.scr.cut_err + (size_t)(live ? b : 0) * p.mls_cap * CUT_ERR;
     const double* Dl = p.scr.cut_dtinv + 16 * (size_t)(live ? b : 0);
     const double st = p.cfg.cut_step;
     const double rlo = p.cfg.cut_rng[0], rhi = p.cfg.cut_rng[1];
@@ -1055,7 +1105,7 @@
 #pragma unroll
             for (int i = 1; i < 6; ++i) usable = usable && e6[i] < __builtin_inff();
             n_unb += usable ? 0 : 1;
-            if (j < 6 && live) reinterpret_cast<float*>(const_cast<double*>(rec_l) + (size_t)m * CUT_REC + CUT_NX)[j] = e6[j];
+            if (j < 6 && live) reinterpret_cast<float*>(err_l + (size_t)m * CUT_ERR + CUT_ERR_EB)[j] = e6[j];
         }
         const double vs0 = PROOF ? vtab[g][0] : cl[10], ve0 = PROOF ? vtab[g][CUT_KS] : cl[15];
         dc = cut_dcore_p1<PROOF>(cl[0], vs0, cl[5], ve0, cl[20], cl[29], cl[30], cl[31], cmpl[g].eb, tq, c_ok);
@@ -1064,20 +1114,25 @@
         if (!PF) return;
         const char* src = reinterpret_cast<const char*>(rec_l + (size_t)mm * CUT_REC) + 16 * j;
 #pragma unroll
-        for (int k = 0; k < (PF ? 5 : 0); ++k) {
+        for (int k = 0; k < (PF ? CUT_PIECES : 0); ++k) {
             const uint32_t dst = (uint32_t)(uintptr_t)&nxl[k][0];
             asm volatile("s_mov_b32 m0, %1\n\tglobal_load_lds_dwordx4 %0, off" ::"v"(src + 128 * k), "s"(dst)
                          : "memory", "m0");
         }
+    };
+    auto load_fst = [&]() {
+        const double* rm = rec_l + (size_t)m * CUT_REC;
+        cut_rec_expand(fst[g], j, [&](int s) { return rm[s]; });
+        if (PROOF) fst[g][PD_ERR + j] = err_l[(size_t)m * CUT_ERR + j];
     };
     if (m < nls) {
         q_cur = lb + mls[0];
         if (nls > 1) q_nx = lb + mls[1];
-        for (int e = j; e < CUT_FAST; e += 8) fst[g][e] = rec_l[e];
+        load_fst();
 #pragma unroll
         for (int e = j; e < 21; e += 8) {
             const double s0 = p.scr.cut_sum[24 * b + e];
-            sumA[g][e] = s0 - rec_l[CUT_FAST + e];
+            sumA[g][e] = s0 - rec_l[cut_rec_info_slot(e)];
             sumE[g][e] = s0;
         }
         wave_lds_sync();
@@ -1235,10 +1290,7 @@
                         info[kk] = cut_ours_info(xs, is, ie, ra, cb);
                     }
                 }
-                if (!PF) {
-#pragma unroll
-                    for (int k = 0; k < CUT_FAST / 8; ++k) fst[g][j + 8 * k] = rec_l[(size_t)m * CUT_REC + j + 8 * k];
-                }
+                if (!PF) load_fst();
                 if (!PROOF) {
                     if (PF) asm volatile("s_waitcnt vmcnt(0)" ::: "memory");
                     if (j == 0) {
@@ -1248,11 +1300,7 @@
                     if (rec && 8 * j < lstep)
                         *reinterpret_cast<unsigned long long*>(path + (size_t)(m - 1) * CUT_PATH + 8 * j) =
                             *reinterpret_cast<const unsigned long long*>(&pth[g][8 * j]);
-#pragma unroll
-                    for (int k = 0; k < (PF ? CUT_FAST / 8 : 0); ++k) {
-                        const int e = j + 8 * k;
-                        fst[g][e] = nxl[e >> 4][16 * g + (e & 15)];
-                    }
+                    if (PF) cut_rec_expand(fst[g], j, [&](int s) { return nxl[s >> 4][16 * g + (s & 15)]; });
                 }
             }
             wave_lds_sync();
@@ -1267,7 +1315,9 @@
 #pragma unroll
                 for (int kk = 0; kk < 3; ++kk) {
                     const int e = j + 8 * kk;
-                    const int x = CUT_FAST + e;
+                    int jx = j;
+                    if (kk == 2) asm volatile("" : "+v"(jx));
+                    const int x = cut_rec_info_slot(jx + 8 * kk);
                     if (e < 21) {
                         const double mid = sumA[g][e] + info[kk];
                         const double nw = mid - (PF ? nxl[x >> 4][16 * g + (x & 15)] : rec_l[(size_t)m * CUT_REC + x]);
@@ -1457,10 +1507,10 @@
     };
     if (nls > 0) {
         q_cur = lb + mls[0];
-        for (int e = lane; e < CUT_FAST; e += 64) fst[e] = rec_l[e];
+        if (lane < PD_ERR) fst[lane] = CutRec{rec_l}[lane];
         if (lane < 21) {
             const double s0 = p.scr.cut_sum[24 * b + lane];
-            sumA[lane] = s0 - rec_l[CUT_FAST + lane];
+            sumA[lane] = s0 - rec_l[cut_rec_info_slot(lane)];
             sumE[lane] = s0;
         }
         wave_lds_sync();
@@ -1473,8 +1523,8 @@
             int iv = mn;
             asm volatile("" : "+v"(iv));
             const double* rn = rec_l + (size_t)iv * CUT_REC;
-            pf_i0 = lane < 21 ? rn[CUT_FAST + lane] : 0.0;
-            pf_f0 = rn[lane < CUT_FAST ? lane : 0];
+            pf_i0 = lane < 21 ? rn[cut_rec_info_slot(lane)] : 0.0;
+            pf_f0 = CutRec{rn}[lane < PD_ERR ? lane : 0];
             pf_q = mls[iv];
         }
     };
@@ -1736,7 +1786,7 @@
             TCK(0);
             if (m < nls) {
                 wave_lds_sync();
-                if (lane < CUT_FAST) fst[lane] = pf_f0;
+                if (lane < PD_ERR) fst[lane] = pf_f0;
                 if (lane < 21) sumA[lane] = (sumA[lane] + info) - pf_i0;
                 q_cur = lb + __builtin_amdgcn_readfirstlane(pf_q);
                 first = 1;
@@ -1808,7 +1858,7 @@
         for (int kk = 0; kk < 3; ++kk) {
             const int e = j + 8 * kk;
             if (e < 21) {
-                ci[kk] = rec_l[(size_t)m * CUT_REC + CUT_FAST + e];
+                ci[kk] = rec_l[(size_t)m * CUT_REC + cut_rec_info_slot(e)];
                 ss[kk] = se[kk] - ci[kk];
                 smat[g][e] = se[kk];
             }
@@ -1998,7 +2048,7 @@
 }
 
 __device__ __forceinline__ void vref_replay(const KParams& p, int b, int m) {
-    const double* fd = p.scr.cut_rec + ((size_t)b * p.mls_cap + m) * CUT_REC;
+    const CutRec fd{p.scr.cut_rec + ((size_t)b * p.mls_cap + m) * CUT_REC};
     double* out = p.scr.cut_vmax + ((size_t)b * p.mls_cap + m) * CUT_VMAX;
     const uint8_t* path = p.scr.cut_path + ((size_t)b * p.mls_cap + m) * CUT_PATH;
     const DevLines& L = p.prev.ls;
@@ -2190,7 +2240,7 @@
             const int ln = it >> 6, side = (it >> 5) & 1, kk = it & 31;
             const int mm = blockIdx.x * 64 + ln;
             const size_t q = (size_t)b * p.kl_cap + qln[ln];
-            const double* fd = p.scr.cut_rec + ((size_t)b * p.mls_cap + mm) * CUT_REC;
+            const CutRec fd{p.scr.cut_rec + ((size_t)b * p.mls_cap + mm) * CUT_REC};
             double P0[3], P1[3], C0[9], C1[9], Jl[2], qc[5];
             const double* A3 = side ? L.eP : L.sP;
             const double* B3 = side ? L.sP : L.eP;
@@ -2245,7 +2295,7 @@
     const int b = blockIdx.y;
     const int m = blockIdx.x * 64 + threadIdx.x;
     if (m >= p.tr.n_matched_ls[b]) return;
-    const double* fd = p.scr.cut_rec + ((size_t)b * p.mls_cap + m) * CUT_REC;
+    const CutRec fd{p.scr.cut_rec + ((size_t)b * p.mls_cap + m) * CUT_REC};
     if (fd[PD_OK] == 0.0) return;
     const size_t q = (size_t)b * p.kl_cap + p.tr.matched_ls[(size_t)b * p.mls_cap + m];
     double Dl[16];
@@ -2296,7 +2346,7 @@
 }
 
 __device__ __attribute__((noinline)) int verify_line_detail(const KParams& p, const double* Dl, size_t q,
-                                                            const uint8_t* path_m, const double* fd, double r0f,
+                                                            const uint8_t* path_m, const CutRec fd, double r0f,
                                                             double r1f, double K0, double A1, double B1, double cs,
                                                             double ce, double R0, double rts, double rte, bool line_ok,
                                                             const double* Scol, int sstride, int& n_xchk) {
@@ -2341,7 +2391,7 @@
                     if (!(vok && line_ok && E * 1.0001 <= R0)) {
                         double Sref[21], Sfull[21];
 #pragma unroll
-                        for (int e = 0; e < 21; ++e) { Sfull[e] = Scol[sstride * e]; Sref[e] = Sfull[e] - fd[CUT_FAST + e]; }
+                        for (int e = 0; e < 21; ++e) { Sfull[e] = Scol[sstride * e]; Sref[e] = Sfull[e] - fd.info(e); }
                         ++n_xchk;
                         if (!verify_exact_step(p, Dl, q, r0, r1, first, Sref, Sfull, (by & CUT_P_STAY) ? CUT_P_STAY : (by & 7)))
                             bad |= 512;
@@ -2368,7 +2418,7 @@
     double K0, A1, B1, cs, ce, R0, rts, rte, epsS, kt;
     int ok;
 };
-__device__ __forceinline__ LineBound verify_line_bound(const KParams& p, size_t q, const double* fd, const double* vmx,
+__device__ __forceinline__ LineBound verify_line_bound(const KParams& p, size_t q, const CutRec fd, const double* vmx,
                                                       const double* Dl, const double* So, const double* Sf) {
     const double rlo = p.cfg.cut_rng[0], rhi = p.cfg.cut_rng[1];
     const double T = fmax(fabs(rlo), fabs(rhi));
@@ -2442,7 +2492,7 @@
 #pragma unroll
             for (int k = 0; k < 6; ++k) {
                 const int e = tri(i > k ? i : k, i > k ? k : i);
-                const double sref = Sf[65 * e] - fd[CUT_FAST + e];
+                const double sref = Sf[65 * e] - fd.info(e);
                 const double dd = 1.0000000000000004 * fabs(So[65 * e] - sref);
                 dSn = dSn + dd * sqrt(sg[i] * sg[k]);
             }
@@ -2491,7 +2541,7 @@
     double sA = 0.0, sE = 0.0;
     if (nls > 0 && lane < 21) {
         const double s0 = p.scr.cut_sum[24 * b + lane];
-        sA = s0 - rec_l[CUT_FAST + lane];
+        sA = s0 - rec_l[cut_rec_info_slot(lane)];
         sE = s0;
     }
 #ifdef GFPL_VERIFY_CLOCK
@@ -2505,7 +2555,7 @@
         const int m = c0 + lane;
         const bool on = m < nls;
         const size_t q = lb + (on ? mls[m] : mls[0]);
-        const double* fd = rec_l + (size_t)(on ? m : 0) * CUT_REC;
+        const CutRec fd{rec_l + (size_t)(on ? m : 0) * CUT_REC};
         const double r0f = L.cut[2 * q], r1f = L.cut[2 * q + 1];
         {
             LineCutData d;
@@ -2551,7 +2601,7 @@
 #pragma unroll
                 for (int k = 0; k < 17; ++k) {
                     const int mm = c0 + l0 + k;
-                    v[k] = (l0 + k <= cnt && mm < nls) ? rec_l[(size_t)mm * CUT_REC + CUT_FAST + lane] : 0.0;
+                    v[k] = (l0 + k <= cnt && mm < nls) ? rec_l[(size_t)mm * CUT_REC + cut_rec_info_slot(lane)] : 0.0;
                 }
             };
             double iv[17];
@@ -2668,7 +2718,7 @@
         const int b = e / p.mls_cap, m = e % p.mls_cap;
         const double* pl = p.scr.cut_dtl + (size_t)i * 32;
         const size_t q = (size_t)b * p.kl_cap + p.tr.matched_ls[(size_t)b * p.mls_cap + m];
-        const double* fd = p.scr.cut_rec + ((size_t)b * p.mls_cap + m) * CUT_REC;
+        const CutRec fd{p.scr.cut_rec + ((size_t)b * p.mls_cap + m) * CUT_REC};
         const uint8_t* path = p.scr.cut_path + ((size_t)b * p.mls_cap + m) * CUT_PATH;
         double Dl[16];
 #pragma unroll
diff --git a/gf-pl-slam_amd/gfpl/__init__.py b/gf-pl-slam_amd/gfpl/__init__.py
--- a/gf-pl-slam_amd/gfpl/__init__.py
+++ b/gf-pl-slam_amd/gfpl/__init__.py
@@ -15,6 +15,7 @@
 MAX_LEVELS = 8
 MAX_MATCHED_PT = 2048
 MAX_MATCHED_LS = 1024
+CUT_REC, CUT_ERR = 64, 12
 PREV, CURR = 0, 1
 HAMMING, HAMMING2 = 1, 2
 
@@ -336,6 +337,7 @@
             "gfpl_last_step_track_counts": ([P, P], C.c_int),
             "gfpl_last_step_cut_proof": ([P, P], C.c_int),
             "gfpl_debug_cut_records": ([P, C.c_int, P, C.c_int], C.c_int),
+            "gfpl_debug_cut_bounds": ([P, C.c_int, P, C.c_int], C.c_int),
             "gfpl_debug_step_records": ([P, P], C.c_int),
             "gfpl_debug_clocks": ([P, P], C.c_int),
             "gfpl_lsd_create": ([P, P, C.c_int, C.c_int, C.c_int, C.c_int, C.c_int, C.POINTER(P)], C.c_int),
@@ -942,8 +944,13 @@
         return {"redone": int(v[0]), "steps_proven": int(v[1]), "vref_evals": int(v[2]), "lines": int(v[3])}
 
     def debug_cut_records(self, b: int, n_lines: int) -> np.ndarray:
-        out = np.zeros((n_lines, 80), np.float64)
+        out = np.zeros((n_lines, CUT_REC), np.float64)
         check(self.L.gfpl_debug_cut_records(self.h, b, out.ctypes.data, n_lines), "debug_cut_records")
+        return out
+
+    def debug_cut_bounds(self, b: int, n_lines: int) -> np.ndarray:
+        out = np.zeros((n_lines, CUT_ERR), np.float64)
+        check(self.L.gfpl_debug_cut_bounds(self.h, b, out.ctypes.data, n_lines), "debug_cut_bounds")
         return out
 
     def debug_step_records(self) -> np.ndarray:
diff --git a/include/gfpl.h b/include/gfpl.h
--- a/include/gfpl.h
+++ b/include/gfpl.h
@@ -375,6 +375,7 @@
 int  gfpl_last_step_track_counts(gfpl_seqbatch* sb, int64_t* counts4);
 int  gfpl_last_step_cut_proof(gfpl_seqbatch* sb, int64_t* counts4);
 int  gfpl_debug_cut_records(gfpl_seqbatch* sb, int b, double* out, int n_lines);
+int  gfpl_debug_cut_bounds(gfpl_seqbatch* sb, int b, double* out, int n_lines);
 int  gfpl_debug_step_records(gfpl_seqbatch* sb, int64_t* out);
 int  gfpl_debug_clocks(gfpl_seqbatch* sb, int64_t* out);
 int  gfpl_get_kernel_times(gfpl_ctx* ctx, float* ms4);
```

After: 798,800. No clear change (-0.4%).
